# sangyun884/HR-VITON

Measured on AMD Instinct MI355X. Metric: 1024x768 try-on images/sec (train_generator.py step: tocg+glue, G fwd/bwd, D fwd/bwd x2, VGG, Adam), higher is better.
Workload: dtype bf16; 1 GPU; BASELINE configs[3] (SURVEY 8d config #4, headline): train_generator.py 1024x768, 4 img/GPU, --fp16 (bf16 MFMA operands, fp32 accumulate), SPADE ng...; global_batch=4, height=1024, width=768, parallelism=dp1-allreduce, persistent_grid_cus=256, dist_backend=none (single process), world_size=1, rccl_ranks=0

## Files before the change

hr-viton_amd/_lib.py:

```python
from __future__ import annotations

import ctypes as C
import os

HERE = os.path.dirname(os.path.abspath(__file__))
LIB_PATH = os.path.join(HERE, "libhrviton_hip.so")

HRV_MAX_SRC = 4
ACT_NONE, ACT_RELU, ACT_LRELU, ACT_TANH = 0, 1, 2, 3


class hrv_src_t(C.Structure):
    _fields_ = [("ptr", C.c_void_p), ("C", C.c_int32), ("cstride", C.c_int32), ("coff", C.c_int32),
                ("up_shift", C.c_int32), ("pre_act", C.c_int32), ("C_real", C.c_int32)]


class hrv_spade_epi_t(C.Structure):
    _fields_ = [("x", C.c_void_p), ("x_cstride", C.c_int32), ("x_coff", C.c_int32), ("C", C.c_int32),
                ("_pad", C.c_int32), ("mean", C.c_void_p), ("rstd", C.c_void_p), ("noise_z", C.c_void_p),
                ("noise_scale", C.c_void_p), ("g1p_out", C.c_void_p)]


class hrv_norm_bwd_t(C.Structure):
    _fields_ = [("N", C.c_int32), ("H", C.c_int32), ("W", C.c_int32), ("C", C.c_int32),
                ("x", C.c_void_p), ("x_cstride", C.c_int32), ("x_coff", C.c_int32),
                ("noise_z", C.c_void_p), ("noise_scale", C.c_void_p), ("mean", C.c_void_p), ("rstd", C.c_void_p),
                ("out", C.c_void_p), ("out_cstride", C.c_int32), ("out_coff", C.c_int32),
                ("g1p", C.c_void_p), ("g1p_cstride", C.c_int32), ("g1p_coff", C.c_int32),
                ("dout", C.c_void_p), ("dout_cstride", C.c_int32), ("dout_coff", C.c_int32),
                ("dnh", C.c_void_p), ("dnh_cstride", C.c_int32), ("dnh_coff", C.c_int32),
                ("dgb", C.c_void_p), ("dgb_cstride", C.c_int32), ("dgb_coff", C.c_int32),
                ("dx", C.c_void_p), ("dx_cstride", C.c_int32), ("dx_coff", C.c_int32),
                ("dx_accumulate", C.c_int32), ("act", C.c_int32), ("act_slope", C.c_float),
                ("dns_accumulate", C.c_int32), ("dnoise_scale", C.c_void_p), ("workspace", C.c_void_p),
                ("dgb_bf16", C.c_int32), ("out_bf16", C.c_int32), ("dx_bf16", C.c_int32), ("g1p_bf16", C.c_int32),
                ("dnh_bf16", C.c_int32), ("dout_bf16", C.c_int32),
                ("x_up_channels", C.c_int32), ("x2", C.c_void_p), ("x2_cstride", C.c_int32), ("x2_coff", C.c_int32)]


class hrv_sn_job_t(C.Structure):
    _fields_ = [("w", C.c_void_p), ("u", C.c_void_p), ("v", C.c_void_p), ("sigma", C.c_void_p), ("u_keep", C.c_void_p),
                ("v_keep", C.c_void_p), ("R", C.c_int32), ("K", C.c_int32)]


class hrv_thin_conv_t(C.Structure):
    _fields_ = [("src", C.c_void_p), ("N", C.c_int32), ("H", C.c_int32), ("W", C.c_int32), ("src_channels", C.c_int32),
                ("src_cstride", C.c_int32), ("src_coff", C.c_int32),
                ("w_oihw", C.c_void_p), ("Cout", C.c_int32), ("Cin", C.c_int32), ("KH", C.c_int32), ("KW", C.c_int32),
                ("sigma", C.c_void_p), ("wscale", C.c_float), ("mode", C.c_int32), ("shift", C.c_void_p),
                ("residual", C.c_void_p), ("res_cstride", C.c_int32), ("res_coff", C.c_int32), ("res_bf16", C.c_int32),
                ("res_mode", C.c_int32), ("act", C.c_int32), ("act_slope", C.c_float),
                ("out", C.c_void_p), ("out_cstride", C.c_int32), ("out_coff", C.c_int32), ("out_bf16", C.c_int32)]


class hrv_conv_cout1_t(C.Structure):
    _fields_ = [("x", C.c_void_p), ("N", C.c_int32), ("H", C.c_int32), ("W", C.c_int32), ("C", C.c_int32),
                ("x_cstride", C.c_int32), ("x_coff", C.c_int32), ("w_oihw", C.c_void_p), ("sigma", C.c_void_p),
                ("wscale", C.c_float), ("bias", C.c_void_p), ("K", C.c_int32), ("pad", C.c_int32),
                ("y", C.c_void_p), ("y_cstride", C.c_int32), ("y_coff", C.c_int32),
                ("dx", C.c_void_p), ("dx_cstride", C.c_int32), ("dx_coff", C.c_int32),
                ("add", C.c_void_p), ("add_cstride", C.c_int32), ("add_coff", C.c_int32),
                ("workspace", C.c_void_p), ("round_bf16", C.c_int32)]


class hrv_spade_gb_t(C.Structure):
    _fields_ = [("mode", C.c_int32), ("N", C.c_int32), ("H", C.c_int32), ("W", C.c_int32),
                ("src", C.c_void_p), ("src_cstride", C.c_int32), ("src_coff", C.c_int32), ("w_packed", C.c_void_p),
                ("C", C.c_int32), ("Cp", C.c_int32), ("hid", C.c_int32), ("x_f32", C.c_int32),
                ("x", C.c_void_p), ("x_cstride", C.c_int32), ("x_coff", C.c_int32),
                ("stat_stride", C.c_int32), ("g1p_bf16", C.c_int32),
                ("mean", C.c_void_p), ("rstd", C.c_void_p), ("noise_z", C.c_void_p), ("noise_scale", C.c_void_p),
                ("bias_gamma", C.c_void_p), ("bias_beta", C.c_void_p), ("g1p", C.c_void_p),
                ("act", C.c_int32), ("act_slope", C.c_float),
                ("out", C.c_void_p), ("out_cstride", C.c_int32), ("out_coff", C.c_int32), ("out_f32", C.c_int32),
                ("_pad", C.c_int32), ("mask", C.c_void_p), ("mask_cstride", C.c_int32), ("mask_coff", C.c_int32)]


class hrv_spade_fused_t(C.Structure):
    _fields_ = [("N", C.c_int32), ("H", C.c_int32), ("W", C.c_int32), ("C", C.c_int32),
                ("seg", C.c_void_p), ("seg_H", C.c_int32), ("seg_W", C.c_int32), ("seg_shift", C.c_int32), ("x_f32", C.c_int32),
                ("w_packed", C.c_void_p),
                ("x", C.c_void_p), ("x_cstride", C.c_int32), ("x_coff", C.c_int32),
                ("mean", C.c_void_p), ("rstd", C.c_void_p), ("noise_z", C.c_void_p), ("noise_scale", C.c_void_p),
                ("bias_gamma", C.c_void_p), ("bias_beta", C.c_void_p), ("g1p", C.c_void_p),
                ("act", C.c_int32), ("act_slope", C.c_float),
                ("out", C.c_void_p), ("out_cstride", C.c_int32), ("out_coff", C.c_int32),
                ("actv", C.c_void_p), ("actv_cstride", C.c_int32), ("actv_coff", C.c_int32),
                ("x_up_channels", C.c_int32), ("x2", C.c_void_p), ("x2_cstride", C.c_int32), ("x2_coff", C.c_int32)]


class hrv_conv_p2_t(C.Structure):
    _fields_ = [("N", C.c_int32), ("H", C.c_int32), ("W", C.c_int32), ("Cin", C.c_int32),
                ("src", C.c_void_p), ("src_cstride", C.c_int32), ("src_coff", C.c_int32), ("Cout", C.c_int32),
                ("w_packed", C.c_void_p), ("bias", C.c_void_p),
                ("act", C.c_int32), ("act_slope", C.c_float),
                ("mask", C.c_void_p), ("mask_cstride", C.c_int32), ("mask_coff", C.c_int32), ("mask_slope", C.c_float), ("out_f32", C.c_int32),
                ("out", C.c_void_p), ("out_cstride", C.c_int32), ("out_coff", C.c_int32),
                ("res_f32", C.c_int32), ("residual", C.c_void_p), ("res_cstride", C.c_int32), ("res_coff", C.c_int32),
                ("res_after_mask", C.c_int32)]


class hrv_conv_s2_t(C.Structure):
    _fields_ = [("mode", C.c_int32),
                ("N", C.c_int32), ("Hs", C.c_int32), ("Ws", C.c_int32), ("K", C.c_int32),
                ("src", C.c_void_p), ("src_cstride", C.c_int32), ("src_coff", C.c_int32),
                ("Ho", C.c_int32), ("Wo", C.c_int32), ("cols", C.c_int32), ("Cph", C.c_int32),
                ("w_packed", C.c_void_p), ("bias", C.c_void_p),
                ("act", C.c_int32), ("act_slope", C.c_float),
                ("out", C.c_void_p), ("out_cstride", C.c_int32), ("out_coff", C.c_int32), ("out_f32", C.c_int32),
                ("residual", C.c_void_p), ("res_cstride", C.c_int32), ("res_coff", C.c_int32), ("res_f32", C.c_int32),
                ("mask", C.c_void_p), ("mask_cstride", C.c_int32), ("mask_coff", C.c_int32), ("mask_slope", C.c_float)]


class hrv_s2_pack_job_t(C.Structure):
    _fields_ = [("mode_flags", C.c_int32), ("K", C.c_int32), ("cols", C.c_int32), ("Cph", C.c_int32),
                ("w", C.c_void_p), ("sigma", C.c_void_p), ("wscale", C.c_float), ("_pad", C.c_int32), ("out", C.c_void_p)]


class hrv_conv2d_t(C.Structure):
    _fields_ = [("N", C.c_int32), ("H", C.c_int32), ("W", C.c_int32), ("Ho", C.c_int32), ("Wo", C.c_int32),
                ("KH", C.c_int32), ("KW", C.c_int32), ("stride", C.c_int32), ("pad", C.c_int32),
                ("nsrc", C.c_int32), ("src", hrv_src_t * HRV_MAX_SRC),
                ("w_packed", C.c_void_p), ("w_oihw", C.c_void_p), ("Cout", C.c_int32), ("tile_cfg", C.c_int32),
                ("scale", C.c_void_p), ("shift", C.c_void_p), ("residual", C.c_void_p),
                ("res_cstride", C.c_int32), ("res_coff", C.c_int32), ("act", C.c_int32), ("act_slope", C.c_float),
                ("out", C.c_void_p), ("out_cstride", C.c_int32), ("out_coff", C.c_int32),
                ("spade", C.POINTER(hrv_spade_epi_t)), ("out_up_shift", C.c_int32), ("_pad2", C.c_int32),
                ("workspace", C.c_void_p), ("workspace_bytes", C.c_int64),
                ("pad_w_plus1", C.c_int32), ("free_extent", C.c_int32), ("out_step", C.c_int32),
                ("out_off_h", C.c_int32), ("out_off_w", C.c_int32), ("out_H", C.c_int32), ("out_W", C.c_int32),
                ("res_mode", C.c_int32), ("mixed_flags", C.c_int32), ("_pad3", C.c_int32)]


class hrv_flow_warp_t(C.Structure):
    _fields_ = [("src", C.c_void_p), ("N", C.c_int32), ("H", C.c_int32), ("W", C.c_int32), ("C", C.c_int32),
                ("src_cstride", C.c_int32), ("src_coff", C.c_int32), ("flow", C.c_void_p),
                ("fh", C.c_int32), ("fw", C.c_int32), ("Ho", C.c_int32), ("Wo", C.c_int32),
                ("rh", C.c_float), ("rw", C.c_float), ("norm_x", C.c_float), ("norm_y", C.c_float),
                ("out", C.c_void_p), ("out_cstride", C.c_int32), ("out_coff", C.c_int32), ("flow_up", C.c_void_p)]


class hrv_flow_warp_bwd_t(C.Structure):
    _fields_ = [("src", C.c_void_p), ("N", C.c_int32), ("H", C.c_int32), ("W", C.c_int32), ("C", C.c_int32),
                ("src_cstride", C.c_int32), ("src_coff", C.c_int32), ("flow_up", C.c_void_p),
                ("Ho", C.c_int32), ("Wo", C.c_int32), ("norm_x", C.c_float), ("norm_y", C.c_float),
                ("dout", C.c_void_p), ("dout_cstride", C.c_int32), ("dout_coff", C.c_int32),
                ("dsrc", C.c_void_p), ("dsrc_cstride", C.c_int32), ("dsrc_coff", C.c_int32),
                ("dflow", C.c_void_p), ("dflow_accumulate", C.c_int32), ("_pad", C.c_int32)]


class hrv_lpips_tap_t(C.Structure):
    _fields_ = [("f0", C.c_void_p), ("f1", C.c_void_p), ("lin", C.c_void_p),
                ("HW", C.c_int32), ("C", C.c_int32), ("cstride", C.c_int32), ("_pad", C.c_int32)]


_i32, _i64, _f, _vp = C.c_int32, C.c_int64, C.c_float, C.c_void_p
_ip = C.POINTER(C.c_int32)
SYMBOLS = {
    "hrv_version": (C.c_char_p, []),
    "hrv_last_error": (C.c_char_p, []),
    "hrv_device_check": (C.c_int, []),
    "hrv_set_reserved_cus": (C.c_int, [_i32]),
    "hrv_persistent_cus": (C.c_int, []),
    "hrv_diag_set_tlog": (C.c_int, [_vp, _i64]),
    "hrv_diag_reload_env": (C.c_int, []),
    "hrv_conv2d_pick_tile": (C.c_int, [_i64, _i32]),
    "hrv_conv2d_tile_bn": (C.c_int, [_i32]),
    "hrv_conv2d_tile_bm": (C.c_int, [_i32]),
    "hrv_conv2d_tile_row_bytes": (C.c_int, [_i32]),
    "hrv_conv2d_packed_elems": (_i64, [_i32, _i32, _i32, _i32, _ip, _i32]),
    "hrv_conv2d_pack_weight_f32": (C.c_int, [_vp, _i32, _i32, _i32, _i32, _ip, _ip, _i32, _vp]),
    "hrv_conv2d_pack_weight_dev_f32": (C.c_int, [_vp, _i32, _i32, _i32, _i32, _ip, _ip, _i32, _i32, _i32, _i32, _i32,
                                                 _i32, _f, _vp, _vp, _ip, _vp]),
    "hrv_conv2d_pack_weight_dev_bf16": (C.c_int, [_vp, _i32, _i32, _i32, _i32, _ip, _ip, _i32, _i32, _i32, _i32, _i32,
                                                  _i32, _f, _vp, _vp, _ip, _vp]),
    "hrv_conv2d_pack_record_bytes": (_i32, []),
    "hrv_conv2d_pack_weight_record": (C.c_int, [_vp, _i32, _i32, _i32, _i32, _ip, _ip, _i32, _i32, _i32, _i32, _i32, _i32, _f,
                                                _vp, _i32, _vp, _i32, _i32, _vp, _ip, _vp, _ip]),
    "hrv_conv2d_pack_weight_multi": (C.c_int, [_vp, _vp, _i32, _i32, _vp]),
    "hrv_conv2d_wgrad_workspace_bytes": (_i64, [_i32, _i32, _i32, _i32, _i64]),
    "hrv_conv2d_wgrad_nhwc_f32": (C.c_int, [_vp, _i32, _i32, _i32, _vp, _i32, _i32, _i32, _i32, _i32, _i32, _i32,
                                            _i32, _i32, _i32, _i32, _i32, _i32, _i32, _i32, _i32, _vp, _i64, _vp, _i32,
                                            _vp, _i32, _vp]),
    "hrv_conv2d_wgrad_bf16mma_nhwc_f32": (C.c_int, [_vp, _i32, _i32, _i32, _vp, _i32, _i32, _i32, _i32, _i32, _i32,
                                                    _i32, _i32, _i32, _i32, _i32, _i32, _i32, _i32, _i32, _i32, _vp,
                                                    _i64, _vp, _i32, _vp, _i32, _vp]),
    "hrv_conv2d_wgrad_bf16mma_st_nhwc_f32": (C.c_int, [_vp, _i32, _i32, _i32, _vp, _i32, _i32, _i32, _i32, _i32, _i32,
                                                       _i32, _i32, _i32, _i32, _i32, _i32, _i32, _i32, _i32, _i32,
                                                       _vp, _i64, _vp, _i32, _vp, _i32, _i32, _vp]),
    "hrv_colsum_nhwc_f32": (C.c_int, [_vp, _i64, _i32, _i32, _i32, _vp, _i64, _vp, _i32, _vp]),
    "hrv_norm_bwd_workspace_elems": (_i64, [_i32, _i32, _i32, _i32]),
    "hrv_spade_norm_bwd2_nhwc_f32": (C.c_int, [C.POINTER(hrv_norm_bwd_t), C.POINTER(hrv_norm_bwd_t), _vp]),
    "hrv_spade_norm_bwd_nhwc_f32": (C.c_int, [C.POINTER(hrv_norm_bwd_t), _vp]),
    "hrv_thin_conv_supported": (C.c_int, [_i32, _i32, _i32, _i32]),
    "hrv_thin_conv_bf16": (C.c_int, [C.POINTER(hrv_thin_conv_t), _vp]),
    "hrv_loss_f32": (C.c_int, [_vp, _vp, _i64, _i32, _f, _f, _vp, _vp, _vp, _i32, _vp]),
    "hrv_loss_bf16in_f32": (C.c_int, [_vp, _vp, _i64, _i32, _f, _f, _vp, _vp, _vp, _i32, _vp]),
    "hrv_scale_f32": (C.c_int, [_vp, _i64, _f, _vp, _vp]),
    "hrv_act_bwd_nhwc_f32": (C.c_int, [_vp, _i32, _i32, _vp, _i32, _i32, _i32, _i64, _i32, _f, _vp]),
    "hrv_tanh_bwd_f32": (C.c_int, [_vp, _vp, _i64, _vp, _vp]),
    "hrv_add_slice_nhwc_f32": (C.c_int, [_vp, _i32, _i32, _vp, _i32, _i32, _i32, _i64, _i32, _vp]),
    "hrv_downsum2x2_nhwc_f32": (C.c_int, [_vp, _i32, _i32, _i32, _i32, _i32, _i32, _vp, _i32, _i32, _i32, _vp]),
    "hrv_avgpool3x3s2_bwd_nhwc_f32": (C.c_int, [_vp, _i32, _i32, _i32, _i32, _i32, _i32, _vp, _i32, _i32, _i32, _vp]),
    "hrv_maxpool2x2_nhwc_f32": (C.c_int, [_vp, _i32, _i32, _i32, _i32, _vp, _vp]),
    "hrv_maxpool2x2_nhwc_bf16": (C.c_int, [_vp, _i32, _i32, _i32, _i32, _vp, _vp]),
    "hrv_maxpool2x2_bwd_nhwc_f32": (C.c_int, [_vp, _vp, _i32, _i32, _i32, _i32, _vp, _vp]),
    "hrv_maxpool2x2_bwd_relu_nhwc_f32": (C.c_int, [_vp, _vp, _i32, _i32, _i32, _i32, _vp, _vp]),
    "hrv_maxpool2x2_bwd_relu_nhwc_xbf16": (C.c_int, [_vp, _vp, _i32, _i32, _i32, _i32, _vp, _vp]),
    "hrv_maxpool2x2_bwd_relu_nhwc_bf16": (C.c_int, [_vp, _vp, _i32, _i32, _i32, _i32, _vp, _vp]),
    "hrv_add_slice_nhwc_bf16": (C.c_int, [_vp, _i32, _i32, _vp, _i32, _i32, _i32, _i64, _i32, _vp]),
    "hrv_adam_f32": (C.c_int, [_vp, _vp, _vp, _vp, _i64, _f, _f, _f, _f, _f, _i32, _f, _vp]),
    "hrv_adam_hyper_f32": (C.c_int, [_vp, _vp, _f, _f, _vp, _vp]),
    "hrv_adam_dev_f32": (C.c_int, [_vp, _vp, _vp, _vp, _i64, _vp, _f, _f, _f, _f, _f, _vp]),
    "hrv_spectral_norm_f32": (C.c_int, [_vp, _i32, _i32, _vp, _vp, _i32, _f, _vp, _vp, _vp]),
    "hrv_spectral_norm_bwd_f32": (C.c_int, [_vp, _vp, _vp, _vp, _vp, _i32, _i32, _vp, _vp, _i32, _vp]),
    "hrv_spectral_norm_batched_f32": (C.c_int, [_vp, _i32, _i32, _f, _vp, _vp]),
    "hrv_conv2d_pack_weight_pair_dev": (C.c_int, [_vp, _vp, _i32, _i32, _i32, _i32, _i32, _i32, _ip, _ip, _i32, _i32, _i32,
                                                  _i32, _vp, _ip, _vp]),
    "hrv_spade_vec_prep_f32": (C.c_int, [_vp, _vp, _vp, _i32, _vp, _vp, _vp]),
    "hrv_spade_vec_prep_multi_f32": (C.c_int, [_i32, _vp, _vp, _vp, _vp, _vp, _vp, _vp, _vp, _vp]),
    "hrv_shared_taps_prep_f32": (C.c_int, [_vp, _vp, _i32, _i32, _i32, _i32, _vp, _vp, _vp]),
    "hrv_shared_taps_grad_f32": (C.c_int, [_vp, _vp, _i32, _i32, _i32, _i32, _vp, _vp, _vp]),
    "hrv_conv2d_workspace_bytes": (_i64, [C.POINTER(hrv_conv2d_t)]),
    "hrv_conv2d_nhwc_f32": (C.c_int, [C.POINTER(hrv_conv2d_t), _vp]),
    "hrv_conv2d_packed_elems_bf16": (_i64, [_i32, _i32, _i32, _i32, _ip, _i32]),
    "hrv_conv2d_pack_weight_bf16": (C.c_int, [_vp, _i32, _i32, _i32, _i32, _ip, _ip, _i32, _vp]),
    "hrv_conv2d_nhwc_bf16": (C.c_int, [C.POINTER(hrv_conv2d_t), _vp]),
    "hrv_conv2d_naive_nhwc_f32": (C.c_int, [C.POINTER(hrv_conv2d_t), _vp]),
    "hrv_tapsum_nhwc_f32": (C.c_int, [_vp, _i32, _i32, _i32, _i32, _i32, _i32, _i32, _i32, _vp, _vp, _i32, _vp, _i32,
                                      _vp]),
    "hrv_instnorm_workspace_elems": (_i64, [_i32, _i32, _i32, _i32]),
    "hrv_instnorm_stats_nhwc_f32": (C.c_int, [_vp, _i32, _i32, _i32, _i32, _i32, _i32, _vp, _vp, _f, _vp, _vp, _vp,
                                              _vp]),
    "hrv_instnorm_stats2_nhwc_f32": (C.c_int, [_vp, _i32, _i32, _i32, _i32, _i32, _i32, _vp, _vp, _vp, _vp, _f, _vp, _vp, _vp, _vp, _vp, _vp]),
    "hrv_instnorm_stats2_up_nhwc_f32": (C.c_int, [_vp, _i32, _i32, _i32, _vp, _i32, _i32, _i32, _i32, _i32, _i32, _vp, _vp, _vp, _vp, _f, _vp,
                                                  _vp, _vp, _vp, _vp, _vp]),
    "hrv_instnorm_stats_nhwc_bf16": (C.c_int, [_vp, _i32, _i32, _i32, _i32, _i32, _i32, _vp, _vp, _f, _vp, _vp, _vp,
                                               _vp]),
    "hrv_instnorm_apply_nhwc_f32": (C.c_int, [_vp, _i32, _i32, _i32, _i32, _i32, _i32, _vp, _vp, _i32, _f, _vp, _i32,
                                              _i32, _vp]),
    "hrv_avgpool3x3s2_nhwc_f32": (C.c_int, [_vp, _i32, _i32, _i32, _i32, _i32, _i32, _vp, _i32, _i32, _vp]),
    "hrv_mul_channel_nhwc_f32": (C.c_int, [_vp, _i32, _i32, _vp, _i32, _i32, _i32, _i64, _vp]),
    "hrv_gauss_blur_nhwc_f32": (C.c_int, [_vp, _i32, _i32, _i32, _i32, _i32, _vp, _i32, _vp, _vp, _vp]),
    "hrv_parse_argmax_nhwc_f32": (C.c_int, [_vp, _i32, _i32, _i64, _vp, _vp, _i32, _vp]),
    "hrv_resize_nchw_f32": (C.c_int, [_vp, _i32, _i32, _i32, _i32, _i32, _i32, _vp, _vp]),
    "hrv_occlusion_nhwc_f32": (C.c_int, [_vp, _i32, _i32, _vp, _i32, _vp, _i32, _i32, _i64, _vp]),
    "hrv_nchw_to_nhwc_f32": (C.c_int, [_vp, _i32, _i32, _i32, _i32, _vp, _i32, _i32, _i32, _vp]),
    "hrv_nchw_f32_to_nhwc_bf16": (C.c_int, [_vp, _i32, _i32, _i32, _i32, _vp, _i32, _i32, _i32, _vp]),
    "hrv_nhwc_bf16_to_nchw_f32": (C.c_int, [_vp, _i32, _i32, _i32, _i32, _i32, _i32, _vp, _vp]),
    "hrv_nhwc_to_nchw_f32": (C.c_int, [_vp, _i32, _i32, _i32, _i32, _i32, _i32, _vp, _vp]),
    "hrv_space_to_depth2_nhwc_f32": (C.c_int, [_vp, _i32, _i32, _i32, _i32, _i32, _i32, _vp, _vp]),
    "hrv_depth_to_space2_nhwc_f32": (C.c_int, [_vp, _i32, _i32, _i32, _i32, _vp, _vp]),
    "hrv_conv_cout1_fwd_f32": (C.c_int, [C.POINTER(hrv_conv_cout1_t), _vp]),
    "hrv_conv_cout1_dgrad_f32": (C.c_int, [C.POINTER(hrv_conv_cout1_t), _vp]),
    "hrv_conv_cout1_wgrad_slabs": (_i32, [_i32, _i32, _i32]),
    "hrv_conv_cout1_wgrad_f32": (C.c_int, [C.POINTER(hrv_conv_cout1_t), _vp, _i32, _vp, _i32, _vp]),
    "hrv_concat_nhwc_nchw_f32": (C.c_int, [_vp, _i32, _i32, _i32, _vp, _i32, _i32, _i32, _i32, _vp, _i32, _vp]),
    "hrv_resize_bilinear_nhwc_f32": (C.c_int, [_vp, _i32, _i32, _i32, _i32, _i32, _i32, _i32, _i32, _f, _f,
                                               _vp, _i32, _i32, _vp, _i32, _i32, _vp]),
    "hrv_flow_warp_nhwc_f32": (C.c_int, [C.POINTER(hrv_flow_warp_t), _vp]),
    "hrv_bn_finalize_f32": (C.c_int, [_vp, _vp, _i32, _i32, _i32, _f, _i64, _vp, _vp, _f, _f, _vp, _vp, _vp, _vp, _vp,
                                      _vp, _vp]),
    "hrv_affine_act_nhwc_f32": (C.c_int, [_vp, _i32, _i32, _i32, _i64, _vp, _vp, _vp, _i32, _i32, _i32, _f, _vp, _i32,
                                          _i32, _vp]),
    "hrv_bn_bwd_workspace_elems": (_i64, [_i32]),
    "hrv_bn_bwd_nhwc_f32": (C.c_int, [_vp, _i32, _i32, _vp, _i32, _i32, _i32, _i64, _vp, _vp, _vp, _vp, _vp, _i32, _i32,
                                      _i32, _vp, _vp, _i32, _vp]),
    "hrv_resize_bilinear_bwd_nhwc_f32": (C.c_int, [_vp, _i32, _i32, _i32, _i32, _i32, _i32, _f, _f, _vp, _i32, _i32,
                                                   _i32, _i32, _i32, _vp]),
    "hrv_resize_nearest_nchw_f32": (C.c_int, [_vp, _i32, _i32, _i32, _i32, _i32, _vp, _vp]),
    "hrv_resize_nearest_nchw_bwd_f32": (C.c_int, [_vp, _i32, _i32, _i32, _i32, _i32, _vp, _vp]),
    "hrv_resize_nearest_nhwc_f32": (C.c_int, [_vp, _i32, _i32, _i32, _i32, _i32, _i32, _i32, _i32, _vp, _i32, _i32, _vp, _i32, _i32, _vp]),
    "hrv_resize_nearest_bwd_nhwc_f32": (C.c_int, [_vp, _i32, _i32, _i32, _i32, _i32, _i32, _vp, _i32, _i32, _i32, _i32, _i32, _vp]),
    "hrv_flow_warp_bwd_nhwc_f32": (C.c_int, [C.POINTER(hrv_flow_warp_bwd_t), _vp]),
    "hrv_grid_sample_nchw_f32": (C.c_int, [_vp, _i32, _i32, _i32, _i32, _vp, _i32, _i32, _vp, _vp]),
    "hrv_grid_sample_nchw_bwd_f32": (C.c_int, [_vp, _i32, _i32, _i32, _i32, _vp, _i32, _i32, _vp, _vp, _vp, _vp]),
    "hrv_softmax_nchw_f32": (C.c_int, [_vp, _i32, _i32, _i64, _vp, _vp]),
    "hrv_softmax_nchw_bwd_f32": (C.c_int, [_vp, _vp, _i32, _i32, _i64, _vp, _vp]),
    "hrv_cross_entropy_nchw_f32": (C.c_int, [_vp, _vp, _i32, _i32, _i64, _f, _vp, _vp, _vp, _vp]),
    "hrv_tapsum_bwd_nhwc_f32": (C.c_int, [_vp, _i32, _i32, _i32, _i32, _i32, _i32, _i32, _i32, _vp, _i32, _vp]),
    "hrv_tap_expand_nhwc": (C.c_int, [_vp, _i32, _i32, _i32, _i32, _i32, _i32, _i32, _i32, _i32, _i32, _vp, _vp]),
    "hrv_mul_f32": (C.c_int, [_vp, _vp, _i64, _vp, _vp]),
    "hrv_spade_gb_packed_bytes": (_i64, [_i32, _i32, _i32, _i32]),
    "hrv_spade_gb_supported": (C.c_int, [_i32, _i32, _i32, _i32, _i32, _i32, _i32]),
    "hrv_spade_gb_pack_dev": (C.c_int, [_i32, _vp, _vp, _i32, _i32, _i32, _vp, _vp]),
    "hrv_spade_gb_bf16": (C.c_int, [C.POINTER(hrv_spade_gb_t), _vp]),
    "hrv_conv_p2_packed_bytes": (C.c_int64, [_i32, _i32]),
    "hrv_conv_p2_supported": (C.c_int, [_i32, _i32, _i32, _i32, _i32]),
    "hrv_conv_p2_pack_dev": (C.c_int, [_i32, _vp, _vp, _i32, _i32, _vp, _f, _vp, _vp]),
    "hrv_conv_p2_bf16": (C.c_int, [C.POINTER(hrv_conv_p2_t), _vp]),
    "hrv_conv_s2_packed_bytes": (C.c_int64, [_i32, _i32, _i32]),
    "hrv_conv_s2_supported": (C.c_int, [_i32, _i32, _i32, _i32, _i32, _i32, _i32]),
    "hrv_conv_s2_pack_dev": (C.c_int, [_i32, _vp, _i32, _i32, _i32, _vp, _f, _vp, _vp]),
    "hrv_conv_s2_pack_multi_dev": (C.c_int, [_i32, C.POINTER(hrv_s2_pack_job_t), _vp]),
    "hrv_conv_s2_bf16": (C.c_int, [C.POINTER(hrv_conv_s2_t), _vp]),
    "hrv_space_to_depth2_cells_bf16": (C.c_int, [_vp, _i32, _i32, _i32, _i32, _i32, _i32, _i32, _i32, _i32, _vp, _vp]),
    "hrv_instnorm_apply_nhwc_bf16out": (C.c_int, [_vp, _i32, _i32, _i32, _i32, _i32, _i32, _vp, _vp, _i32, _f, _vp, _i32, _i32, _vp]),
    "hrv_scale_bf16": (C.c_int, [_vp, _i64, _f, _vp, _vp]),
    "hrv_split3_nhwc_bf16": (C.c_int, [_vp, _i64, _i32, _i32, _i32, _vp, _vp]),
    "hrv_conv2d_wgrad_s2_supported": (C.c_int, [_i32, _i32, _i32, _i32, _i32, _i32, _i32, _i32, _i32]),
    "hrv_conv2d_wgrad_tr_supported": (C.c_int, [_i32, _i32, _i32, _i32, _i32, _i32, _i32, _i32, _i32, _i32, _i32, _i32]),
    "hrv_pad_width_nhwc_bf16": (C.c_int, [_vp, _i64, _i32, _i32, _i32, _vp, _vp]),
    "hrv_spade_fused_packed_bytes": (C.c_int64, [_i32]),
    "hrv_spade_fused_supported": (C.c_int, [_i32, _i32, _i32, _i32, _i32, _i32]),
    "hrv_spade_fused_pack_dev": (C.c_int, [_vp, _vp, _i32, _vp, _vp, _i32, _vp, _vp]),
    "hrv_spade_fused_bf16": (C.c_int, [C.POINTER(hrv_spade_fused_t), _vp]),
    "hrv_tv_loss_f32": (C.c_int, [_vp, _i32, _i32, _i32, _vp, _vp, _vp, _vp]),
    "hrv_rgb_to_gray_u8": (C.c_int, [_vp, _i64, _vp, _vp]),
    "hrv_pair_stats_workspace_bytes": (_i64, [_i32, _i32, _i32]),
    "hrv_pair_stats_u8": (C.c_int, [_vp, _vp, _vp, _i32, _i32, _i32, _vp, _i64, _vp, _vp, _vp]),
    "hrv_lpips_prep_u8": (C.c_int, [_vp, _i32, _i32, _i32, C.POINTER(C.c_float), C.POINTER(C.c_float), _vp, _vp]),
    "hrv_lpips_prep_nchw_f32": (C.c_int, [_vp, _i32, _i32, _i32, _i32, C.POINTER(C.c_float), C.POINTER(C.c_float), _vp, _vp]),
    "hrv_maxpool3x3s2_nhwc_f32": (C.c_int, [_vp, _i32, _i32, _i32, _i32, _vp, _vp]),
    "hrv_lpips_head_f32": (C.c_int, [C.POINTER(hrv_lpips_tap_t), _i32, _i32, _vp, _vp]),
}

_lib = None


class HrvError(RuntimeError):
    pass


def load():
    global _lib
    if _lib is not None:
        return _lib
    if not os.path.exists(LIB_PATH):
        raise HrvError(
            f"{LIB_PATH} is missing: build it with `python -c 'import __graft_entry__ as g; g.build()'` "
            "(hipcc --offload-arch=gfx950). There is no CPU fallback for the HIP path.")
    lib = C.CDLL(LIB_PATH)
    for name, (res, args) in SYMBOLS.items():
        fn = getattr(lib, name)
        fn.restype = res
        fn.argtypes = args
    _lib = lib
    return lib


def reload_env():
    if _lib is not None:
        _lib.hrv_diag_reload_env()


# ... 5 lines not shown
```

hr-viton_amd/csrc/train.hip:

```cpp
#include <string.h>

#include "hrv_common.h"

namespace hrv {

typedef float f32x4 __attribute__((ext_vector_type(4)));

static inline int grid_for(size_t work, int block = 256) {
  size_t g = (work + block - 1) / block;
  const size_t cap = 256 * 16;
  return (int)(g < 1 ? 1 : (g > cap ? cap : g));
}

__device__ __forceinline__ float dact(float y, int act, float slope) {
  if (act == HRV_ACT_RELU) return y > 0.f ? 1.f : 0.f;
  if (act == HRV_ACT_LRELU) return y > 0.f ? 1.f : slope;
  return 1.f;
}

struct XSrc {
  const float* x; int x_cs, x_co;
  const float* x2; int x2_cs, x2_co, up_g;
  int H, W;
};
struct XThread {
  const float* base;
  int cs, lo, W, Wl;
};
__device__ __forceinline__ XThread xsrc_thread(const XSrc& s, int n, int g) {
  XThread t;
  t.W = s.W; t.Wl = s.W >> 1;
  t.lo = (s.up_g > 0 && g < s.up_g) ? 1 : 0;
  if (s.up_g > 0 && !t.lo) {
    t.cs = s.x2_cs;
    t.base = s.x2 + (size_t)n * s.H * s.W * s.x2_cs + s.x2_co + (g - s.up_g) * 4;
  } else {
    t.cs = s.x_cs;
    t.base = s.x + (size_t)n * (t.lo ? (s.H >> 1) * (s.W >> 1) : s.H * s.W) * s.x_cs + s.x_co + g * 4;
  }
  return t;
}
__device__ __forceinline__ const float* xsrc_ptr(const XThread& t, int px) {
  int q = px;
  if (t.lo) {
    const int h = px / t.W, w = px - h * t.W;
    q = (h >> 1) * t.Wl + (w >> 1);
  }
  return t.base + (size_t)q * t.cs;
}

struct NormBwdParams {
  XSrc xs;
  const float* z; const float* ns;
  const float* mean; const float* rstd;
  const float* out; int out_cs, out_co;
  const float* g1p; int g_cs, g_co;
  const float* dout; int do_cs, do_co;
  float* dnh; int dn_cs, dn_co;
  float* dgb; int dgb_cs, dgb_co;
  int N, H, W, C4, act; float slope;
  int NB; float* part;
  int dgb_bf16, out_bf16;
  int g1p_bf16;
  int dnh_bf16;
  int dout_bf16;
  int dbeta_in_place;
};

__device__ __forceinline__ f32x4 ld4(const float* p) { return *reinterpret_cast<const f32x4*>(p); }
__device__ __forceinline__ f32x4 ld4_bf16(const void* base, size_t elem) {
  const uint2 u = *reinterpret_cast<const uint2*>(reinterpret_cast<const unsigned short*>(base) + elem);
  f32x4 v;
  v[0] = __builtin_bit_cast(float, u.x << 16); v[1] = __builtin_bit_cast(float, u.x & 0xFFFF0000u);
  v[2] = __builtin_bit_cast(float, u.y << 16); v[3] = __builtin_bit_cast(float, u.y & 0xFFFF0000u);
  return v;
}
typedef __bf16 bf16x4t __attribute__((ext_vector_type(4)));
__device__ __forceinline__ void st4_bf16(void* base, size_t elem, f32x4 v) {
  *reinterpret_cast<bf16x4t*>(reinterpret_cast<unsigned short*>(base) + elem) = __builtin_convertvector(v, bf16x4t);
}

__global__ __launch_bounds__(256) void norm_bwd_stage1_kernel(const NormBwdParams p) {
  __shared__ f32x4 red[2][256];
  const int n = blockIdx.y, b = blockIdx.x, t = threadIdx.x;
  const int HW = p.H * p.W, C = p.C4 * 4;
  const int PB = (HW + p.NB - 1) / p.NB;
  const int p0 = b * PB, p1 = min(p0 + PB, HW);
  const int GB = p.C4 < NORM_GCAP ? p.C4 : NORM_GCAP;
  const int R = 256 / GB;
  const int r = t / GB, gl = t - r * GB;
  {
    const int g = blockIdx.z * GB + gl;
    f32x4 s1 = (f32x4)(0.f), s2 = (f32x4)(0.f);
    if (r < R && g < p.C4) {
      const f32x4 mu = ld4(p.mean + (size_t)n * C + g * 4), rs = ld4(p.rstd + (size_t)n * C + g * 4);
      const f32x4 ns4 = p.z ? ld4(p.ns + g * 4) : (f32x4)(0.f);
      const XThread xt = xsrc_thread(p.xs, n, g);
      struct In { f32x4 v, d, o, g1; float zz; };
      auto load = [&](int px) {
        In L;
        const size_t pix = (size_t)n * HW + px;
        L.v = ld4(xsrc_ptr(xt, px));
        L.zz = 0.f;
        if (p.z) {
          const int h = px / p.W, w = px - h * p.W;
          L.zz = p.z[((size_t)n * p.W + w) * p.H + h];
        }
        L.d = p.dout_bf16 ? ld4_bf16(p.dout, pix * p.do_cs + p.do_co + g * 4) : ld4(p.dout + pix * p.do_cs + p.do_co + g * 4);
        L.o = (f32x4)(0.f);
        if (p.act != HRV_ACT_NONE) {
          const size_t oe = pix * p.out_cs + p.out_co + g * 4;
          L.o = p.out_bf16 ? ld4_bf16(p.out, oe) : ld4(p.out + oe);
        }
        L.g1 = (f32x4)(1.f);
        if (p.g1p) {
          const size_t ge1 = pix * p.g_cs + p.g_co + g * 4;
          L.g1 = p.g1p_bf16 ? ld4_bf16(p.g1p, ge1) : ld4(p.g1p + ge1);
        }
        return L;
      };
      auto finish = [&](int px, const In& L) {
        const size_t pix = (size_t)n * HW + px;
        f32x4 v = L.v;
        if (p.z) v += L.zz * ns4;
        const f32x4 nh = (v - mu) * rs;
        f32x4 dpre = L.d;
        if (p.act != HRV_ACT_NONE) {
#pragma unroll
          for (int e = 0; e < 4; ++e) dpre[e] *= dact(L.o[e], p.act, p.slope);
        }
        f32x4 dnh = dpre;
        if (p.g1p) dnh *= L.g1;
        if (p.dnh_bf16) st4_bf16(p.dnh, pix * p.dn_cs + p.dn_co + g * 4, dnh);
        else *reinterpret_cast<f32x4*>(p.dnh + pix * p.dn_cs + p.dn_co + g * 4) = dnh;
        if (p.dgb) {
          const size_t ge = pix * p.dgb_cs + p.dgb_co + g * 4;
          if (p.dgb_bf16) {
            st4_bf16(p.dgb, ge, dpre * nh);
            if (!p.dbeta_in_place) st4_bf16(p.dgb, ge + C, dpre);
          } else {
            *reinterpret_cast<f32x4*>(p.dgb + ge) = dpre * nh;
            if (!p.dbeta_in_place) *reinterpret_cast<f32x4*>(p.dgb + ge + C) = dpre;
          }
        }
        s1 += dnh;
        s2 += dnh * nh;
      };
      int px = p0 + r;
      for (; px + R < p1; px += 2 * R) {
        const In A = load(px), B = load(px + R);
        finish(px, A);
        finish(px + R, B);
      }
      if (px < p1) finish(px, load(px));
    }
    red[0][t] = s1;
    red[1][t] = s2;
    __syncthreads();
    if (r == 0 && g < p.C4) {
      for (int rr = 1; rr < R; ++rr) { s1 += red[0][rr * GB + gl]; s2 += red[1][rr * GB + gl]; }
      float* dst = p.part + (((size_t)n * p.NB + b) * C + g * 4) * 2;
#pragma unroll
      for (int e = 0; e < 4; ++e) { dst[2 * e] = s1[e]; dst[2 * e + 1] = s2[e]; }
    }
  }
}

__global__ void norm_bwd_finalize_kernel(const float* __restrict__ part, int N, int NB, int C, int HW,
                                         float* __restrict__ m1, float* __restrict__ m2) {
  const int t = blockIdx.x * blockDim.x + threadIdx.x;
  const int i = t >> 4, l = t & 15;
  const bool live = i < N * C;
  const int ii = live ? i : 0;
  const int n = ii / C, c = ii - n * C;
  double s1 = 0.0, s2 = 0.0;
  for (int b = l; b < NB; b += 16) {
    const float* src = part + (((size_t)n * NB + b) * C + c) * 2;
    s1 += (double)src[0];
    s2 += (double)src[1];
  }
#pragma unroll
  for (int o = 8; o > 0; o >>= 1) {
    s1 += __shfl_xor(s1, o, 16);
    s2 += __shfl_xor(s2, o, 16);
  }
  if (live && l == 0) {
    m1[i] = (float)(s1 / HW);
    m2[i] = (float)(s2 / HW);
  }
}

struct NormBwd2Params {
  XSrc xs;
  const float* z; const float* ns;
  const float* mean; const float* rstd; const float* m1; const float* m2;
  const float* dnh; int dn_cs, dn_co; int dnh_bf16;
  float* dx; int dx_cs, dx_co; int accumulate;
  int dx_bf16;
  int N, H, W, C4;
  int NB; float* part;
};

__global__ __launch_bounds__(256) void norm_bwd_stage2_kernel(const NormBwd2Params p) {
  __shared__ f32x4 red[256];
  const int n = blockIdx.y, b = blockIdx.x, t = threadIdx.x;
  const int HW = p.H * p.W, C = p.C4 * 4;
  const int PB = (HW + p.NB - 1) / p.NB;
  const int p0 = b * PB, p1 = min(p0 + PB, HW);
  const int GB = p.C4 < NORM_GCAP ? p.C4 : NORM_GCAP;
  const int R = 256 / GB;
  const int r = t / GB, gl = t - r * GB;
  {
    const int g = blockIdx.z * GB + gl;
    f32x4 sz = (f32x4)(0.f);
    if (r < R && g < p.C4) {
      const size_t sc = (size_t)n * C + g * 4;
      const f32x4 mu = ld4(p.mean + sc), rs = ld4(p.rstd + sc), a1 = ld4(p.m1 + sc), a2 = ld4(p.m2 + sc);
      const f32x4 ns4 = p.z ? ld4(p.ns + g * 4) : (f32x4)(0.f);
      const XThread xt = xsrc_thread(p.xs, n, g);
      struct In { f32x4 v, dn, acc; float zz; };
      auto load = [&](int px) {
        In L;
        const size_t pix = (size_t)n * HW + px;
        L.v = ld4(xsrc_ptr(xt, px));
        L.zz = 0.f;
        if (p.z) {
          const int h = px / p.W, w = px - h * p.W;
          L.zz = p.z[((size_t)n * p.W + w) * p.H + h];
        }
        const size_t de = pix * p.dn_cs + p.dn_co + g * 4;
        L.dn = p.dnh_bf16 ? ld4_bf16(p.dnh, de) : ld4(p.dnh + de);
        L.acc = (f32x4)(0.f);
        if (!p.dx_bf16 && p.accumulate) L.acc = ld4(p.dx + pix * p.dx_cs + p.dx_co + g * 4);
        return L;
      };
      auto finish = [&](int px, const In& L) {
#pragma clang fp contract(off)
        const size_t pix = (size_t)n * HW + px;
        f32x4 v = L.v;
        if (p.z) v += L.zz * ns4;
        const f32x4 nh = (v - mu) * rs;
        f32x4 d = rs * (L.dn - a1 - nh * a2);
        sz += d * L.zz;
        if (p.dx_bf16) {
          st4_bf16(p.dx, pix * p.dx_cs + p.dx_co + g * 4, d);
        } else {
          float* o = p.dx + pix * p.dx_cs + p.dx_co + g * 4;
          if (p.accumulate) d += L.acc;
          *reinterpret_cast<f32x4*>(o) = d;
        }
      };
      int px = p0 + r;
      for (; px + R < p1; px += 2 * R) {
        const In A = load(px), B = load(px + R);
        finish(px, A);
        finish(px + R, B);
      }
      if (px < p1) finish(px, load(px));
    }
    if (p.z) {
      red[t] = sz;
      __syncthreads();
      if (r == 0 && g < p.C4) {
        for (int rr = 1; rr < R; ++rr) sz += red[rr * GB + gl];
        *reinterpret_cast<f32x4*>(p.part + ((size_t)n * p.NB + b) * C + g * 4) = sz;
      }
    }
  }
}

__global__ __launch_bounds__(256) void norm_bwd2_stage1_kernel(const NormBwdParams pa, const NormBwdParams pb) {
  __shared__ f32x4 red[4][256];
  const NormBwdParams& p = pa;
  const int n = blockIdx.y, b = blockIdx.x, t = threadIdx.x;
  const int HW = p.H * p.W, C = p.C4 * 4;
  const int PB = (HW + p.NB - 1) / p.NB;
  const int p0 = b * PB, p1 = min(p0 + PB, HW);
  const int GB = p.C4 < NORM_GCAP ? p.C4 : NORM_GCAP;
  const int R = 256 / GB;
  const int r = t / GB, gl = t - r * GB;
  const int g = blockIdx.z * GB + gl;
  f32x4 s1a = (f32x4)(0.f), s2a = (f32x4)(0.f), s1b = (f32x4)(0.f), s2b = (f32x4)(0.f);
  if (r < R && g < p.C4) {
    const f32x4 mua = ld4(pa.mean + (size_t)n * C + g * 4), rsa = ld4(pa.rstd + (size_t)n * C + g * 4);
    const f32x4 mub = ld4(pb.mean + (size_t)n * C + g * 4), rsb = ld4(pb.rstd + (size_t)n * C + g * 4);
    const f32x4 nsa = pa.z ? ld4(pa.ns + g * 4) : (f32x4)(0.f), nsb = pb.z ? ld4(pb.ns + g * 4) : (f32x4)(0.f);
    const XThread xt = xsrc_thread(p.xs, n, g);
    struct In1 { f32x4 d, o, g1; float zz; };
    struct In { f32x4 v; In1 a, b; };
    auto load1 = [&](const NormBwdParams& q, size_t pix, int h, int w) {
      In1 L;
      L.zz = q.z ? q.z[((size_t)n * p.W + w) * p.H + h] : 0.f;
      L.d = q.dout_bf16 ? ld4_bf16(q.dout, pix * q.do_cs + q.do_co + g * 4) : ld4(q.dout + pix * q.do_cs + q.do_co + g * 4);
      L.o = (f32x4)(0.f);
      if (q.act != HRV_ACT_NONE) {
        const size_t oe = pix * q.out_cs + q.out_co + g * 4;
        L.o = q.out_bf16 ? ld4_bf16(q.out, oe) : ld4(q.out + oe);
      }
      L.g1 = (f32x4)(1.f);
      if (q.g1p) {
        const size_t ge1 = pix * q.g_cs + q.g_co + g * 4;
        L.g1 = q.g1p_bf16 ? ld4_bf16(q.g1p, ge1) : ld4(q.g1p + ge1);
      }
      return L;
    };
    auto load = [&](int px) {
      In L;
      const size_t pix = (size_t)n * HW + px;
      L.v = ld4(xsrc_ptr(xt, px));
      const int h = px / p.W, w = px - h * p.W;
      L.a = load1(pa, pix, h, w);
      L.b = load1(pb, pix, h, w);
      return L;
    };
    auto finish1 = [&](const NormBwdParams& q, size_t pix, f32x4 v, const In1& L, f32x4 mu, f32x4 rs, f32x4 ns4, f32x4& s1, f32x4& s2) {
      if (q.z) v += L.zz * ns4;
      const f32x4 nh = (v - mu) * rs;
      f32x4 dpre = L.d;
      if (q.act != HRV_ACT_NONE) {
#pragma unroll
        for (int e = 0; e < 4; ++e) dpre[e] *= dact(L.o[e], q.act, q.slope);
      }
      f32x4 dnh = dpre;
      if (q.g1p) dnh *= L.g1;
      if (q.dnh_bf16) st4_bf16(q.dnh, pix * q.dn_cs + q.dn_co + g * 4, dnh);
      else *reinterpret_cast<f32x4*>(q.dnh + pix * q.dn_cs + q.dn_co + g * 4) = dnh;
      if (q.dgb) {
        const size_t ge = pix * q.dgb_cs + q.dgb_co + g * 4;
        if (q.dgb_bf16) {
          st4_bf16(q.dgb, ge, dpre * nh);
          if (!q.dbeta_in_place) st4_bf16(q.dgb, ge + C, dpre);
        } else {
          *reinterpret_cast<f32x4*>(q.dgb + ge) = dpre * nh;
          if (!q.dbeta_in_place) *reinterpret_cast<f32x4*>(q.dgb + ge + C) = dpre;
        }
      }
      s1 += dnh;
      s2 += dnh * nh;
    };
    auto finish = [&](int px, const In& L) {
      const size_t pix = (size_t)n * HW + px;
      finish1(pa, pix, L.v, L.a, mua, rsa, nsa, s1a, s2a);
      finish1(pb, pix, L.v, L.b, mub, rsb, nsb, s1b, s2b);
    };
    for (int px = p0 + r; px < p1; px += R) finish(px, load(px));
  }
  red[0][t] = s1a; red[1][t] = s2a; red[2][t] = s1b; red[3][t] = s2b;
  __syncthreads();
  if (r == 0 && g < p.C4) {
    for (int rr = 1; rr < R; ++rr) {
      s1a += red[0][rr * GB + gl]; s2a += red[1][rr * GB + gl];
      s1b += red[2][rr * GB + gl]; s2b += red[3][rr * GB + gl];
    }
    const size_t o = (((size_t)n * p.NB + b) * C + g * 4) * 2;
#pragma unroll
    for (int e = 0; e < 4; ++e) {
      pa.part[o + 2 * e] = s1a[e]; pa.part[o + 2 * e + 1] = s2a[e];
      pb.part[o + 2 * e] = s1b[e]; pb.part[o + 2 * e + 1] = s2b[e];
    }
  }
}

__global__ __launch_bounds__(256) void norm_bwd2_stage2_kernel(const NormBwd2Params pa, const NormBwd2Params pb) {
  __shared__ f32x4 red[2][256];
  const NormBwd2Params& p = pa;
  const int n = blockIdx.y, b = blockIdx.x, t = threadIdx.x;
  const int HW = p.H * p.W, C = p.C4 * 4;
  const int PB = (HW + p.NB - 1) / p.NB;
  const int p0 = b * PB, p1 = min(p0 + PB, HW);
  const int GB = p.C4 < NORM_GCAP ? p.C4 : NORM_GCAP;
  const int R = 256 / GB;
  const int r = t / GB, gl = t - r * GB;
  const int g = blockIdx.z * GB + gl;
  f32x4 sza = (f32x4)(0.f), szb = (f32x4)(0.f);
  if (r < R && g < p.C4) {
    const size_t sc = (size_t)n * C + g * 4;
    const f32x4 mua = ld4(pa.mean + sc), rsa = ld4(pa.rstd + sc), a1a = ld4(pa.m1 + sc), a2a = ld4(pa.m2 + sc);
    const f32x4 mub = ld4(pb.mean + sc), rsb = ld4(pb.rstd + sc), a1b = ld4(pb.m1 + sc), a2b = ld4(pb.m2 + sc);
    const f32x4 nsa = pa.z ? ld4(pa.ns + g * 4) : (f32x4)(0.f), nsb = pb.z ? ld4(pb.ns + g * 4) : (f32x4)(0.f);
    const XThread xt = xsrc_thread(p.xs, n, g);
    struct In { f32x4 v, dna, dnb; float za, zb; };
    auto load = [&](int px) {
      In L;
      const size_t pix = (size_t)n * HW + px;
      L.v = ld4(xsrc_ptr(xt, px));
      const int h = px / p.W, w = px - h * p.W;
      const size_t zi = ((size_t)n * p.W + w) * p.H + h;
      L.za = pa.z ? pa.z[zi] : 0.f;
      L.zb = pb.z ? pb.z[zi] : 0.f;
      const size_t dea = pix * pa.dn_cs + pa.dn_co + g * 4, deb = pix * pb.dn_cs + pb.dn_co + g * 4;
      L.dna = pa.dnh_bf16 ? ld4_bf16(pa.dnh, dea) : ld4(pa.dnh + dea);
      L.dnb = pb.dnh_bf16 ? ld4_bf16(pb.dnh, deb) : ld4(pb.dnh + deb);
      return L;
    };
    auto finish = [&](int px, const In& L) {
#pragma clang fp contract(off)
      const size_t pix = (size_t)n * HW + px;
      f32x4 va = L.v, vb = L.v;
      if (pa.z) va += L.za * nsa;
      if (pb.z) vb += L.zb * nsb;
      const f32x4 nha = (va - mua) * rsa, nhb = (vb - mub) * rsb;
      const f32x4 da = rsa * (L.dna - a1a - nha * a2a);
      const f32x4 db = rsb * (L.dnb - a1b - nhb * a2b);
      sza += da * L.za;
      szb += db * L.zb;
      *reinterpret_cast<f32x4*>(p.dx + pix * p.dx_cs + p.dx_co + g * 4) = db + da;
    };
    int px = p0 + r;
    for (; px + R < p1; px += 2 * R) {
      const In A = load(px), B = load(px + R);
      finish(px, A);
      finish(px + R, B);
    }
    if (px < p1) finish(px, load(px));
  }
  red[0][t] = sza; red[1][t] = szb;
  __syncthreads();
  if (r == 0 && g < p.C4) {
    for (int rr = 1; rr < R; ++rr) { sza += red[0][rr * GB + gl]; szb += red[1][rr * GB + gl]; }
    if (pa.z) *reinterpret_cast<f32x4*>(pa.part + ((size_t)n * p.NB + b) * C + g * 4) = sza;
    if (pb.z) *reinterpret_cast<f32x4*>(pb.part + ((size_t)n * p.NB + b) * C + g * 4) = szb;
  }
}

template <bool AB>
__global__ __launch_bounds__(256) void loss_kernel(const float* __restrict__ a, const float* __restrict__ b, size_t n,
                                                   int mode_flags, float gscale, float* __restrict__ grad,
                                                   float* __restrict__ part, int vec) {
  __shared__ float red[256];
  float s = 0.f;
  const int mode = mode_flags & 15;
  const bool relu_mask = (mode_flags & 16) != 0;
  const bool grad_bf16 = (mode_flags & 32) != 0;
  auto term = [&](float x, float y, float& g) -> float {
    float l;
    if (mode == 0) { const float d = x - y; l = fabsf(d); g = d > 0.f ? 1.f : (d < 0.f ? -1.f : 0.f); }
    else if (mode == 1) { l = fmaxf(1.f + x, 0.f); g = x > -1.f ? 1.f : 0.f; }
    else if (mode == 2) { l = fmaxf(1.f - x, 0.f); g = x < 1.f ? -1.f : 0.f; }
    else if (mode == 3) { l = -x; g = -1.f; }
    else { const float d = x - y; l = d * d; g = 2.f * d; }
    g = (relu_mask && !(x > 0.f)) ? 0.f : gscale * g;
    return l;
  };
  typedef unsigned short u16x4v __attribute__((ext_vector_type(4)));
  auto ld4v = [](const float* p, size_t k) -> f32x4 {
    if constexpr (AB) {
      const u16x4v h = *reinterpret_cast<const u16x4v*>(reinterpret_cast<const unsigned short*>(p) + k);
      f32x4 v;
#pragma unroll
      for (int e = 0; e < 4; ++e) v[e] = __builtin_bit_cast(float, (unsigned)h[e] << 16);
      return v;
    } else {
      return *reinterpret_cast<const f32x4*>(p + k);
    }
  };
  const size_t n4 = vec ? n / 4 : 0;
  for (size_t i = (size_t)blockIdx.x * blockDim.x + threadIdx.x; i < n4; i += (size_t)gridDim.x * blockDim.x) {
    const f32x4 x4 = ld4v(a, 4 * i);
    const f32x4 y4 = b ? ld4v(b, 4 * i) : (f32x4)(0.f);
    f32x4 g4;
#pragma unroll
    for (int e = 0; e < 4; ++e) {
      float g;
      s += term(x4[e], y4[e], g);
      g4[e] = g;
    }
    if (grad) {
      if (grad_bf16) st4_bf16(grad, 4 * i, g4);
      else *reinterpret_cast<f32x4*>(grad + 4 * i) = g4;
    }
  }
  for (size_t i = 4 * n4 + (size_t)blockIdx.x * blockDim.x + threadIdx.x; i < n; i += (size_t)gridDim.x * blockDim.x) {
    float x, y = 0.f, g;
    if constexpr (AB) {
      x = __builtin_bit_cast(float, (unsigned)reinterpret_cast<const unsigned short*>(a)[i] << 16);
      if (b) y = __builtin_bit_cast(float, (unsigned)reinterpret_cast<const unsigned short*>(b)[i] << 16);
    } else {
      x = a[i];
      if (b) y = b[i];
    }
    s += term(x, y, g);
    if (grad) {
      if (grad_bf16) reinterpret_cast<unsigned short*>(grad)[i] = (unsigned short)(__builtin_bit_cast(unsigned, __builtin_bit_cast(unsigned, g) + 0x7fffu + ((__builtin_bit_cast(unsigned, g) >> 16) & 1u)) >> 16);
      else grad[i] = g;
    }
  }
  red[threadIdx.x] = s;
  __syncthreads();
  for (int o = 128; o > 0; o >>= 1) {
    if (threadIdx.x < o) red[threadIdx.x] += red[threadIdx.x + o];
    __syncthreads();
  }
  if (threadIdx.x == 0) part[blockIdx.x] = red[0];
}

__global__ void loss_final_kernel(const float* __restrict__ part, int nb, float lscale, float* __restrict__ out,
                                  int accumulate) {
  if (blockIdx.x != 0 || threadIdx.x >= 64) return;
  double s = 0.0;
  for (int i = threadIdx.x; i < nb; i += 64) s += (double)part[i];
#pragma unroll
  for (int o = 32; o > 0; o >>= 1) s += __shfl_down(s, o, 64);
  if (threadIdx.x == 0) {
    const float v = (float)(s * (double)lscale);
    out[0] = accumulate ? out[0] + v : v;
  }
}

__global__ void scale_kernel(float* __restrict__ x, size_t n, float s_host, const float* __restrict__ s_dev) {
  const float s = s_dev ? s_host * s_dev[0] : s_host;
  for (size_t i = (size_t)blockIdx.x * blockDim.x + threadIdx.x; i < n; i += (size_t)gridDim.x * blockDim.x) x[i] *= s;
}

__global__ void tanh_bwd_kernel(const float* __restrict__ dy, const float* __restrict__ y, size_t n, float* __restrict__ out) {
  for (size_t i = (size_t)blockIdx.x * blockDim.x + threadIdx.x; i < n; i += (size_t)gridDim.x * blockDim.x) {
    const float t = y[i];
    out[i] = dy[i] * (1.f - t * t);
  }
}

__global__ void act_bwd_kernel(float* __restrict__ d, int dcs, int dco, const float* __restrict__ y, int ycs, int yco, int C4,
                               size_t npix, int act, float slope) {
  const size_t total = npix * C4;
  for (size_t i = (size_t)blockIdx.x * blockDim.x + threadIdx.x; i < total; i += (size_t)gridDim.x * blockDim.x) {
    const int g = (int)(i % C4);
    const size_t pix = i / C4;
    float* o = d + pix * dcs + dco + g * 4;
    f32x4 v = ld4(o);
    const f32x4 yy = ld4(y + pix * ycs + yco + g * 4);
#pragma unroll
    for (int e = 0; e < 4; ++e) v[e] *= dact(yy[e], act, slope);
    *reinterpret_cast<f32x4*>(o) = v;
  }
}

__global__ void add_slice_kernel(const float* __restrict__ a, int acs, int aco, float* __restrict__ out, int ocs, int oco,
                                 int C4, size_t npix, int accumulate) {
  const size_t total = npix * C4;
  for (size_t i = (size_t)blockIdx.x * blockDim.x + threadIdx.x; i < total; i += (size_t)gridDim.x * blockDim.x) {
    const int g = (int)(i % C4);
    const size_t pix = i / C4;
    f32x4 v = ld4(a + pix * acs + aco + g * 4);
    float* o = out + pix * ocs + oco + g * 4;
    if (accumulate) v += ld4(o);
    *reinterpret_cast<f32x4*>(o) = v;
  }
}

__global__ void downsum2x2_kernel(const float* __restrict__ dhi, int N, int Hl, int Wl, int C4, int hcs, int hco,
                                  float* __restrict__ dlo, int lcs, int lco, int accumulate) {
  const size_t total = (size_t)N * Hl * Wl * C4;
  for (size_t i = (size_t)blockIdx.x * blockDim.x + threadIdx.x; i < total; i += (size_t)gridDim.x * blockDim.x) {
    const int g = (int)(i % C4);
    const size_t pix = i / C4;
    const int w = (int)(pix % Wl);
    const size_t t = pix / Wl;
    const int h = (int)(t % Hl);
    const int n = (int)(t / Hl);
    const float* s = dhi + (((size_t)n * 2 * Hl + 2 * h) * 2 * Wl + 2 * w) * hcs + hco + g * 4;
    f32x4 v = ld4(s) + ld4(s + hcs) + ld4(s + (size_t)2 * Wl * hcs) + ld4(s + (size_t)2 * Wl * hcs + hcs);
    if (accumulate == 2) {
      st4_bf16(dlo, pix * lcs + lco + g * 4, v);
      continue;
    }
    float* o = dlo + pix * lcs + lco + g * 4;
    if (accumulate) v += ld4(o);
    *reinterpret_cast<f32x4*>(o) = v;
  }
}

__global__ void avgpool3s2_bwd_kernel(const float* __restrict__ dy, int N, int H, int W, int C4, int Ho, int Wo,
                                      int ycs, int yco, float* __restrict__ dx, int xcs, int xco, int accumulate) {
  const size_t total = (size_t)N * H * W * C4;
  for (size_t i = (size_t)blockIdx.x * blockDim.x + threadIdx.x; i < total; i += (size_t)gridDim.x * blockDim.x) {
    const int g = (int)(i % C4);
    const size_t pix = i / C4;
// ... 372 lines not shown
  float* const nso = ns_all + j.off_ns[q];
  for (int i = blockIdx.x * 256 + threadIdx.x; i < ncols; i += gridDim.x * 256) {
    const int l = i & 63, c = (i >> 6) * 32 + (l & 31);
    bc[i] = c < C ? (l < 32 ? j.gb[q][c] : j.bb[q][c]) : 0.f;
    if (i < Cp) nso[i] = i < C ? j.ns[q][i] : 0.f;
  }
}

struct SharedTaps {
  const float* w[4];
  const float* b[4];
  float* gw[4];
  float* gb[4];
  int n, hid, c, cp;
};
__global__ __launch_bounds__(256) void shared_taps_prep_kernel(const SharedTaps p, float* __restrict__ wt, float* __restrict__ bt) {
  const int K = 9 * p.cp, total = p.n * p.hid * K;
  for (int i = blockIdx.x * 256 + threadIdx.x; i < total; i += gridDim.x * 256) {
    const int k = i % K, row = i / K;
    const int tap = k / p.cp, ch = k - tap * p.cp;
    const int j = row / p.hid, o = row - j * p.hid;
    wt[i] = ch < p.c ? p.w[j][((size_t)o * p.c + ch) * 9 + tap] : 0.f;
  }
  for (int i = blockIdx.x * 256 + threadIdx.x; i < p.n * p.hid; i += gridDim.x * 256) bt[i] = p.b[i / p.hid][i % p.hid];
}
__global__ __launch_bounds__(256) void shared_taps_grad_kernel(const SharedTaps p, const float* __restrict__ dw,
                                                               const float* __restrict__ db) {
  const int per = p.hid * p.c * 9, total = p.n * per, K = 9 * p.cp;
  for (int i = blockIdx.x * 256 + threadIdx.x; i < total; i += gridDim.x * 256) {
    const int j = i / per, r = i - j * per;
    const int tap = r % 9, ch = (r / 9) % p.c, o = r / (9 * p.c);
    p.gw[j][r] = dw[(size_t)(j * p.hid + o) * K + tap * p.cp + ch];
  }
  for (int i = blockIdx.x * 256 + threadIdx.x; i < p.n * p.hid; i += gridDim.x * 256) p.gb[i / p.hid][i % p.hid] = db[i];
}

}

using namespace hrv;

extern "C" int hrv_spade_vec_prep_f32(const float* gamma_bias, const float* beta_bias, const float* noise_scale, int32_t C,
                                      float* bias_interleaved, float* noise_scale_padded, hrv_stream_t stream) {
  HRV_REQUIRE(gamma_bias && beta_bias && noise_scale && bias_interleaved && noise_scale_padded && C > 0, "spade_vec_prep: bad args");
  const int ncols = (C + 31) / 32 * 64, Cp = (C + 3) / 4 * 4;
  hipLaunchKernelGGL(spade_vec_prep_kernel, dim3((ncols + 255) / 256), dim3(256), 0, (hipStream_t)stream, gamma_bias, beta_bias,
                     noise_scale, C, ncols, Cp, bias_interleaved, noise_scale_padded);
  return check_launch("spade_vec_prep_kernel");
}

extern "C" int hrv_spade_vec_prep_multi_f32(int32_t n, const float* const* gamma_bias, const float* const* beta_bias,
                                            const float* const* noise_scale, const int32_t* C, const int32_t* off_bias, const int32_t* off_noise,
                                            float* bias_interleaved_all, float* noise_scale_padded_all, hrv_stream_t stream) {
  HRV_REQUIRE(n > 0 && n <= VEC_MAXJOBS && gamma_bias && beta_bias && noise_scale && C && off_bias && off_noise && bias_interleaved_all &&
                  noise_scale_padded_all, "spade_vec_prep_multi: 1 .. %d norms", VEC_MAXJOBS);
  VecJobs j;
  memset(&j, 0, sizeof(j));
  int cmax = 0;
  for (int i = 0; i < n; ++i) {
    HRV_REQUIRE(gamma_bias[i] && beta_bias[i] && noise_scale[i] && C[i] > 0 && off_bias[i] >= 0 && off_noise[i] >= 0 && off_bias[i] % 4 == 0 &&
                    off_noise[i] % 4 == 0, "spade_vec_prep_multi: job %d", i);
    j.gb[i] = gamma_bias[i]; j.bb[i] = beta_bias[i]; j.ns[i] = noise_scale[i];
    j.C[i] = C[i]; j.off_bc[i] = off_bias[i]; j.off_ns[i] = off_noise[i];
    if (C[i] > cmax) cmax = C[i];
  }
  const int ncols = (cmax + 31) / 32 * 64;
  hipLaunchKernelGGL(spade_vec_prep_multi_kernel, dim3((ncols + 255) / 256, n), dim3(256), 0, (hipStream_t)stream, j, bias_interleaved_all,
                     noise_scale_padded_all);
  return check_launch("spade_vec_prep_multi_kernel");
}

static int shared_taps_fill(SharedTaps& p, const float* const* w, const float* const* b, float* const* gw, float* const* gb,
                            int32_t n, int32_t hid, int32_t c, int32_t cp) {
  HRV_REQUIRE(n >= 1 && n <= 4 && hid > 0 && c > 0 && cp >= c, "shared_taps: n in 1..4, cp >= c");
  memset(&p, 0, sizeof(p));
  for (int i = 0; i < n; ++i) {
    if (w) { HRV_REQUIRE(w[i] && b[i], "shared_taps: null weight"); p.w[i] = w[i]; p.b[i] = b[i]; }
    if (gw) { HRV_REQUIRE(gw[i] && gb[i], "shared_taps: null gradient"); p.gw[i] = gw[i]; p.gb[i] = gb[i]; }
  }
  p.n = n; p.hid = hid; p.c = c; p.cp = cp;
  return HRV_OK;
}

extern "C" int hrv_shared_taps_prep_f32(const float* const* w, const float* const* b, int32_t n, int32_t hid, int32_t c,
                                        int32_t cp, float* wt, float* bt, hrv_stream_t stream) {
  HRV_REQUIRE(w && b && wt && bt, "shared_taps_prep: null pointer");
  SharedTaps p;
  const int rc = shared_taps_fill(p, w, b, nullptr, nullptr, n, hid, c, cp);
  if (rc) return rc;
  hipLaunchKernelGGL(shared_taps_prep_kernel, dim3(grid_for((size_t)n * hid * 9 * cp)), dim3(256), 0, (hipStream_t)stream, p, wt, bt);
  return check_launch("shared_taps_prep_kernel");
}

extern "C" int hrv_shared_taps_grad_f32(const float* dw, const float* db, int32_t n, int32_t hid, int32_t c, int32_t cp,
                                        float* const* gw, float* const* gb, hrv_stream_t stream) {
  HRV_REQUIRE(dw && db && gw && gb, "shared_taps_grad: null pointer");
  SharedTaps p;
  const int rc = shared_taps_fill(p, nullptr, nullptr, gw, gb, n, hid, c, cp);
  if (rc) return rc;
  hipLaunchKernelGGL(shared_taps_grad_kernel, dim3(grid_for((size_t)n * hid * c * 9)), dim3(256), 0, (hipStream_t)stream, p, dw, db);
  return check_launch("shared_taps_grad_kernel");
}

extern "C" int64_t hrv_norm_bwd_workspace_elems(int32_t N, int32_t H, int32_t W, int32_t C) {
  if (N <= 0 || H <= 0 || W <= 0 || C <= 0) return -1;
  const int nb = norm_slabs(H * W);
  return (int64_t)N * nb * ((C + 3) / 4 * 4) * 2 + (int64_t)N * ((C + 3) / 4 * 4) * 2;
}

static int norm_bwd_check(const hrv_norm_bwd_t* d) {
  HRV_REQUIRE(d && d->x && d->mean && d->rstd && d->dout && d->dnh && d->dx && d->workspace, "norm_bwd: null pointer");
  HRV_REQUIRE(d->N > 0 && d->H > 0 && d->W > 0 && d->C > 0 && d->C % 4 == 0, "norm_bwd: extent (C %% 4 == 0)");
  HRV_REQUIRE((d->noise_z == nullptr) == (d->noise_scale == nullptr), "norm_bwd: noise_z/noise_scale go together");
  HRV_REQUIRE(d->act == HRV_ACT_NONE || d->out, "norm_bwd: activation output needed for its derivative");
  HRV_REQUIRE(((d->x_cstride | d->x_coff | d->out_cstride | d->out_coff | d->g1p_cstride | d->g1p_coff | d->dout_cstride |
                d->dout_coff | d->dnh_cstride | d->dnh_coff | d->dgb_cstride | d->dgb_coff | d->dx_cstride | d->dx_coff) & 3) == 0,
              "norm_bwd: strides/offsets must be multiples of 4");
  const int C = d->C;
  if (d->x_up_channels > 0) {
    HRV_REQUIRE(d->x2 && d->x_up_channels % 4 == 0 && d->x_up_channels < C && d->H % 2 == 0 && d->W % 2 == 0 &&
                    d->x_coff + d->x_up_channels <= d->x_cstride && d->x2_cstride % 4 == 0 && d->x2_coff % 4 == 0 &&
                    d->x2_coff + (C - d->x_up_channels) <= d->x2_cstride && ((uintptr_t)d->x2 & 15) == 0,
                "norm_bwd: upsampled source (%d of %d channels, %d x %d)", d->x_up_channels, C, d->H, d->W);
  }
  HRV_REQUIRE(!(d->dx_bf16 && d->dx_accumulate), "norm_bwd: a bf16 dx cannot be accumulated into");
  return HRV_OK;
}

static void norm_bwd_fill(const hrv_norm_bwd_t* d, NormBwdParams& p, NormBwd2Params& q, float*& m1, float*& m2) {
  const int C = d->C, nb = norm_slabs(d->H * d->W);
  float* part = d->workspace;
  m1 = part + (size_t)d->N * nb * C * 2;
  m2 = m1 + (size_t)d->N * C;
  XSrc xs;
  xs.x = d->x; xs.x_cs = d->x_cstride; xs.x_co = d->x_coff; xs.H = d->H; xs.W = d->W;
  xs.x2 = d->x2; xs.x2_cs = d->x2_cstride; xs.x2_co = d->x2_coff; xs.up_g = d->x_up_channels / 4;
  p.xs = xs; p.z = d->noise_z; p.ns = d->noise_scale;
  p.mean = d->mean; p.rstd = d->rstd; p.out = d->out; p.out_cs = d->out_cstride; p.out_co = d->out_coff;
  p.g1p = d->g1p; p.g_cs = d->g1p_cstride; p.g_co = d->g1p_coff; p.g1p_bf16 = d->g1p_bf16;
  p.dout = d->dout; p.do_cs = d->dout_cstride; p.do_co = d->dout_coff; p.dout_bf16 = d->dout_bf16;
  p.dnh = d->dnh; p.dn_cs = d->dnh_cstride; p.dn_co = d->dnh_coff; p.dnh_bf16 = d->dnh_bf16;
  p.dgb = d->dgb; p.dgb_cs = d->dgb_cstride; p.dgb_co = d->dgb_coff;
  p.N = d->N; p.H = d->H; p.W = d->W; p.C4 = C / 4; p.act = d->act; p.slope = d->act_slope; p.NB = nb; p.part = part;
  p.dgb_bf16 = d->dgb_bf16; p.out_bf16 = d->out_bf16;
  p.dbeta_in_place = (d->dgb != nullptr && (const void*)d->dout == (const void*)d->dgb && d->dout_cstride == d->dgb_cstride &&
                      d->dout_coff == d->dgb_coff + C && d->dout_bf16 == d->dgb_bf16 && d->act == HRV_ACT_NONE) ? 1 : 0;
  q.xs = xs; q.z = d->noise_z; q.ns = d->noise_scale;
  q.mean = d->mean; q.rstd = d->rstd; q.m1 = m1; q.m2 = m2;
  q.dnh = d->dnh; q.dn_cs = d->dnh_cstride; q.dn_co = d->dnh_coff; q.dnh_bf16 = d->dnh_bf16;
  q.dx = d->dx; q.dx_cs = d->dx_cstride; q.dx_co = d->dx_coff; q.accumulate = d->dx_accumulate;
  q.dx_bf16 = d->dx_bf16;
  q.N = d->N; q.H = d->H; q.W = d->W; q.C4 = C / 4; q.NB = nb; q.part = part;
}

extern "C" int hrv_spade_norm_bwd_nhwc_f32(const hrv_norm_bwd_t* d, hrv_stream_t stream) {
  int rc = norm_bwd_check(d);
  if (rc) return rc;
  const int HW = d->H * d->W, C = d->C;
  const int nb = norm_slabs(HW);
  hipStream_t st = (hipStream_t)stream;
  NormBwdParams p;
  NormBwd2Params q;
  float *m1, *m2;
  norm_bwd_fill(d, p, q, m1, m2);
  hipLaunchKernelGGL(norm_bwd_stage1_kernel, dim3(nb, d->N, norm_chunks(C / 4)), dim3(256), 0, st, p);
  rc = check_launch("norm_bwd_stage1_kernel");
  if (rc) return rc;
  hipLaunchKernelGGL(norm_bwd_finalize_kernel, dim3((d->N * C * 16 + 255) / 256), dim3(256), 0, st, p.part, d->N, nb, C, HW, m1, m2);
  rc = check_launch("norm_bwd_finalize_kernel");
  if (rc) return rc;
  hipLaunchKernelGGL(norm_bwd_stage2_kernel, dim3(nb, d->N, norm_chunks(C / 4)), dim3(256), 0, st, q);
  rc = check_launch("norm_bwd_stage2_kernel");
  if (rc) return rc;
  if (d->noise_z && d->dnoise_scale) {
    hipLaunchKernelGGL(sum_rows_kernel<>, dim3((C + 15) / 16), dim3(256), 0, st, p.part, d->N * nb, C, d->dnoise_scale,
                       d->dns_accumulate);
    rc = check_launch("sum_rows_kernel");
  }
  return rc;
}

extern "C" int hrv_spade_norm_bwd2_nhwc_f32(const hrv_norm_bwd_t* a, const hrv_norm_bwd_t* b, hrv_stream_t stream) {
  int rc = norm_bwd_check(a);
  if (rc) return rc;
  rc = norm_bwd_check(b);
  if (rc) return rc;
  HRV_REQUIRE(a->x == b->x && a->x2 == b->x2 && a->x_cstride == b->x_cstride && a->x_coff == b->x_coff && a->x_up_channels == b->x_up_channels &&
                  a->N == b->N && a->H == b->H && a->W == b->W && a->C == b->C,
              "norm_bwd2: both norms must normalise the same x");
  HRV_REQUIRE(!a->dx_bf16 && !a->dx_accumulate && a->workspace != b->workspace && a->dnh != b->dnh, "norm_bwd2: dx fp32 (written, = dx_a + dx_b); separate scratch");
  const int HW = a->H * a->W, C = a->C;
  const int nb = norm_slabs(HW);
  hipStream_t st = (hipStream_t)stream;
  NormBwdParams pa, pb;
  NormBwd2Params qa, qb;
  float *m1a, *m2a, *m1b, *m2b;
  norm_bwd_fill(a, pa, qa, m1a, m2a);
  norm_bwd_fill(b, pb, qb, m1b, m2b);
  hipLaunchKernelGGL(norm_bwd2_stage1_kernel, dim3(nb, a->N, norm_chunks(C / 4)), dim3(256), 0, st, pa, pb);
  rc = check_launch("norm_bwd2_stage1_kernel");
  if (rc) return rc;
  hipLaunchKernelGGL(norm_bwd_finalize_kernel, dim3((a->N * C * 16 + 255) / 256), dim3(256), 0, st, pa.part, a->N, nb, C, HW, m1a, m2a);
  hipLaunchKernelGGL(norm_bwd_finalize_kernel, dim3((a->N * C * 16 + 255) / 256), dim3(256), 0, st, pb.part, a->N, nb, C, HW, m1b, m2b);
  rc = check_launch("norm_bwd_finalize_kernel");
  if (rc) return rc;
  hipLaunchKernelGGL(norm_bwd2_stage2_kernel, dim3(nb, a->N, norm_chunks(C / 4)), dim3(256), 0, st, qa, qb);
  rc = check_launch("norm_bwd2_stage2_kernel");
  if (rc) return rc;
  const hrv_norm_bwd_t* ds[2] = {a, b};
  const NormBwdParams* ps[2] = {&pa, &pb};
  for (int k = 0; k < 2; ++k)
    if (ds[k]->noise_z && ds[k]->dnoise_scale) {
      hipLaunchKernelGGL(sum_rows_kernel<>, dim3((C + 15) / 16), dim3(256), 0, st, ps[k]->part, a->N * nb, C, ds[k]->dnoise_scale,
                         ds[k]->dns_accumulate);
      rc = check_launch("sum_rows_kernel");
    }
  return rc;
}

extern "C" int hrv_loss_f32(const float* a, const float* b, int64_t n, int32_t mode, float lscale, float gscale,
                            float* grad, float* workspace, float* loss_out, int32_t accumulate, hrv_stream_t stream) {
  HRV_REQUIRE(a && workspace && loss_out && n > 0 && mode >= 0 && (mode & 15) <= 4 && (mode & ~31) == 0, "loss: bad args");
  HRV_REQUIRE(((mode & 15) != 0 && (mode & 15) != 4) || b, "loss: mode needs a target tensor");
  const int nb = grid_for((size_t)n) > 1024 ? 1024 : grid_for((size_t)n);
  hipStream_t st = (hipStream_t)stream;
  const int vec = (((uintptr_t)a | (uintptr_t)b | (uintptr_t)grad) & 15) == 0;
  hipLaunchKernelGGL(loss_kernel<false>, dim3(nb), dim3(256), 0, st, a, b, (size_t)n, mode, gscale, grad, workspace, vec);
  int rc = check_launch("loss_kernel");
  if (rc) return rc;
  hipLaunchKernelGGL(loss_final_kernel, dim3(1), dim3(64), 0, st, workspace, nb, lscale, loss_out, accumulate);
  return check_launch("loss_final_kernel");
}

extern "C" int hrv_loss_bf16in_f32(const uint16_t* a, const uint16_t* b, int64_t n, int32_t mode, float lscale, float gscale,
                                   float* grad, float* workspace, float* loss_out, int32_t accumulate, hrv_stream_t stream) {
  HRV_REQUIRE(a && workspace && loss_out && n > 0 && mode >= 0 && (mode & 15) <= 4 && (mode & ~63) == 0, "loss_bf16in: bad args");
  HRV_REQUIRE(((mode & 15) != 0 && (mode & 15) != 4) || b, "loss_bf16in: mode needs a target tensor");
  const int nb = grid_for((size_t)n) > 1024 ? 1024 : grid_for((size_t)n);
  hipStream_t st = (hipStream_t)stream;
  const int vec = ((((uintptr_t)a | (uintptr_t)b) & 7) | ((uintptr_t)grad & 15)) == 0;
  hipLaunchKernelGGL(loss_kernel<true>, dim3(nb), dim3(256), 0, st, (const float*)a, (const float*)b, (size_t)n, mode, gscale, grad,
                     workspace, vec);
  int rc = check_launch("loss_kernel[bf16 in]");
  if (rc) return rc;
  hipLaunchKernelGGL(loss_final_kernel, dim3(1), dim3(64), 0, st, workspace, nb, lscale, loss_out, accumulate);
  return check_launch("loss_final_kernel");
}

extern "C" int hrv_downsum2x2_nhwc_f32(const float* dhi, int32_t N, int32_t Hl, int32_t Wl, int32_t C, int32_t hi_cstride,
                                       int32_t hi_coff, float* dlo, int32_t lo_cstride, int32_t lo_coff,
                                       int32_t accumulate, hrv_stream_t stream) {
  HRV_REQUIRE(dhi && dlo && N > 0 && Hl > 0 && Wl > 0 && C > 0 && C % 4 == 0 &&
                  ((hi_cstride | hi_coff | lo_cstride | lo_coff) & 3) == 0, "downsum2x2: bad args");
  const size_t total = (size_t)N * Hl * Wl * (C / 4);
  hipLaunchKernelGGL(downsum2x2_kernel, dim3(grid_for(total)), dim3(256), 0, (hipStream_t)stream, dhi, N, Hl, Wl, C / 4,
                     hi_cstride, hi_coff, dlo, lo_cstride, lo_coff, accumulate);
  return check_launch("downsum2x2_kernel");
}

extern "C" int hrv_avgpool3x3s2_bwd_nhwc_f32(const float* dy, int32_t N, int32_t H, int32_t W, int32_t C, int32_t dy_cstride,
                                             int32_t dy_coff, float* dx, int32_t dx_cstride, int32_t dx_coff,
                                             int32_t accumulate, hrv_stream_t stream) {
  HRV_REQUIRE(dy && dx && N > 0 && H > 0 && W > 0 && C > 0 && C % 4 == 0 &&
                  ((dy_cstride | dy_coff | dx_cstride | dx_coff) & 3) == 0, "avgpool_bwd: bad args");
  const int Ho = (H + 2 - 3) / 2 + 1, Wo = (W + 2 - 3) / 2 + 1;
  const size_t total = (size_t)N * H * W * (C / 4);
  hipLaunchKernelGGL(avgpool3s2_bwd_kernel, dim3(grid_for(total)), dim3(256), 0, (hipStream_t)stream, dy, N, H, W, C / 4,
                     Ho, Wo, dy_cstride, dy_coff, dx, dx_cstride, dx_coff, accumulate);
  return check_launch("avgpool3s2_bwd_kernel");
}

extern "C" int hrv_maxpool2x2_nhwc_f32(const float* x, int32_t N, int32_t H, int32_t W, int32_t C, float* y,
                                       hrv_stream_t stream) {
  HRV_REQUIRE(x && y && N > 0 && H > 0 && W > 0 && H % 2 == 0 && W % 2 == 0 && C > 0 && C % 4 == 0, "maxpool: bad args");
  const size_t total = (size_t)N * (H / 2) * (W / 2) * (C / 4);
  hipLaunchKernelGGL(maxpool2_kernel<false>, dim3(grid_for(total)), dim3(256), 0, (hipStream_t)stream, x, N, H / 2, W / 2, C / 4, C,
                     y, C);
  return check_launch("maxpool2_kernel");
}

extern "C" int hrv_maxpool2x2_nhwc_bf16(const uint16_t* x, int32_t N, int32_t H, int32_t W, int32_t C, uint16_t* y,
                                        hrv_stream_t stream) {
  HRV_REQUIRE(x && y && N > 0 && H > 0 && W > 0 && H % 2 == 0 && W % 2 == 0 && C > 0 && C % 8 == 0, "maxpool_bf16: bad args");
  const size_t total = (size_t)N * (H / 2) * (W / 2) * (C / 4);
  hipLaunchKernelGGL(maxpool2_kernel<true>, dim3(grid_for(total)), dim3(256), 0, (hipStream_t)stream, (const float*)x, N, H / 2,
                     W / 2, C / 4, C, (float*)y, C);
  return check_launch("maxpool2_kernel[bf16]");
}

extern "C" int hrv_maxpool2x2_bwd_nhwc_f32(const float* x, const float* dy, int32_t N, int32_t H, int32_t W, int32_t C,
                                           float* dx, hrv_stream_t stream) {
  HRV_REQUIRE(x && dy && dx && N > 0 && H > 0 && W > 0 && H % 2 == 0 && W % 2 == 0 && C > 0 && C % 4 == 0, "maxpool_bwd: bad args");
  const size_t total = (size_t)N * (H / 2) * (W / 2) * (C / 4);
  hipLaunchKernelGGL(maxpool2_bwd_kernel<false>, dim3(grid_for(total)), dim3(256), 0, (hipStream_t)stream, x, dy, N, H / 2, W / 2,
                     C / 4, C, C, dx, 0);
  return check_launch("maxpool2_bwd_kernel");
}

extern "C" int hrv_maxpool2x2_bwd_relu_nhwc_f32(const float* x, const float* dy, int32_t N, int32_t H, int32_t W, int32_t C,
                                                float* dx, hrv_stream_t stream) {
  HRV_REQUIRE(x && dy && dx && N > 0 && H > 0 && W > 0 && H % 2 == 0 && W % 2 == 0 && C > 0 && C % 4 == 0, "maxpool_bwd_relu: bad args");
  const size_t total = (size_t)N * (H / 2) * (W / 2) * (C / 4);
  hipLaunchKernelGGL(maxpool2_bwd_kernel<false>, dim3(grid_for(total)), dim3(256), 0, (hipStream_t)stream, x, dy, N, H / 2, W / 2,
                     C / 4, C, C, dx, 1);
  return check_launch("maxpool2_bwd_kernel[relu]");
}

extern "C" int hrv_maxpool2x2_bwd_relu_nhwc_xbf16(const uint16_t* x, const float* dy, int32_t N, int32_t H, int32_t W, int32_t C,
                                                  float* dx, hrv_stream_t stream) {
  HRV_REQUIRE(x && dy && dx && N > 0 && H > 0 && W > 0 && H % 2 == 0 && W % 2 == 0 && C > 0 && C % 8 == 0, "maxpool_bwd_xbf16: bad args");
  const size_t total = (size_t)N * (H / 2) * (W / 2) * (C / 4);
  hipLaunchKernelGGL(maxpool2_bwd_kernel<true>, dim3(grid_for(total)), dim3(256), 0, (hipStream_t)stream, (const float*)x, dy, N,
                     H / 2, W / 2, C / 4, C, C, dx, 1);
  return check_launch("maxpool2_bwd_kernel[relu, bf16 x]");
}

extern "C" int hrv_maxpool2x2_bwd_relu_nhwc_bf16(const uint16_t* x, const uint16_t* dy, int32_t N, int32_t H, int32_t W, int32_t C,
                                                 uint16_t* dx, hrv_stream_t stream) {
  HRV_REQUIRE(x && dy && dx && N > 0 && H > 0 && W > 0 && H % 2 == 0 && W % 2 == 0 && C > 0 && C % 8 == 0, "maxpool_bwd_bf16: bad args");
  const size_t total = (size_t)N * (H / 2) * (W / 2) * (C / 4);
  hipLaunchKernelGGL((maxpool2_bwd_kernel<true, true>), dim3(grid_for(total)), dim3(256), 0, (hipStream_t)stream, (const float*)x,
                     (const float*)dy, N, H / 2, W / 2, C / 4, C, C, (float*)dx, 1);
  return check_launch("maxpool2_bwd_kernel[relu, bf16]");
}

extern "C" int hrv_add_slice_nhwc_bf16(const uint16_t* a, int32_t a_cstride, int32_t a_coff, uint16_t* out, int32_t out_cstride,
                                       int32_t out_coff, int32_t C, int64_t npix, int32_t accumulate, hrv_stream_t stream) {
  HRV_REQUIRE(a && out && npix > 0 && C > 0 && C % 4 == 0 && ((a_cstride | a_coff | out_cstride | out_coff) & 3) == 0,
              "add_slice_bf16: bad args");
  hipLaunchKernelGGL(add_slice_bf16_kernel, dim3(grid_for((size_t)npix * (C / 4))), dim3(256), 0, (hipStream_t)stream, a, a_cstride,
                     a_coff, out, out_cstride, out_coff, C / 4, (size_t)npix, accumulate);
  return check_launch("add_slice_bf16_kernel");
}

extern "C" int hrv_adam_f32(float* w, const float* g, float* m, float* v, int64_t n, float lr, float beta1, float beta2,
                            float eps, float weight_decay, int32_t step, float grad_scale, hrv_stream_t stream) {
  HRV_REQUIRE(w && g && m && v && n > 0 && step >= 1, "adam: bad args");
  const float bc1 = 1.f - powf(beta1, (float)step);
  const float bc2s = sqrtf(1.f - powf(beta2, (float)step));
  hipLaunchKernelGGL(adam_kernel, dim3(grid_for((size_t)n)), dim3(256), 0, (hipStream_t)stream, w, g, m, v, (size_t)n, lr,
                     beta1, beta2, eps, weight_decay, bc1, bc2s, grad_scale);
  return check_launch("adam_kernel");
}

extern "C" int hrv_adam_hyper_f32(int32_t* step_dev, const float* lr_dev, float beta1, float beta2, float* hyper_dev,
                                  hrv_stream_t stream) {
  HRV_REQUIRE(step_dev && lr_dev && hyper_dev, "adam_hyper: null pointer");
  hipLaunchKernelGGL(adam_hyper_kernel, dim3(1), dim3(64), 0, (hipStream_t)stream, step_dev, lr_dev, beta1, beta2, hyper_dev);
  return check_launch("adam_hyper_kernel");
}

extern "C" int hrv_adam_dev_f32(float* w, const float* g, float* m, float* v, int64_t n, const float* hyper_dev, float beta1,
                                float beta2, float eps, float weight_decay, float grad_scale, hrv_stream_t stream) {
  HRV_REQUIRE(w && g && m && v && hyper_dev && n > 0, "adam_dev: bad args");
  hipLaunchKernelGGL(adam_dev_kernel, dim3(grid_for((size_t)n)), dim3(256), 0, (hipStream_t)stream, w, g, m, v, (size_t)n, hyper_dev,
                     beta1, beta2, eps, weight_decay, grad_scale);
  return check_launch("adam_dev_kernel");
}

// ... 94 lines not shown
```

hr-viton_amd/gen_train.py:

```python
from __future__ import annotations

import os
from typing import Dict, List, Optional, Sequence, Tuple

import torch
import torch.nn as nn

from . import ops
from . import train_ops as T
from .ops import ACT_LRELU, ACT_NONE, ACT_RELU, ACT_TANH, Act, _ceil4

Grads = Dict[nn.Parameter, torch.Tensor]


def attach_grad_sync(sync):
    for p in sync.params:
        p._hrv_grad_sync = sync


def detach_grad_sync(params):
    for p in params:
        if hasattr(p, "_hrv_grad_sync"):
            del p._hrv_grad_sync

# ... 135 lines not shown
                out is not None or out_up != 0 or self._w2 is None):
            self._cache = None
            return super().forward(srcs, act, residual, out, out_up, slope, out_bf16)
        a2 = T.space_to_depth2(a)
        self._cache = (a.t.data_ptr(), a.coff, a2)
        b = self.bparam
        return T.conv_forward_dev(self.w2, [(a2, 0)], 1, 1, sigma=self.sigma, shift=None if b is None else b.data, act=act,
                                  slope=slope, name=self.name, out_bf16=out_bf16, batch=getattr(self, "pack_batch", None))

    def backward(self, dy: Act, srcs, grads: Grads, need_dx: bool = True, act_mask=None, slope: float = 0.2,
                 need_w: bool = True, dx_bf16: bool = False, dy_wgrad=None, add=None):
        a, _ = srcs[0]
        c = self._cache
        if c is None or c[0] != a.t.data_ptr() or c[1] != a.coff or act_mask is not None or add is not None:
            return super().backward(dy, srcs, grads, need_dx, act_mask, slope, need_w, dx_bf16, dy_wgrad, add)
        a2 = Act(c[2].t[:a.N], c[2].C)
        w = self.wparam.data
        Cout, cin = w.shape[0], w.shape[1]
        if need_w:
            dw2 = torch.empty_like(self._w2)
            db = grad_buffer(self.bparam) if self.bparam is not None else None
            T.conv_wgrad(dy, a2, 0, 0, 4 * self.Cq, 2, 2, 1, 1, dw2.view(Cout, 4 * self.Cq, 2, 2), name=self.name + ".wgrad",
                         dbias=db)
            G = dw2[:, :, :, :cin].permute(0, 3, 4, 1, 5, 2).reshape(Cout, cin, 4, 4)
            if self.spectral:
                dwo = grad_buffer(self.wparam)
                T.spectral_grad(G, w, self.u, self.v, self.sigma, dwo)
                _acc(grads, self.wparam, dwo)
            else:
                _acc(grads, self.wparam, G)
            if db is not None:
                _acc(grads, self.bparam, db)
        if not need_dx:
            return None
        d2 = T.conv_dgrad(dy, self.w2, a2.H, a2.W, 1, 1, sigma=self.sigma, name=self.name + ".dgrad",
                          batch=getattr(self, "pack_batch", None))
        return T.depth_to_space2(d2, a.C)


class SpadeT:

    def __init__(self, norm: nn.Module, act: int, name: str):
        self.norm, self.act, self.name = norm, act, name
        self.shared = TConv(norm.conv_shared[0], 1, 1, name + ".conv_shared")
        self.C = norm.conv_gamma.out_channels
        self.Cp = _ceil4(self.C)
        self.hid = norm.conv_gamma.in_channels
        G = (self.C + 31) // 32
        self.G = G
        self.cfg = 0 if G % 2 == 0 else 6
        dev = norm.conv_gamma.weight.device
        rows_g = torch.tensor([g * 64 + l for g in range(G) for l in range(32) if g * 32 + l < self.C], device=dev)
        self.rows_g, self.rows_b = rows_g, rows_g + 32

    def vecs(self):
        v = getattr(self, "_vec_pre", None)
        if v is not None:
            return v
        n = self.norm
        return T.spade_vec_prep(n.conv_gamma.bias.data, n.conv_beta.bias.data, n.noise_scale.data)

    def shared_as_1x1(self) -> Tuple[torch.Tensor, torch.Tensor, int]:
        w = self.shared.wparam.data
        co, c, kh, kw = w.shape
        return w.permute(0, 2, 3, 1), self.shared.bparam.data, c

    def forward(self, x: Act, actv: Optional[Act], z: Optional[torch.Tensor], save: bool = True, fused=None, stats=None):
        n = self.norm
        dev = x.t.device
        if fused is not None:
            sg, shift = fused
            zz = z
            if stats is not None:
                ns, (mean, rstd) = stats
            else:
                ns = self.vecs()[1] if zz is not None else None
                mean, rstd = ops.instnorm_stats(x, zz, ns if zz is not None else None)
            out = ops.alloc(x.N, x.H, x.W, self.C, dev, bf16=True)
            g1p = torch.empty((x.N, x.H, x.W, self.Cp), dtype=torch.bfloat16, device=dev) if save else None
            pk = T.spade_fused_pack(self.shared.wparam.data, self.shared.bparam.data, n.conv_gamma.weight.data, n.conv_beta.weight.data)
            T.spade_fused_forward(sg, shift, x, mean, rstd, zz, n.noise_scale.data, pk, n.conv_gamma.bias.data, n.conv_beta.bias.data,
                                  self.act, 0.2, out, g1p, actv if save else None, self.name + ".conv_shared+gamma|beta")
            ctx = dict(x=x, z=zz, ns=ns, mean=mean, rstd=rstd, actv=actv, g1p=Act(g1p, self.C) if save else None, out=out)
            return out, ctx
        bc, ns = self.vecs()
        zz = z
        if stats is not None:
            mean, rstd = stats[1]
        else:
            mean, rstd = ops.instnorm_stats(x, zz, ns if zz is not None else None)
        mb = T.MMA_BF16[0]
        cfg = ((8 if self.G % 2 == 0 else 9) if mb else self.cfg)
        if mb:
            cfg = ops.patch_tile(actv.bf16, 3, 3, 1, 1, 1, 0, self.hid, self.G * 64, x.N, x.H, x.W, wide=True) or cfg
        out_bf16 = mb and actv.bf16 and self.C % 8 == 0
        if (mb and actv.bf16 and out_bf16 and x.cstride % 4 == 0 and
                T.spade_gb_ok(0, self.C, self.Cp, self.hid, x.N, x.H, x.W)):
            out = ops.alloc(x.N, x.H, x.W, self.C, dev, bf16=True)
            g1p = torch.empty((x.N, x.H, x.W, self.Cp), dtype=torch.bfloat16, device=dev) if save else None
            pk = T.spade_gb_pack(0, n.conv_gamma.weight.data, n.conv_beta.weight.data)
            fl = 2.0 * x.N * x.H * x.W * 2 * self.C * self.hid * 9
            nbytes = (ops.act_bytes(actv) + (1.5 if save else 1) * ops.act_bytes(x) + ops.act_bytes(out) +
                      2.0 * self.C * self.hid * 9 * 2)
            T.spade_gb_forward(actv, x, mean, rstd, zz, n.noise_scale.data, pk, n.conv_gamma.bias.data, n.conv_beta.bias.data,
                               self.act, 0.2, out, g1p, self.name + ".conv_gamma|beta", fl, nbytes)
            ctx = dict(x=x, z=zz, ns=ns, mean=mean, rstd=rstd, actv=actv, g1p=Act(g1p, self.C) if save else None, out=out)
            return out, ctx
        packed, _, _ = T.pack_weight_pair_dev(n.conv_gamma.weight.data, n.conv_beta.weight.data, 1, [self.hid], [self.hid],
                                              cfg, 0, 1, mb, batch=getattr(self.shared, "pack_batch", None))
        out = ops.alloc(x.N, x.H, x.W, self.C, dev, bf16=mb and actv.bf16 and self.C % 8 == 0)
        g1p = torch.empty((x.N, x.H, x.W, self.Cp), dtype=torch.float32, device=dev) if save else None
        e = ops._lib.hrv_spade_epi_t()
        e.x, e.x_cstride, e.x_coff, e.C = x.t.data_ptr(), x.cstride, x.coff, self.Cp
        e.mean, e.rstd = mean.data_ptr(), rstd.data_ptr()
        if zz is not None:
            e.noise_z, e.noise_scale = zz.data_ptr(), ns.data_ptr()
        if save:
            e.g1p_out = g1p.data_ptr()
        import ctypes as C
        lib = ops._lib.load()
        d = ops._lib.hrv_conv2d_t()
        d.N, d.H, d.W, d.Ho, d.Wo = x.N, x.H, x.W, x.H, x.W
        d.KH, d.KW, d.stride, d.pad = 3, 3, 1, 1
        d.nsrc = 1
        s = d.src[0]
        s.ptr, s.C, s.cstride, s.coff, s.up_shift, s.pre_act, s.C_real = (actv.t.data_ptr(), self.hid, actv.cstride,
                                                                          actv.coff, 0, 0, self.hid)
        d.w_packed, d.Cout, d.tile_cfg = packed.data_ptr(), self.G * 64, cfg
        d.mixed_flags = ((7 if actv.bf16 else 15) & ~(1 if out.bf16 else 0)) if mb else 0
        d.shift = bc.data_ptr()
        d.act, d.act_slope = self.act, 0.2
        d.out, d.out_cstride, d.out_coff = out.t.data_ptr(), out.cstride, out.coff
        d.spade = C.pointer(e)
        fl = 2.0 * x.N * x.H * x.W * 2 * self.C * self.hid * 9
        nbytes = (ops.act_bytes(actv) + (2 if save else 1) * ops.act_bytes(x) + ops.act_bytes(out) +
                  2.0 * self.C * self.hid * 9 * (2 if mb else 4))
        with ops._Timed("conv", self.name + ".conv_gamma|beta", fl, nbytes, f"conv_mfma_kernel[tile {cfg}]"):
            fn = lib.hrv_conv2d_nhwc_bf16 if mb else lib.hrv_conv2d_nhwc_f32
            ops._lib.check(fn(C.byref(d), ops._stream()), "hrv_conv2d_nhwc_%s[spade]" % ("bf16" if mb else "f32"))
        ctx = dict(x=x, z=zz, ns=ns, mean=mean, rstd=rstd, actv=actv, g1p=Act(g1p, self.C) if save else None, out=out)
        return out, ctx

    def norm_args(self, ctx, dout: Act):
        n = self.norm
        dns = None
        if ctx["z"] is not None:
            dns = grad_buffer(n.noise_scale) if self.Cp == self.C else torch.empty(self.Cp, device=dout.t.device)
        return dict(mean=ctx["mean"], rstd=ctx["rstd"], dout=dout, act=self.act, slope=0.2,
                    out=ctx["out"] if self.act != ACT_NONE else None, g1p=ctx["g1p"], z=ctx["z"],
                    noise_scale=ctx["ns"] if ctx["z"] is not None else None, want_dgb=True, dnoise_scale=dns,
                    dgb_bf16=ctx["actv"].bf16)

    def dout_slot(self, ctx, want_bf16: bool):
        if (os.environ.get("HRV_DBETA_INPLACE", "1") == "0" or os.environ.get("HRV_NORM_BWD2", "0") != "0" or
                not T.MMA_BF16[0] or not want_bf16 or self.Cp != self.C or
                self.C % 8 != 0 or not ctx["actv"].bf16 or not ctx["out"].bf16):
            return None
        dgb, dbeta = T.norm_bwd_dgb(ctx["x"], True)
        return dgb, dbeta, (ctx["out"] if self.act != ACT_NONE else None)

    def backward(self, ctx, dout: Act, grads: Grads, dx: Optional[Act], dx_accumulate: bool, dact: Act,
                 dx_bf16: bool = False, dgb: Optional[Act] = None) -> Act:
        a = self.norm_args(ctx, dout)
        if dgb is not None:
            a.update(act=ACT_NONE, out=None, dgb=dgb)
        dx, dgb = T.norm_bwd(ctx["x"], dx=dx, dx_accumulate=dx_accumulate, dx_bf16=dx_bf16 and ctx["actv"].bf16, **a)
        self.after_norm(ctx, dgb, a["dnoise_scale"], grads, dact)
        return dx

    def after_norm(self, ctx, dgb: Act, dns: Optional[torch.Tensor], grads: Grads, dact: Act):
        n = self.norm
        C_, Cp = self.C, self.Cp
        dev = dgb.t.device
        if dns is not None:
            _acc(grads, n.noise_scale, dns[:C_])
        else:
            _acc(grads, n.noise_scale, torch.zeros(C_, device=dev))
        actv = ctx["actv"]
        if Cp == C_:
            wcat = (n.conv_gamma.weight.data, n.conv_beta.weight.data)
        else:
            wcat = torch.zeros((2 * Cp, self.hid, 3, 3), device=dev)
            wcat[:C_] = n.conv_gamma.weight.data
            wcat[Cp:Cp + C_] = n.conv_beta.weight.data
        with T.wgrad_side(dgb.N * dgb.H * dgb.W, dgb, actv):
            dwcat, db = _pair_slot(n.conv_gamma.weight, n.conv_beta.weight), _pair_slot(n.conv_gamma.bias, n.conv_beta.bias)
            if Cp != C_ or dwcat is None or db is None:
                dwcat = torch.empty((2 * Cp, self.hid, 3, 3), device=dev)
                db = torch.empty(2 * Cp, device=dev)
            T.conv_wgrad(dgb, actv, 0, 0, self.hid, 3, 3, 1, 1, dwcat, name=self.name + ".gb.wgrad", dbias=db)
            direct = flat_grad_slot(n.conv_gamma.weight) is not None
            keep = (lambda t: t) if direct else (lambda t: t.clone())
            _acc(grads, n.conv_gamma.weight, keep(dwcat[:C_]))
            _acc(grads, n.conv_beta.weight, keep(dwcat[Cp:Cp + C_]))
            _acc(grads, n.conv_gamma.bias, keep(db[:C_]))
            _acc(grads, n.conv_beta.bias, keep(db[Cp:Cp + C_]))
        if (Cp == C_ and T.MMA_BF16[0] and dgb.bf16 and actv.bf16 and dact.cstride % 8 == 0 and (2 * C_) % 32 == 0 and
                T.conv_p2_ok(2 * C_, self.hid, actv.N, actv.H, actv.W)):
            pk = T.conv_p2_pack(2, n.conv_gamma.weight.data, n.conv_beta.weight.data, 2 * C_, self.hid)
            T.conv_p2(dgb, pk, self.hid, dact, mask=actv, mask_slope=0.0, name=self.name + ".gb.dgrad",
                      flops=2.0 * actv.N * actv.H * actv.W * 2 * C_ * self.hid * 9, tag=" [spade_gb]")
        elif (Cp == C_ and T.MMA_BF16[0] and dgb.bf16 and actv.bf16 and
                T.spade_gb_ok(1, C_, Cp, self.hid, actv.N, actv.H, actv.W)):
            T.spade_gb_dgrad(dgb, T.spade_gb_pack(1, n.conv_gamma.weight.data, n.conv_beta.weight.data), C_, actv, 0.0, dact,
                             self.name + ".gb.dgrad")
        else:
            T.conv_dgrad(dgb, wcat, actv.H, actv.W, 1, 1, act_mask=actv, slope=0.0, out=dact, name=self.name + ".gb.dgrad",
                         batch=getattr(self.shared, "pack_batch", None) if Cp == C_ else None)


class BlockT:
    def __init__(self, blk: nn.Module, name: str):
        self.blk, self.name = blk, name
        self.learned = blk.learned_shortcut
        self.n0 = SpadeT(blk.norm_0, ACT_LRELU, name + ".norm_0")
        self.n1 = SpadeT(blk.norm_1, ACT_LRELU, name + ".norm_1")
        self.c0 = TConv(blk.conv_0, 1, 1, name + ".conv_0")
        self.c1 = TConv(blk.conv_1, 1, 1, name + ".conv_1")
        if self.learned:
            self.ns_ = SpadeT(blk.norm_s, ACT_NONE, name + ".norm_s")
            self.cs = TConv(blk.conv_s, 1, 0, name + ".conv_s")

    def convs(self):
        return [self.c0, self.c1] + ([self.cs] if self.learned else [])

    def wants_bf16_dout(self, ctx) -> bool:
        return bool(self.learned and ctx["h1"].bf16 and ctx["hs"].bf16 and self.c1.conv.out_channels % 8 == 0)

    def norms(self):
        return ([self.ns_] if self.learned else []) + [self.n0, self.n1]

    def _fused_ok(self, N: int, H: int, W: int, x_cstride: int, seg: Act, seg_shift: int) -> bool:
        if not (T.MMA_BF16[0] and seg.coff == 0 and seg.cstride == 8 and (seg.W >> seg_shift) % 4 == 0 and x_cstride % 4 == 0):
            return False
        return all(n_.C % 8 == 0 and n_.Cp == n_.C and n_.norm.conv_shared[0].weight.shape[1] <= 8 and
                   T.spade_fused_ok(n_.C, n_.hid, n_.norm.conv_shared[0].weight.shape[1], N, H, W) for n_ in self.norms())

    def fused_label_map(self, x: Act, seg: Act, seg_shift: int) -> Optional[Act]:
        if not self._fused_ok(x.N, x.H, x.W, x.cstride, seg, seg_shift):
            return None
        sg = seg if seg.bf16 else getattr(seg, "_as_bf16", None)
        if sg is None:
            sg = seg._as_bf16 = Act(seg.t.to(torch.bfloat16), seg.C)
        return sg

    def reads_upsampled_input(self, N: int, H: int, W: int, C_in: int, seg: Act, seg_shift: int) -> bool:
        if os.environ.get("HRV_XUP", "1") == "0" or os.environ.get("HRV_STATS2", "1") == "0" or not self.learned:
            return False
        if H % 2 or W % 2 or (C_in - 16) % 32 != 0 or self.n0.C != C_in or self.ns_.C != C_in:
            return False
        return self._fused_ok(N, H, W, 4, seg, seg_shift)

    def shared_forward(self, seg: Act, seg_shift: int):
        norms = self.norms()
        mb = T.MMA_BF16[0] and (seg.W >> seg_shift) % 4 == 0
        sg = seg
        if mb and seg.coff == 0 and seg.cstride == 8:
            sg = getattr(seg, "_as_bf16", None)
            if sg is None:
                sg = seg._as_bf16 = Act(seg.t.to(torch.bfloat16), seg.C)
        mb = mb and sg.bf16
        segx = ops.tap_expand(sg, seg_shift, 3)
        cp = sg.Cp
        wt_all, b_all = T.shared_taps_prep([n_.shared.wparam.data for n_ in norms], [n_.shared.bparam.data for n_ in norms], cp)
        hid = norms[0].hid
        actv_all = T.conv_forward_dev(wt_all, [(segx, 0)], 1, 0, shift=b_all, act=ACT_RELU,
                                      out_bf16=mb, name=self.name + ".conv_shared[x%d as 1x1 over taps]" % len(norms))
        return segx, [actv_all.slice(hid * i, hid) for i in range(len(norms))]

    def shared_backward(self, segx: Act, dact_all: Act, grads: Grads):
        norms = self.norms()
        hid, cp = norms[0].hid, segx.C // 9
        with T.wgrad_side(dact_all.N * dact_all.H * dact_all.W, dact_all, segx):
            dw = torch.empty((hid * len(norms), segx.C, 1, 1), device=dact_all.t.device)
            db = torch.empty(hid * len(norms), device=dact_all.t.device)
            T.conv_wgrad(dact_all, segx, 0, 0, segx.C, 1, 1, 1, 0, dw, name=self.name + ".conv_shared.wgrad", dbias=db)
            gws = [grad_buffer(n_.shared.wparam) for n_ in norms]
            gbs = [grad_buffer(n_.shared.bparam) for n_ in norms]
            T.shared_taps_grad(dw, db, gws, gbs, cp)
            for n_, gw, gb in zip(norms, gws, gbs):
                _acc(grads, n_.shared.wparam, gw)
                _acc(grads, n_.shared.bparam, gb)

    def forward(self, x: Act, seg: Act, seg_shift: int, zs, out: Optional[Act], out_up: int, out_act: int,
                save: bool = True):
        zi = iter(zs)
        ctx = {"x": x}
        sgf = self.fused_label_map(x, seg, seg_shift)
        fused = None
        if sgf is not None:
            fused = (sgf, seg_shift)
            norms = self.norms()
            hid = norms[0].hid
            segx, actvs = None, [None] * len(norms)
            if save:
                segx = ops.tap_expand(sgf, seg_shift, 3)
                actv_all = Act(torch.empty((x.N, x.H, x.W, hid * len(norms)), dtype=torch.bfloat16, device=x.t.device), hid * len(norms))
                actvs = [actv_all.slice(hid * i, hid) for i in range(len(norms))]
        else:
            segx, actvs = self.shared_forward(seg, seg_shift)
        ai = iter(actvs)
        ctx["segx"] = segx
        st_s = st_0 = None
        if self.learned:
            z_s, z_0 = next(zi), next(zi)
            if z_s is not None and z_0 is not None and not x.bf16 and os.environ.get("HRV_STATS2", "1") != "0":
                ns_s = self.ns_.vecs()[1]
                ns_0 = self.n0.vecs()[1]
                ms, m0 = ops.instnorm_stats2(x, z_s, ns_s, z_0, ns_0)
                st_s, st_0 = (ns_s, ms), (ns_0, m0)
            hs, ctx["ns"] = self.ns_.forward(x, next(ai), z_s, save, fused, st_s)
            x_s = self.cs.forward([(hs, 0)])
            ctx["hs"] = hs
        else:
            x_s = x
            z_0 = next(zi)
        h0, ctx["n0"] = self.n0.forward(x, next(ai), z_0, save, fused, st_0)
        dx = self.c0.forward([(h0, 0)])
        h1, ctx["n1"] = self.n1.forward(dx, next(ai), next(zi), save, fused)
        o = self.c1.forward([(h1, 0)], residual=x_s, act=out_act, out=out, out_up=out_up,
                            out_bf16=out is None and h1.bf16 and self.c1.conv.out_channels % 8 == 0)
        ctx.update(h0=h0, h1=h1)
        return o, ctx

    def backward(self, ctx, d_out: Act, grads: Grads) -> Act:
        x = ctx["x"]
        norms = self.norms()
        hid = norms[0].hid
        dact_all = ops.alloc(x.N, x.H, x.W, hid * len(norms), x.t.device,
                             bf16=bool(T.MMA_BF16[0] and ctx["segx"].bf16 and x.W % 4 == 0))
        k0 = 1 if self.learned else 0
        dh16 = bool(T.MMA_BF16[0] and os.environ.get("HRV_DH_BF16", "1") != "0")
        def down(conv, d_y, h, norm, nctx):
            slot = norm.dout_slot(nctx, dh16 and h.bf16)
            if slot is None:
                return conv.backward(d_y, [(h, 0)], grads, dx_bf16=dh16 and h.bf16), None
            dgb, dbeta, mask = slot
            conv.backward(d_y, [(h, 0)], grads, act_mask=mask, slope=0.2, dx_out=dbeta)
            return dbeta, dgb
        d_h1, dgb1 = down(self.c1, d_out, ctx["h1"], self.n1, ctx["n1"])
        d_dx = self.n1.backward(ctx["n1"], d_h1, grads, None, False, dact_all.slice(hid * (k0 + 1), hid), dx_bf16=True, dgb=dgb1)
        d_h0, dgb0 = down(self.c0, d_dx, ctx["h0"], self.n0, ctx["n0"])
        if (self.learned and ctx["n0"]["z"] is not None and ctx["ns"]["z"] is not None and not x.bf16 and
                os.environ.get("HRV_NORM_BWD2", "0") != "0"):
            d_hs = self.cs.backward(d_out, [(ctx["hs"], 0)], grads, dx_bf16=dh16 and ctx["hs"].bf16)
            a0, as_ = self.n0.norm_args(ctx["n0"], d_h0), self.ns_.norm_args(ctx["ns"], d_hs)
            d_x, dgb0, dgbs = T.norm_bwd2(x, a0, as_)
            self.n0.after_norm(ctx["n0"], dgb0, a0["dnoise_scale"], grads, dact_all.slice(hid * k0, hid))
            self.ns_.after_norm(ctx["ns"], dgbs, as_["dnoise_scale"], grads, dact_all.slice(0, hid))
            self.shared_backward(ctx["segx"], dact_all, grads)
            return d_x
        d_x = self.n0.backward(ctx["n0"], d_h0, grads, None, False, dact_all.slice(hid * k0, hid), dgb=dgb0)
        if self.learned:
            d_hs, dgbs = down(self.cs, d_out, ctx["hs"], self.ns_, ctx["ns"])
            self.ns_.backward(ctx["ns"], d_hs, grads, d_x, True, dact_all.slice(0, hid), dgb=dgbs)
        else:
            T.add_slice(d_out, d_x, True)
        self.shared_backward(ctx["segx"], dact_all, grads)
        return d_x


def noise_elems(gen: nn.Module, N: int) -> int:
    return sum((3 if getattr(gen, name).learned_shortcut else 2) * ((N * (gen.sw << j) * (gen.sh << j) + 3) // 4 * 4)
               for j, name in enumerate(gen._blocks()))


def noise_planes(gen: nn.Module, N: int, zall: torch.Tensor):
    out, off = {}, 0
    for j, name in enumerate(gen._blocks()):
        h, w = gen.sh << j, gen.sw << j
        zn = N * w * h
        planes = []
        for _ in range(3 if getattr(gen, name).learned_shortcut else 2):
            planes.append(zall[off:off + zn].view(N, w, h, 1))
            off += (zn + 3) // 4 * 4
        out[name] = planes
    return out


class GeneratorTrainPlan:
    def __init__(self, gen: nn.Module):
        self.gen = gen
        names = gen._blocks()
        self.names = names
        self.blocks = [BlockT(getattr(gen, n), n) for n in names]
        self.stems = [TConv(getattr(gen, f"conv_{i}"), 1, 1, f"conv_{i}") for i in range(len(names))]
        self.img = TConv(gen.conv_img, 1, 1, "conv_img")

    def forward(self, x: torch.Tensor, seg, noise, power_iteration: bool, save: bool = True):
        gen = self.gen
        N, _, H, W = x.shape
        nb = len(self.names)
        top = nb - 1
        dev = x.device
        T.prepare_convs(self, [c for b in self.blocks for c in b.convs()] + list(self.stems) + [self.img] +
                        [n_.shared for b in self.blocks for n_ in b.norms()], power_iteration, backward=save,
                        extra_weights=[w_ for b in self.blocks for n_ in b.norms()
                                       for w_ in (n_.norm.conv_gamma.weight.data, n_.norm.conv_beta.weight.data)])
        norms_all = [n_ for b in self.blocks for n_ in b.norms()]
        if os.environ.get("HRV_VEC_PREP_MULTI", "1") != "0":
            pre = T.spade_vec_prep_multi([(n_.norm.conv_gamma.bias.data, n_.norm.conv_beta.bias.data, n_.norm.noise_scale.data) for n_ in norms_all])
            for n_, v in zip(norms_all, pre):
                n_._vec_pre = v
        try:
            return self._forward(x, seg, noise, save)
        finally:
            for n_ in norms_all:
                n_._vec_pre = None

    def _forward(self, x: torch.Tensor, seg, noise, save: bool):
        gen = self.gen
        N, _, H, W = x.shape
        nb = len(self.names)
        top = nb - 1
        dev = x.device
        xin = ops.to_nhwc(x)
        xin_top = ops.to_nhwc(x, bf16=True) if (T.MMA_BF16[0] and W % 4 == 0) else xin
        sg = seg if isinstance(seg, Act) else ops.to_nhwc(seg)
        ctxs = []
        stem_in = []
        cur = None
        if noise is None:
            noise = noise_planes(gen, N, torch.randn(noise_elems(gen, N), device=dev))
        for j, name in enumerate(self.names):
            blk = self.blocks[j]
            h, w = gen.sh << j, gen.sw << j
            shift = top - j
            cin = getattr(gen, name).input_nc
            xs, xsh = (xin_top, 0) if shift == 0 else (xin, -shift)
            if (0 < shift <= 2 and xin_top.bf16 and N * h * w >= 65536 and w % 4 == 0 and os.environ.get("HRV_STEM_DOWN", "1") != "0"):
                f = 1 << shift
                xs, xsh = Act(xin_top.t[:, ::f, ::f, :].contiguous(), xin_top.C), 0
            stem_in.append((xs, xsh))
            if j == 0:
                cur = self.stems[0].forward([(xs, xsh)])
            elif isinstance(cur, ops.ActUp):
                self.stems[j].forward([(xs, xsh)], out=cur.hi)
            else:
                self.stems[j].forward([(xs, xsh)], out=cur.slice(cin - 16, 16))
            k = 3 if blk.learned else 2
            zs = [z.to(dev).contiguous() for z in noise[name]]
            assert len(zs) == k, (name, len(zs), k)
            if j == nb - 1:
                o, c = blk.forward(cur, sg, shift, zs, None, 0, ACT_LRELU, save)
            else:
                nxt_c = getattr(gen, self.names[j + 1]).input_nc
                if self.blocks[j + 1].reads_upsampled_input(N, h * 2, w * 2, nxt_c, sg, shift - 1):
                    lo = ops.alloc(N, h, w, nxt_c - 16, dev)
                    _, c = blk.forward(cur, sg, shift, zs, lo, 0, ACT_NONE, save)
                    o = ops.ActUp(lo, ops.alloc(N, h * 2, w * 2, 16, dev))
                else:
                    nxt = ops.alloc(N, h * 2, w * 2, nxt_c, dev)
                    o, c = blk.forward(cur, sg, shift, zs, nxt.slice(0, nxt_c - 16), 1, ACT_NONE, save)
                    o = nxt
            c["shift"] = shift
            ctxs.append(c)
            cur = o
        img = self.img.forward([(cur, 0)], act=ACT_TANH)
        return ops.to_nchw(img), dict(blocks=ctxs, last=cur, img=img, stem_in=stem_in)

    def backward(self, ctx, d_img: torch.Tensor) -> Grads:
        grads: Grads = {}
        gen = self.gen
        img: Act = ctx["img"]
        dimg = ops.to_nhwc(d_img.contiguous())
        dpre = Act(T.tanh_bwd(dimg.t, img.t), 3)
        dpre8 = None
        if ctx["last"].bf16:
            t8 = torch.zeros(dpre.t.shape[:3] + (8,), dtype=torch.bfloat16, device=dpre.t.device)
            t8[..., :4].copy_(dpre.t)
            dpre8 = Act(t8, 3)
        d_cur = self.img.backward(dpre if dpre8 is None else dpre8, [(ctx["last"], 0)], grads, act_mask=ctx["last"],
                                  slope=0.2, dx_bf16=self.blocks[-1].wants_bf16_dout(ctx["blocks"][-1]))
        for j in range(len(self.names) - 1, -1, -1):
            blk, c = self.blocks[j], ctx["blocks"][j]
            d_x = blk.backward(c, d_cur, grads)
            cin = getattr(gen, self.names[j]).input_nc
            xin, xsh = ctx["stem_in"][j]
            if j == 0:
                self.stems[0].backward(d_x, [(xin, xsh)], grads, need_dx=False)
            else:
                d_stem = d_x.slice(cin - 16, 16)
                d_stem_w = None
                if xin.bf16 and xsh == 0 and not d_stem.bf16:
                    d_stem_w = Act(d_stem.t[..., d_stem.coff:d_stem.coff + 16].to(torch.bfloat16), 16)
                self.stems[j].backward(d_stem, [(xin, xsh)], grads, need_dx=False, dy_wgrad=d_stem_w)
                d_cur = T.downsum2x2(d_x.slice(0, cin - 16), out_bf16=self.blocks[j - 1].wants_bf16_dout(ctx["blocks"][j - 1]))
        return grads


class _GenFn(torch.autograd.Function):
    @staticmethod
    def forward(ctx, gen, plan, x, seg, noise, *params):
        out, saved = plan.forward(x, seg, noise, power_iteration=True)
        ctx.plan, ctx.saved, ctx.params = plan, saved, params
        return out

    @staticmethod
    def backward(ctx, d_out):
        grads = ctx.plan.backward(ctx.saved, d_out)
        ctx.saved = None
        T.wgrad_join()
        return (None, None, None, None, None) + tuple(grads.get(p) for p in ctx.params)


def generator_train_forward(gen: nn.Module, x: torch.Tensor, seg, noise=None) -> torch.Tensor:
    ops.require_cuda(x, "SPADEGenerator.forward(x)")
# ... 560 lines not shown
```

hr-viton_amd/train_ops.py:

```python
from __future__ import annotations

import ctypes as C
import itertools
import os
from typing import Optional, Sequence, Tuple

import torch

from . import _lib, ops
from .ops import ACT_LRELU, ACT_NONE, ACT_RELU, Act, _ceil4, _stream, _Timed, _workspace


MMA_BF16 = [False]


def _bf16_tile(cout: int) -> int:
    p64, p128 = (cout + 63) // 64 * 64, (cout + 127) // 128 * 128
    return 8 if p128 <= p64 else 9


_FROZEN_PACKS: dict = {}


def evict_serving_packs(tokens):
# ... 567 lines not shown
            _thin_ok(dy, KH, KW, 1, pad, cin, N, H, W)):
        return _thin_conv(dy, w, 1, sigma, wscale, None, act_mask, res_mode, ACT_NONE, slope, out, name, fl)
    if p2:
        pk = (conv_p2_pack(2, pair[0], pair[1], Cout, cin) if pair is not None else
              conv_p2_pack(1, w, None, Cout, cin, sigma, wscale, frozen))
        return conv_p2(dy, pk, cin, out, mask=act_mask if res_mode == 1 else None, mask_slope=slope, name=name, flops=fl,
                       residual=add_after, res_after_mask=add_after is not None, variant="mode 2" if pair is not None else "mode 1")
    if stride == 1:
        if mb and (Ho, Wo) == (H, W):
            cfg = ops.patch_tile(dy.bf16, KH, KW, 1, KH - 1 - pad, 1, 0, dy.Cp, cin, N, H, W) or cfg
        if pair is not None:
            packed, g, _ = pack_weight_pair_dev(pair[0], pair[1], 2, [_ceil4(cin)], [cin], cfg, 1, pad, mb, batch=batch)
        else:
            packed, g = pack_weight_dev(w, [_ceil4(cin)], [cin], cfg, 1, 1, pad, wscale=wscale, sigma=sigma, bf16=mb,
                                        frozen=frozen, batch=batch)
        _run_engine([(dy, 0, Cout)], packed, cin, cfg, N, Ho, Wo, H, W, g[0], g[1], 1, g[2], g[3], out,
                    residual=act_mask, res_mode=res_mode, slope=slope, name=name, flops=fl, mma_bf16=mb)
        return out
    assert stride == 2, "data gradient implemented for stride 1 and 2"
    for a in range(2):
        for b in range(2):
            Hp, Wp = (H - a + 1) // 2, (W - b + 1) // 2
            if Hp <= 0 or Wp <= 0:
                continue
            cfg_p = _bf16_tile(cin) if mb else _f32_tile(N * Hp * Wp, cin)
            packed, g = pack_weight_dev(w, [_ceil4(cin)], [cin], cfg_p, 2, 2, pad, (a, b), wscale, sigma, bf16=mb, batch=batch)
            _run_engine([(dy, 0, Cout)], packed, cin, cfg_p, N, Ho, Wo, Hp, Wp, g[0], g[1], 1, g[2], g[3], out,
                        residual=act_mask, res_mode=res_mode, slope=slope, free_extent=1, out_step=2, out_off=(a, b),
                        out_hw=(H, W), name=f"{name}[phase {a}{b}]", flops=fl / 4, mma_bf16=mb)
    return out


def conv_wgrad(dy: Act, x: Act, x_up: int, ci_base: int, cin_tot: int, KH: int, KW: int, stride: int, pad: int,
               dw: torch.Tensor, accumulate: bool = False, name: str = "wgrad", dbias: Optional[torch.Tensor] = None,
               dbias_accumulate: bool = False):
    lib = _lib.load()
    N, Ho, Wo, Cout = dy.N, dy.H, dy.W, dy.C
    H, W = (x.H << x_up, x.W << x_up) if x_up >= 0 else (x.H >> -x_up, x.W >> -x_up)
    assert dw.is_contiguous() and tuple(dw.shape) == (Cout, cin_tot, KH, KW), (dw.shape, Cout, cin_tot, KH, KW)
    if (Cout == 1 and x_up == 0 and ci_base == 0 and cin_tot == x.C and not dy.bf16 and
            (Ho, Wo) == (H + 2 * pad - KH + 1, W + 2 * pad - KW + 1) and _cout1_ok(dw, x, stride, pad, "wgrad")):
        S = lib.hrv_conv_cout1_wgrad_slabs(N, Ho, Wo)
        ws = _workspace(dy.t.device, 4 * S * (x.C * KH * KW + 1))
        d = _cout1_desc(dw, x, pad, 1.0, None, dy)
        d.workspace = ws.data_ptr()
        with _Timed("wgrad", name, 2.0 * N * Ho * Wo * x.C * KH * KW, ops.act_bytes(x) + 4.0 * N * Ho * Wo, "cout1_kernel"):
            _lib.check(lib.hrv_conv_cout1_wgrad_f32(C.byref(d), dw.data_ptr(), 1 if accumulate else 0,
                                                    None if dbias is None else dbias.data_ptr(), 1 if dbias_accumulate else 0,
                                                    _stream()), f"hrv_conv_cout1_wgrad_f32[{name}]")
        return
    wo_real = Wo
    served = ""
    if MMA_BF16[0] and dy.bf16 and x.bf16 and x_up == 0:
        if stride == 1 and (Ho, Wo) == (H, W):
            c = lib.hrv_conv2d_wgrad_tr_supported(Cout, x.Cp, x.cstride, x.coff, dy.cstride, dy.coff, N, H, W, KH, KW, pad)
            if c > 0:
                served = f"conv_wgrad_tr_kernel[class {c - 1}]"
        elif (KH, KW, stride, pad) == (4, 4, 2, 2) and (Ho, Wo) == (H // 2 + 1, W // 2 + 1):
            c = lib.hrv_conv2d_wgrad_s2_supported(Cout, x.Cp, x.cstride, x.coff, dy.cstride, dy.coff, N, H, W)
            if c > 0:
                served = "conv_wgrad_s2_kernel"
    if MMA_BF16[0] and Wo % 4 != 0 and dy.bf16 and x.bf16 and dy.coff == 0 and dy.cstride == dy.C and dy.C % 8 == 0 and not served:
        dy = pad_width_bf16(dy)
        Wo = dy.W
    if (MMA_BF16[0] and Wo % 4 != 0 and Wo >= 32 and not (x.bf16 or dy.bf16) and dy.coff == 0 and dy.cstride == dy.Cp):
        with _Timed("layout", "pad_width", 0.0, 2.0 * ops.act_bytes(dy)):
            dy = Act(torch.nn.functional.pad(dy.t, (0, 0, 0, (-Wo) % 4)), dy.C)
        Wo = dy.W
    need = lib.hrv_conv2d_wgrad_workspace_bytes(Cout, cin_tot, KH, KW, N * Ho * Wo)
    ws = _workspace(dy.t.device, need)
    fl = 2.0 * N * Ho * wo_real * Cout * x.C * KH * KW
    fn = lib.hrv_conv2d_wgrad_bf16mma_nhwc_f32 if (MMA_BF16[0] and Wo % 4 == 0) else lib.hrv_conv2d_wgrad_nhwc_f32
    args = (dy.t.data_ptr(), dy.cstride, dy.coff, Cout, x.t.data_ptr(), x.Cp, x.cstride, x.coff, x_up, x.C, ci_base,
            cin_tot, N, H, W, Ho, Wo, KH, KW, stride, pad, ws.data_ptr(), ws.numel() * 4, dw.data_ptr(),
            1 if accumulate else 0, None if dbias is None else dbias.data_ptr(), 1 if dbias_accumulate else 0)
    nbytes = ops.act_bytes(dy) + ops.act_bytes(x) + 4.0 * Cout * x.C * KH * KW
    if served:
        kern, _, var = served.partition("[")
        var = var.rstrip("]")
    elif x.bf16 or dy.bf16:
        kern, var = "conv_wgrad_kernel", "bf16 stored" if dy.bf16 else "bf16 x-stored"
    else:
        kern, var = "conv_wgrad_kernel", "bf16" if fn is lib.hrv_conv2d_wgrad_bf16mma_nhwc_f32 else "fp32"
    with _Timed("wgrad", name, fl, nbytes, kern, var):
        if x.bf16 or dy.bf16:
            assert MMA_BF16[0] and (Wo % 4 == 0 or served), f"{name}: bf16-stored operands need the bf16 matrix-core weight gradient"
            assert x.bf16, f"{name}: bf16 dY with an fp32 X is not built"
            _lib.check(lib.hrv_conv2d_wgrad_bf16mma_st_nhwc_f32(*args, (1 if dy.bf16 else 0) | 2, _stream()),
                       "hrv_conv2d_wgrad_bf16mma_st_nhwc_f32")
        else:
            _lib.check(fn(*args, _stream()), "hrv_conv2d_wgrad_bf16mma_nhwc_f32" if fn is lib.hrv_conv2d_wgrad_bf16mma_nhwc_f32
                       else "hrv_conv2d_wgrad_nhwc_f32")


def colsum(a: Act, out: Optional[torch.Tensor] = None, accumulate: bool = False) -> torch.Tensor:
    lib = _lib.load()
    if out is None:
        out = torch.empty(a.C, dtype=torch.float32, device=a.t.device)
        accumulate = False
    P = a.N * a.H * a.W
    ws = _workspace(a.t.device, 256 * a.Cp * 4)
    _lib.check(lib.hrv_colsum_nhwc_f32(a.t.data_ptr(), P, a.C, a.cstride, a.coff, ws.data_ptr(), ws.numel() * 4,
                                       out.data_ptr(), 1 if accumulate else 0, _stream()), "hrv_colsum_nhwc_f32")
    return out


def _norm_bwd_desc(x, mean, rstd, dout, act, slope, out, g1p, z, noise_scale, want_dgb, dx, dx_accumulate, dnoise_scale, dns_accumulate,
                   dgb_bf16, dx_bf16, dgb=None):
    lib = _lib.load()
    N, H, W, Cp = x.N, x.H, x.W, x.Cp
    dev = x.t.device
    if dx is None:
        dx = ops.alloc(N, H, W, x.C, dev, bf16=dx_bf16 and x.C % 8 == 0)
        dx_accumulate = False
    dnh = torch.empty((N, H, W, Cp), dtype=torch.bfloat16 if MMA_BF16[0] else torch.float32, device=dev)
    if dgb is None:
        dgb = Act(torch.empty((N, H, W, 2 * Cp), dtype=torch.bfloat16 if dgb_bf16 else torch.float32, device=dev),
                  2 * Cp) if want_dgb else None
    ws = torch.empty(lib.hrv_norm_bwd_workspace_elems(N, H, W, Cp), dtype=torch.float32, device=dev)
    d = _lib.hrv_norm_bwd_t()
    d.N, d.H, d.W, d.C = N, H, W, Cp
    if isinstance(x, ops.ActUp):
        d.x, d.x_cstride, d.x_coff = x.lo.t.data_ptr(), x.lo.cstride, x.lo.coff
        d.x_up_channels, d.x2, d.x2_cstride, d.x2_coff = x.lo.C, x.hi.t.data_ptr(), x.hi.cstride, x.hi.coff
    else:
        d.x, d.x_cstride, d.x_coff = x.t.data_ptr(), x.cstride, x.coff
    if z is not None:
        d.noise_z, d.noise_scale = z.data_ptr(), noise_scale.data_ptr()
    d.mean, d.rstd = mean.data_ptr(), rstd.data_ptr()
    if out is not None:
        d.out, d.out_cstride, d.out_coff = out.t.data_ptr(), out.cstride, out.coff
        d.out_bf16 = 1 if out.bf16 else 0
    if g1p is not None:
        d.g1p, d.g1p_cstride, d.g1p_coff = g1p.t.data_ptr(), g1p.cstride, g1p.coff
        d.g1p_bf16 = 1 if g1p.bf16 else 0
    d.dout, d.dout_cstride, d.dout_coff = dout.t.data_ptr(), dout.cstride, dout.coff
    d.dout_bf16 = 1 if dout.bf16 else 0
    d.dnh, d.dnh_cstride, d.dnh_coff = dnh.data_ptr(), Cp, 0
    d.dnh_bf16 = 1 if dnh.dtype == torch.bfloat16 else 0
    if dgb is not None:
        d.dgb, d.dgb_cstride, d.dgb_coff = dgb.t.data_ptr(), dgb.cstride, dgb.coff
        d.dgb_bf16 = 1 if dgb.bf16 else 0
    d.dx, d.dx_cstride, d.dx_coff = dx.t.data_ptr(), dx.cstride, dx.coff
    d.dx_accumulate = 1 if dx_accumulate else 0
    d.dx_bf16 = 1 if dx.bf16 else 0
    assert not (dx.bf16 and dx_accumulate)
    d.act, d.act_slope = act, slope
    d.dns_accumulate = 1 if dns_accumulate else 0
    d.dnoise_scale = None if dnoise_scale is None else dnoise_scale.data_ptr()
    d.workspace = ws.data_ptr()
    return d, dx, dgb, (dnh, ws)


def norm_bwd(x: Act, mean: torch.Tensor, rstd: torch.Tensor, dout: Act, act: int = ACT_NONE, slope: float = 0.2,
             out: Optional[Act] = None, g1p: Optional[Act] = None, z: Optional[torch.Tensor] = None,
             noise_scale: Optional[torch.Tensor] = None, want_dgb: bool = False, dx: Optional[Act] = None,
             dx_accumulate: bool = False, dnoise_scale: Optional[torch.Tensor] = None, dns_accumulate: bool = False,
             dgb_bf16: bool = False, dx_bf16: bool = False, dgb: Optional[Act] = None):
    lib = _lib.load()
    d, dx, dgb, _keep = _norm_bwd_desc(x, mean, rstd, dout, act, slope, out, g1p, z, noise_scale, want_dgb, dx, dx_accumulate, dnoise_scale,
                                       dns_accumulate, dgb_bf16, dx_bf16, dgb)
    with _Timed("norm_bwd", "spade_norm_bwd", 0.0, 4.0 * x.N * x.H * x.W * x.Cp * (7 + (2 if want_dgb else 0))):
        _lib.check(lib.hrv_spade_norm_bwd_nhwc_f32(C.byref(d), _stream()), "hrv_spade_norm_bwd_nhwc_f32")
    return dx, dgb


def norm_bwd_dgb(x: Act, bf16: bool) -> Tuple[Act, Act]:
    dgb = Act(torch.empty((x.N, x.H, x.W, 2 * x.Cp), dtype=torch.bfloat16 if bf16 else torch.float32, device=x.t.device), 2 * x.Cp)
    return dgb, dgb.slice(x.Cp, x.C)


def norm_bwd2(x: Act, a: dict, b: dict):
    lib = _lib.load()
    da, dx, dgb_a, _ka = _norm_bwd_desc(x, a["mean"], a["rstd"], a["dout"], a.get("act", ACT_NONE), a.get("slope", 0.2), a.get("out"), a.get("g1p"),
                                        a.get("z"), a.get("noise_scale"), a.get("want_dgb", False), None, False, a.get("dnoise_scale"),
                                        a.get("dns_accumulate", False), a.get("dgb_bf16", False), False)
    db, _, dgb_b, _kb = _norm_bwd_desc(x, b["mean"], b["rstd"], b["dout"], b.get("act", ACT_NONE), b.get("slope", 0.2), b.get("out"), b.get("g1p"),
                                       b.get("z"), b.get("noise_scale"), b.get("want_dgb", False), dx, False, b.get("dnoise_scale"),
                                       b.get("dns_accumulate", False), b.get("dgb_bf16", False), False)
    with _Timed("norm_bwd", "spade_norm_bwd x2", 0.0, 4.0 * x.N * x.H * x.W * x.Cp * (10 + 2 * (a.get("want_dgb", False) + b.get("want_dgb", False)))):
        _lib.check(lib.hrv_spade_norm_bwd2_nhwc_f32(C.byref(da), C.byref(db), _stream()), "hrv_spade_norm_bwd2_nhwc_f32")
    return dx, dgb_a, dgb_b


LOSS_L1, LOSS_HINGE_D_FAKE, LOSS_HINGE_D_REAL, LOSS_NEG_MEAN, LOSS_MSE = 0, 1, 2, 3, 4
LOSS_RELU_MASK = 16


def loss(a: torch.Tensor, b: Optional[torch.Tensor], mode: int, lscale: float, gscale: float, loss_out: torch.Tensor,
         accumulate: bool = True, want_grad: bool = True, grad_bf16: bool = False) -> Optional[torch.Tensor]:
    lib = _lib.load()
    cl = torch.channels_last
    bf = a.dtype == torch.bfloat16
    assert b is None or b.dtype == a.dtype, "loss: both operands share one storage type"
    ok = a.is_contiguous() and (b is None or (b.shape == a.shape and b.is_contiguous()))
    ok = ok or (a.dim() == 4 and a.is_contiguous(memory_format=cl) and
                (b is None or (b.shape == a.shape and b.is_contiguous(memory_format=cl))))
    assert ok, "loss: operands must share one dense layout (strides of size-1 dims do not matter)"
    grad_bf16 = bool(grad_bf16 and bf and a.numel() % 4 == 0)
    grad = torch.empty_like(a, dtype=torch.bfloat16 if grad_bf16 else torch.float32) if want_grad else None
    if grad_bf16:
        mode |= 32
    ws = _workspace(a.device, 4096)
    fn = lib.hrv_loss_bf16in_f32 if bf else lib.hrv_loss_f32
    with _Timed("loss", "loss_f32", 0.0, (2.0 if bf else 4.0) * a.numel() * (1 + (b is not None)) + 4.0 * a.numel() * (grad is not None)):
        _lib.check(fn(a.data_ptr(), None if b is None else b.data_ptr(), a.numel(), mode, lscale, gscale,
                      None if grad is None else grad.data_ptr(), ws.data_ptr(), loss_out.data_ptr(),
                      1 if accumulate else 0, _stream()), "hrv_loss_f32")
    return grad


def downsum2x2(dhi: Act, dlo: Optional[Act] = None, accumulate: bool = False, out_bf16: bool = False) -> Act:
    lib = _lib.load()
    Hl, Wl = dhi.H // 2, dhi.W // 2
    if dlo is None:
        dlo = ops.alloc(dhi.N, Hl, Wl, dhi.C, dhi.t.device, bf16=out_bf16 and dhi.C % 8 == 0)
        accumulate = False
    assert not (dlo.bf16 and accumulate)
    with _Timed("ew", "downsum2x2", 0.0, ops.act_bytes(dhi) * (1.25 + (0.25 if accumulate else 0))):
        _lib.check(lib.hrv_downsum2x2_nhwc_f32(dhi.t.data_ptr(), dhi.N, Hl, Wl, dhi.Cp, dhi.cstride, dhi.coff,
                                               dlo.t.data_ptr(), dlo.cstride, dlo.coff,
                                               2 if dlo.bf16 else (1 if accumulate else 0), _stream()),
                   "hrv_downsum2x2_nhwc_f32")
    return dlo


def avgpool3x3s2_bwd(dy: Act, H: int, W: int, dx: Optional[Act] = None, accumulate: bool = False) -> Act:
    lib = _lib.load()
    if dx is None:
        dx = ops.alloc(dy.N, H, W, dy.C, dy.t.device)
        accumulate = False
    with _Timed("pool", "avgpool3x3s2_bwd", 0.0, ops.act_bytes(dy) + ops.act_bytes(dx) * (2 if accumulate else 1)):
        _lib.check(lib.hrv_avgpool3x3s2_bwd_nhwc_f32(dy.t.data_ptr(), dy.N, H, W, dy.Cp, dy.cstride, dy.coff,
                                                     dx.t.data_ptr(), dx.cstride, dx.coff, 1 if accumulate else 0,
                                                     _stream()), "hrv_avgpool3x3s2_bwd_nhwc_f32")
    return dx


def maxpool2x2(x: Act) -> Act:
    lib = _lib.load()
    assert x.coff == 0 and x.cstride == x.Cp
    y = ops.alloc(x.N, x.H // 2, x.W // 2, x.C, x.t.device, bf16=x.bf16)
    fn = lib.hrv_maxpool2x2_nhwc_bf16 if x.bf16 else lib.hrv_maxpool2x2_nhwc_f32
    with _Timed("pool", "maxpool2x2", 0.0, ops.act_bytes(x) * 1.25):
        _lib.check(fn(x.t.data_ptr(), x.N, x.H, x.W, x.Cp, y.t.data_ptr(), _stream()), "hrv_maxpool2x2_nhwc")
    return y


def maxpool2x2_bwd(x: Act, dy: Act, relu: bool = False) -> Act:
    lib = _lib.load()
    dx = ops.alloc(x.N, x.H, x.W, x.C, x.t.device, bf16=dy.bf16)
    assert (relu or not x.bf16) and (not dy.bf16 or (x.bf16 and relu)), \
        "maxpool2x2_bwd: a bf16-stored x needs relu=True; bf16 gradients need a bf16 x"
    if dy.bf16:
        fn = lib.hrv_maxpool2x2_bwd_relu_nhwc_bf16
    else:
        fn = (lib.hrv_maxpool2x2_bwd_relu_nhwc_xbf16 if x.bf16 else lib.hrv_maxpool2x2_bwd_relu_nhwc_f32) if relu \
            else lib.hrv_maxpool2x2_bwd_nhwc_f32
    with _Timed("pool", "maxpool2x2_bwd", 0.0, ops.act_bytes(x) + 5.0 * x.N * x.H * x.W * x.C):
        _lib.check(fn(x.t.data_ptr(), dy.t.data_ptr(), x.N, x.H, x.W, x.Cp, dx.t.data_ptr(), _stream()),
                   "hrv_maxpool2x2_bwd_nhwc_f32")
    return dx


def adam_step(w: torch.Tensor, g: torch.Tensor, m: torch.Tensor, v: torch.Tensor, lr: float, beta1: float, beta2: float,
              eps: float, weight_decay: float, step: int, grad_scale: float = 1.0):
    lib = _lib.load()
    with _Timed("adam", "adam_f32", 0.0, 28.0 * w.numel()):
        _lib.check(lib.hrv_adam_f32(w.data_ptr(), g.data_ptr(), m.data_ptr(), v.data_ptr(), w.numel(), lr, beta1, beta2, eps,
                                    weight_decay, step, grad_scale, _stream()), "hrv_adam_f32")


def adam_step_dev(w: torch.Tensor, g: torch.Tensor, m: torch.Tensor, v: torch.Tensor, step_dev: torch.Tensor, lr_dev: torch.Tensor,
                  hyper: torch.Tensor, beta1: float, beta2: float, eps: float, weight_decay: float, grad_scale: float = 1.0):
    lib = _lib.load()
    _lib.check(lib.hrv_adam_hyper_f32(step_dev.data_ptr(), lr_dev.data_ptr(), beta1, beta2, hyper.data_ptr(), _stream()),
               "hrv_adam_hyper_f32")
    with _Timed("adam", "adam_f32", 0.0, 28.0 * w.numel()):
        _lib.check(lib.hrv_adam_dev_f32(w.data_ptr(), g.data_ptr(), m.data_ptr(), v.data_ptr(), w.numel(), hyper.data_ptr(), beta1,
                                        beta2, eps, weight_decay, grad_scale, _stream()), "hrv_adam_dev_f32")


def spectral_sigma(w_orig: torch.Tensor, u: torch.Tensor, v: torch.Tensor, power_iterations: int,
                   eps: float = 1e-12) -> torch.Tensor:
    lib = _lib.load()
    R = w_orig.shape[0]
    K = w_orig.numel() // R
    scratch = torch.empty(R, dtype=torch.float32, device=w_orig.device)
    sigma = torch.empty(1, dtype=torch.float32, device=w_orig.device)
    _lib.check(lib.hrv_spectral_norm_f32(w_orig.data_ptr(), R, K, u.data_ptr(), v.data_ptr(), power_iterations, eps,
                                         scratch.data_ptr(), sigma.data_ptr(), _stream()), "hrv_spectral_norm_f32")
    return sigma


class SpectralBatch:

    def __init__(self, items):
        self.items = list(items)
        self.Rs = [w.shape[0] for w, _, _ in self.items]
        self.Ks = [w.numel() // w.shape[0] for w, _, _ in self.items]
        self.jobs = (_lib.hrv_sn_job_t * len(self.items))()
        for j, (R, K) in enumerate(zip(self.Rs, self.Ks)):
            self.jobs[j].R, self.jobs[j].K = R, K

    def run(self, power_iterations: int, eps: float = 1e-12):
        lib = _lib.load()
        dev = self.items[0][0].device
        n, sR, sK = len(self.items), sum(self.Rs), sum(self.Ks)
        sig = getattr(self, "_sig", None)
        if sig is None or sig.device != dev or sig.numel() != n:
            sig = self._sig = torch.empty(n, dtype=torch.float32, device=dev)
        ub = torch.empty(sR, dtype=torch.float32, device=dev)
        vb = torch.empty(sK, dtype=torch.float32, device=dev)
        scratch = _workspace(dev, 4 * sR)
        sp, up, vp = sig.data_ptr(), ub.data_ptr(), vb.data_ptr()
        ro = ko = 0
        for j, (w, u, v) in enumerate(self.items):
            J = self.jobs[j]
            J.w, J.u, J.v = w.data_ptr(), u.data_ptr(), v.data_ptr()
            J.sigma, J.u_keep, J.v_keep = sp + 4 * j, up + 4 * ro, vp + 4 * ko
            ro, ko = ro + self.Rs[j], ko + self.Ks[j]
        _lib.check(lib.hrv_spectral_norm_batched_f32(self.jobs, n, power_iterations, eps, scratch.data_ptr(), _stream()),
                   "hrv_spectral_norm_batched_f32")
        return sig.split(1), ub.split(self.Rs), vb.split(self.Ks)


def prepare_convs(owner, convs, power_iteration: bool, backward: bool = True, extra_weights: Sequence[torch.Tensor] = ()):
    _prepare_sigmas(owner, convs, power_iteration)
    if not convs:
        return
    dev = convs[0].wparam.data.device
    pb = getattr(owner, "_pack_batch", None)
    if pb is None or pb.device != dev:
        pb = owner._pack_batch = PackBatch(dev)
    for c in convs:
# ... 518 lines not shown
```

include/hrviton_hip.h:

```cpp
#ifndef HRVITON_HIP_H
#define HRVITON_HIP_H

#include <stddef.h>
#include <stdint.h>

#ifdef __cplusplus
extern "C" {
#endif

typedef void* hrv_stream_t;

enum hrv_status {
  HRV_OK = 0,
  HRV_ERR_ARG = -1,
  HRV_ERR_LAUNCH = -2,
  HRV_ERR_NODEV = -3
};

enum hrv_act { HRV_ACT_NONE = 0, HRV_ACT_RELU = 1, HRV_ACT_LRELU = 2, HRV_ACT_TANH = 3 };

const char* hrv_version(void);
const char* hrv_last_error(void);
int hrv_device_check(void);
int hrv_set_reserved_cus(int32_t k);
int hrv_persistent_cus(void);
int hrv_diag_set_tlog(void* buf, int64_t tiles);
int hrv_diag_reload_env(void);

#define HRV_MAX_SRC 4

typedef struct hrv_src {
  const void* ptr;
  int32_t C;
  int32_t cstride;
  int32_t coff;
  int32_t up_shift;
  int32_t pre_act;
  int32_t C_real;
} hrv_src_t;

typedef struct hrv_spade_epi {
  const float* x;
  int32_t x_cstride, x_coff;
  int32_t C;
  int32_t _pad;
  const float* mean;
  const float* rstd;
  const float* noise_z;
  const float* noise_scale;
  float* g1p_out;
} hrv_spade_epi_t;

typedef struct hrv_conv2d {
  int32_t N, H, W;
  int32_t Ho, Wo;
  int32_t KH, KW, stride, pad;
  int32_t nsrc;
  hrv_src_t src[HRV_MAX_SRC];
  const void* w_packed;
  const float* w_oihw;
  int32_t Cout;
  int32_t tile_cfg;
  const float* scale;
  const float* shift;
  const void* residual;
  int32_t res_cstride, res_coff;
  int32_t act;
  float act_slope;
  void* out;
  int32_t out_cstride, out_coff;
  const hrv_spade_epi_t* spade;
  int32_t out_up_shift;
  int32_t _pad2;
  void* workspace;
  int64_t workspace_bytes;
  int32_t pad_w_plus1;
  int32_t free_extent;
  int32_t out_step;
  int32_t out_off_h, out_off_w, out_H, out_W;
  int32_t res_mode;
  int32_t mixed_flags;
  int32_t _pad3;
} hrv_conv2d_t;

int hrv_conv2d_pick_tile(int64_t M, int32_t Cout);
int hrv_conv2d_tile_bn(int32_t tile_cfg);
int hrv_conv2d_tile_bm(int32_t tile_cfg);
int hrv_conv2d_tile_row_bytes(int32_t tile_cfg);
int64_t hrv_conv2d_packed_elems(int32_t Cout, int32_t KH, int32_t KW, int32_t nsrc,
                                const int32_t* srcC, int32_t tile_cfg);
int hrv_conv2d_pack_weight_f32(const float* w_oihw, int32_t Cout, int32_t KH, int32_t KW, int32_t nsrc,
                               const int32_t* srcC, const int32_t* srcC_real, int32_t tile_cfg,
                               float* out);
int hrv_conv2d_pack_weight_dev_f32(const float* w_oihw_dev, int32_t Cout, int32_t KH, int32_t KW, int32_t nsrc,
                                   const int32_t* srcC, const int32_t* srcC_real, int32_t tile_cfg, int32_t mode,
                                   int32_t stride, int32_t pad, int32_t phase_a, int32_t phase_b, float wscale,
                                   const float* sigma_dev, float* out_dev, int32_t* out_geom, hrv_stream_t stream);
int hrv_conv2d_pack_weight_dev_bf16(const float* w_oihw_dev, int32_t Cout, int32_t KH, int32_t KW, int32_t nsrc,
                                    const int32_t* srcC, const int32_t* srcC_real, int32_t tile_cfg, int32_t mode,
                                    int32_t stride, int32_t pad, int32_t phase_a, int32_t phase_b, float wscale,
                                    const float* sigma_dev, uint16_t* out_dev, int32_t* out_geom, hrv_stream_t stream);
int hrv_conv2d_pack_weight_pair_dev(const float* w_a_dev, const float* w_b_dev, int32_t rows_each, int32_t pair_mode,
                                    int32_t Cout, int32_t KH, int32_t KW, int32_t nsrc, const int32_t* srcC,
                                    const int32_t* srcC_real, int32_t tile_cfg, int32_t mode, int32_t pad, int32_t as_bf16,
                                    void* out_dev, int32_t* out_geom, hrv_stream_t stream);
int32_t hrv_conv2d_pack_record_bytes(void);
int hrv_conv2d_pack_weight_record(const float* w_oihw_dev, int32_t Cout, int32_t KH, int32_t KW, int32_t nsrc,
                                  const int32_t* srcC, const int32_t* srcC_real, int32_t tile_cfg, int32_t mode,
                                  int32_t stride, int32_t pad, int32_t phase_a, int32_t phase_b, float wscale,
                                  const float* sigma_dev, int32_t as_bf16, const float* w2_dev, int32_t pair_mode,
                                  int32_t rows_each, void* out_dev, int32_t* out_geom, void* record_host, int32_t* blocks);
int hrv_conv2d_pack_weight_multi(const void* records_dev, const int32_t* first_block_dev, int32_t n, int32_t blocks,
                                 hrv_stream_t stream);
int64_t hrv_conv2d_wgrad_workspace_bytes(int32_t Cout, int32_t CinTot, int32_t KH, int32_t KW, int64_t P);
int hrv_conv2d_wgrad_nhwc_f32(const float* dy, int32_t dy_cstride, int32_t dy_coff, int32_t Cout, const float* x,
                              int32_t x_C, int32_t x_cstride, int32_t x_coff, int32_t x_up_shift, int32_t x_C_real,
                              int32_t ci_base, int32_t CinTot, int32_t N, int32_t H, int32_t W, int32_t Ho, int32_t Wo,
                              int32_t KH, int32_t KW, int32_t stride, int32_t pad, float* workspace,
                              int64_t workspace_bytes, float* dw_oihw, int32_t accumulate, float* dbias,
                              int32_t dbias_accumulate, hrv_stream_t stream);
int hrv_conv2d_wgrad_bf16mma_nhwc_f32(const float* dy, int32_t dy_cstride, int32_t dy_coff, int32_t Cout, const float* x,
                              int32_t x_C, int32_t x_cstride, int32_t x_coff, int32_t x_up_shift, int32_t x_C_real,
                              int32_t ci_base, int32_t CinTot, int32_t N, int32_t H, int32_t W, int32_t Ho, int32_t Wo,
                              int32_t KH, int32_t KW, int32_t stride, int32_t pad, float* workspace,
                              int64_t workspace_bytes, float* dw_oihw, int32_t accumulate, float* dbias,
                              int32_t dbias_accumulate, hrv_stream_t stream);
int hrv_conv2d_wgrad_bf16mma_st_nhwc_f32(const void* dy, int32_t dy_cstride, int32_t dy_coff, int32_t Cout,
                              const void* x, int32_t x_C, int32_t x_cstride, int32_t x_coff, int32_t x_up_shift,
                              int32_t x_C_real, int32_t ci_base, int32_t CinTot, int32_t N, int32_t H, int32_t W,
                              int32_t Ho, int32_t Wo, int32_t KH, int32_t KW, int32_t stride, int32_t pad,
                              float* workspace, int64_t workspace_bytes, float* dw_oihw, int32_t accumulate,
                              float* dbias, int32_t dbias_accumulate, int32_t storage_flags, hrv_stream_t stream);
int hrv_colsum_nhwc_f32(const float* x, int64_t P, int32_t C, int32_t cstride, int32_t coff, float* workspace,
                        int64_t workspace_bytes, float* out, int32_t accumulate, hrv_stream_t stream);

typedef struct hrv_norm_bwd {
  int32_t N, H, W, C;
  const float* x;     int32_t x_cstride, x_coff;
  const float* noise_z; const float* noise_scale;
  const float* mean;  const float* rstd;
  const float* out;   int32_t out_cstride, out_coff;
  const float* g1p;   int32_t g1p_cstride, g1p_coff;
  const float* dout;  int32_t dout_cstride, dout_coff;
  float* dnh;         int32_t dnh_cstride, dnh_coff;
  float* dgb;         int32_t dgb_cstride, dgb_coff;
  float* dx;          int32_t dx_cstride, dx_coff;
  int32_t dx_accumulate;
  int32_t act;        float act_slope;
  int32_t dns_accumulate;
  float* dnoise_scale;
  float* workspace;
  int32_t dgb_bf16;
  int32_t out_bf16;
  int32_t dx_bf16;
  int32_t g1p_bf16;
  int32_t dnh_bf16;
  int32_t dout_bf16;
  int32_t x_up_channels;
  const float* x2;    int32_t x2_cstride, x2_coff;
} hrv_norm_bwd_t;
int64_t hrv_norm_bwd_workspace_elems(int32_t N, int32_t H, int32_t W, int32_t C);

typedef struct {
  const void* src; int32_t N, H, W, src_channels, src_cstride, src_coff;
  const float* w_oihw; int32_t Cout, Cin, KH, KW; const float* sigma; float wscale;
  int32_t mode;
  const float* shift;
  const void* residual; int32_t res_cstride, res_coff, res_bf16, res_mode;
  int32_t act; float act_slope;
  void* out; int32_t out_cstride, out_coff, out_bf16;
} hrv_thin_conv_t;
int hrv_thin_conv_supported(int32_t KH, int32_t KW, int32_t src_channels, int32_t out_columns);
int hrv_thin_conv_bf16(const hrv_thin_conv_t* d, hrv_stream_t stream);
int hrv_spade_norm_bwd_nhwc_f32(const hrv_norm_bwd_t* d, hrv_stream_t stream);
int hrv_spade_norm_bwd2_nhwc_f32(const hrv_norm_bwd_t* a, const hrv_norm_bwd_t* b, hrv_stream_t stream);
int hrv_loss_f32(const float* a, const float* b, int64_t n, int32_t mode, float lscale, float gscale, float* grad,
                 float* workspace, float* loss_out, int32_t accumulate, hrv_stream_t stream);
int hrv_loss_bf16in_f32(const uint16_t* a, const uint16_t* b, int64_t n, int32_t mode, float lscale, float gscale, float* grad,
                        float* workspace, float* loss_out, int32_t accumulate, hrv_stream_t stream);
int hrv_scale_f32(float* x, int64_t n, float s_host, const float* s_dev, hrv_stream_t stream);
int hrv_act_bwd_nhwc_f32(float* d, int32_t d_cstride, int32_t d_coff, const float* y, int32_t y_cstride, int32_t y_coff,
                         int32_t C, int64_t npix, int32_t act, float act_slope, hrv_stream_t stream);
int hrv_tanh_bwd_f32(const float* dy, const float* y, int64_t n, float* out, hrv_stream_t stream);
int hrv_add_slice_nhwc_f32(const float* a, int32_t a_cstride, int32_t a_coff, float* out, int32_t out_cstride,
                           int32_t out_coff, int32_t C, int64_t npix, int32_t accumulate, hrv_stream_t stream);
int hrv_downsum2x2_nhwc_f32(const float* dhi, int32_t N, int32_t Hl, int32_t Wl, int32_t C, int32_t hi_cstride,
                            int32_t hi_coff, float* dlo, int32_t lo_cstride, int32_t lo_coff, int32_t accumulate,
                            hrv_stream_t stream);
int hrv_avgpool3x3s2_bwd_nhwc_f32(const float* dy, int32_t N, int32_t H, int32_t W, int32_t C, int32_t dy_cstride,
                                  int32_t dy_coff, float* dx, int32_t dx_cstride, int32_t dx_coff, int32_t accumulate,
                                  hrv_stream_t stream);
int hrv_maxpool2x2_nhwc_f32(const float* x, int32_t N, int32_t H, int32_t W, int32_t C, float* y, hrv_stream_t stream);
int hrv_maxpool2x2_bwd_nhwc_f32(const float* x, const float* dy, int32_t N, int32_t H, int32_t W, int32_t C, float* dx,
                                hrv_stream_t stream);
int hrv_maxpool2x2_bwd_relu_nhwc_f32(const float* x, const float* dy, int32_t N, int32_t H, int32_t W, int32_t C, float* dx,
                                     hrv_stream_t stream);
int hrv_maxpool2x2_nhwc_bf16(const uint16_t* x, int32_t N, int32_t H, int32_t W, int32_t C, uint16_t* y, hrv_stream_t stream);
int hrv_maxpool2x2_bwd_relu_nhwc_bf16(const uint16_t* x, const uint16_t* dy, int32_t N, int32_t H, int32_t W, int32_t C,
                                      uint16_t* dx, hrv_stream_t stream);
int hrv_add_slice_nhwc_bf16(const uint16_t* a, int32_t a_cstride, int32_t a_coff, uint16_t* out, int32_t out_cstride,
                            int32_t out_coff, int32_t C, int64_t npix, int32_t accumulate, hrv_stream_t stream);
int hrv_maxpool2x2_bwd_relu_nhwc_xbf16(const uint16_t* x, const float* dy, int32_t N, int32_t H, int32_t W, int32_t C,
                                       float* dx, hrv_stream_t stream);
int hrv_adam_f32(float* w, const float* g, float* m, float* v, int64_t n, float lr, float beta1, float beta2, float eps,
                 float weight_decay, int32_t step, float grad_scale, hrv_stream_t stream);
int hrv_adam_hyper_f32(int32_t* step_dev, const float* lr_dev, float beta1, float beta2, float* hyper_dev, hrv_stream_t stream);
int hrv_adam_dev_f32(float* w, const float* g, float* m, float* v, int64_t n, const float* hyper_dev, float beta1, float beta2,
                     float eps, float weight_decay, float grad_scale, hrv_stream_t stream);
int hrv_spectral_norm_f32(const float* w, int32_t R, int32_t K, float* u, float* v, int32_t power_iterations, float eps,
                          float* wv_scratch, float* sigma_out, hrv_stream_t stream);
int hrv_spectral_norm_bwd_f32(const float* G, const float* w_orig, const float* u, const float* v, const float* sigma,
                              int32_t R, int32_t K, float* workspace, float* dw_orig, int32_t accumulate,
                              hrv_stream_t stream);
int hrv_spade_vec_prep_f32(const float* gamma_bias, const float* beta_bias, const float* noise_scale, int32_t C,
                           float* bias_interleaved, float* noise_scale_padded, hrv_stream_t stream);
int hrv_spade_vec_prep_multi_f32(int32_t n, const float* const* gamma_bias, const float* const* beta_bias, const float* const* noise_scale,
                                 const int32_t* C, const int32_t* off_bias, const int32_t* off_noise, float* bias_interleaved_all,
                                 float* noise_scale_padded_all, hrv_stream_t stream);
int hrv_shared_taps_prep_f32(const float* const* w, const float* const* b, int32_t n, int32_t hid, int32_t c, int32_t cp,
                             float* wt, float* bt, hrv_stream_t stream);
int hrv_shared_taps_grad_f32(const float* dw, const float* db, int32_t n, int32_t hid, int32_t c, int32_t cp,
                             float* const* gw, float* const* gb, hrv_stream_t stream);
typedef struct {
  const float* w;
  float *u, *v;
  float* sigma;
  float *u_keep, *v_keep;
  int32_t R, K;
} hrv_sn_job_t;
int hrv_spectral_norm_batched_f32(const hrv_sn_job_t* jobs, int32_t n_jobs, int32_t power_iterations, float eps,
                                  float* wv_scratch, hrv_stream_t stream);

int64_t hrv_conv2d_workspace_bytes(const hrv_conv2d_t* d);
int hrv_conv2d_nhwc_f32(const hrv_conv2d_t* d, hrv_stream_t stream);
int64_t hrv_conv2d_packed_elems_bf16(int32_t Cout, int32_t KH, int32_t KW, int32_t nsrc, const int32_t* srcC,
                                     int32_t tile_cfg);
int hrv_conv2d_pack_weight_bf16(const float* w_oihw, int32_t Cout, int32_t KH, int32_t KW, int32_t nsrc,
                                const int32_t* srcC, const int32_t* srcC_real, int32_t tile_cfg, uint16_t* out);
int hrv_conv2d_nhwc_bf16(const hrv_conv2d_t* d, hrv_stream_t stream);
int hrv_conv2d_naive_nhwc_f32(const hrv_conv2d_t* d, hrv_stream_t stream);

int hrv_tapsum_nhwc_f32(const float* y, int32_t N, int32_t H, int32_t W, int32_t KH, int32_t KW, int32_t pad,
                        int32_t Cout, int32_t y_cstride, const float* bias, const float* residual,
                        int32_t res_cstride, float* out, int32_t out_cstride, hrv_stream_t stream);

int64_t hrv_instnorm_workspace_elems(int32_t N, int32_t H, int32_t W, int32_t C);
int hrv_instnorm_stats_nhwc_f32(const float* x, int32_t N, int32_t H, int32_t W, int32_t C, int32_t cstride,
                                int32_t coff, const float* noise_z, const float* noise_scale, float eps,
                                float* workspace, float* mean, float* rstd, hrv_stream_t stream);
int hrv_instnorm_stats2_nhwc_f32(const float* x, int32_t N, int32_t H, int32_t W, int32_t C, int32_t cstride, int32_t coff,
                                 const float* z_a, const float* ns_a, const float* z_b, const float* ns_b, float eps, float* workspace,
                                 float* mean_a, float* rstd_a, float* mean_b, float* rstd_b, hrv_stream_t stream);
int hrv_instnorm_stats2_up_nhwc_f32(const float* lo, int32_t lo_cstride, int32_t lo_coff, int32_t up_channels, const float* hi,
                                    int32_t hi_cstride, int32_t hi_coff, int32_t N, int32_t H, int32_t W, int32_t C, const float* z_a,
                                    const float* ns_a, const float* z_b, const float* ns_b, float eps, float* workspace, float* mean_a,
                                    float* rstd_a, float* mean_b, float* rstd_b, hrv_stream_t stream);
int hrv_instnorm_stats_nhwc_bf16(const uint16_t* x, int32_t N, int32_t H, int32_t W, int32_t C, int32_t cstride,
                                 int32_t coff, const float* noise_z, const float* noise_scale, float eps,
                                 float* workspace, float* mean, float* rstd, hrv_stream_t stream);
int hrv_instnorm_apply_nhwc_f32(const float* x, int32_t N, int32_t H, int32_t W, int32_t C, int32_t cstride,
                                int32_t coff, const float* mean, const float* rstd, int32_t act, float act_slope,
                                float* out, int32_t out_cstride, int32_t out_coff, hrv_stream_t stream);
int hrv_avgpool3x3s2_nhwc_f32(const float* x, int32_t N, int32_t H, int32_t W, int32_t C, int32_t cstride,
                              int32_t coff, float* out, int32_t out_cstride, int32_t out_coff,
                              hrv_stream_t stream);

int hrv_mul_channel_nhwc_f32(float* x, int32_t x_cstride, int32_t ch, const float* m, int32_t m_cstride,
                             int32_t m_ch, int32_t binarize, int64_t npix, hrv_stream_t stream);
int hrv_gauss_blur_nhwc_f32(const float* in, int32_t N, int32_t H, int32_t W, int32_t C, int32_t cstride,
                            const float* taps_host, int32_t ksize, float* tmp, float* out, hrv_stream_t stream);
int hrv_parse_argmax_nhwc_f32(const float* g, int32_t cstride, int32_t nclass, int64_t npix, int64_t* labels,
                              float* parse7, int32_t parse_cstride, hrv_stream_t stream);
int hrv_resize_nchw_f32(const float* in, int32_t planes, int32_t H, int32_t W, int32_t Ho, int32_t Wo,
                        int32_t nearest, float* out, hrv_stream_t stream);
int hrv_occlusion_nhwc_f32(const float* g, int32_t g_cstride, int32_t nclass, float* cloth, int32_t cloth_cstride,
                           float* cm, int32_t cm_cstride, int32_t cm_ch, int64_t npix, hrv_stream_t stream);

int hrv_nchw_to_nhwc_f32(const float* in, int32_t N, int32_t C, int32_t H, int32_t W, float* out,
                         int32_t out_cstride, int32_t out_coff, int32_t zero_tail, hrv_stream_t stream);
int hrv_nhwc_to_nchw_f32(const float* in, int32_t in_cstride, int32_t in_coff, int32_t N, int32_t C,
                         int32_t H, int32_t W, float* out, hrv_stream_t stream);
int hrv_space_to_depth2_nhwc_f32(const float* in, int32_t N, int32_t H, int32_t W, int32_t C, int32_t in_cstride,
                                 int32_t in_coff, float* out, hrv_stream_t stream);
typedef struct {
  const float* x; int32_t N, H, W, C, x_cstride, x_coff;
  const float* w_oihw;
  const float* sigma; float wscale;
  const float* bias;
  int32_t K, pad;
  float* y; int32_t y_cstride, y_coff;
  float* dx; int32_t dx_cstride, dx_coff;
  const float* add; int32_t add_cstride, add_coff;
  float* workspace;
  int32_t round_bf16;
} hrv_conv_cout1_t;
int hrv_conv_cout1_fwd_f32(const hrv_conv_cout1_t* d, hrv_stream_t stream);
int hrv_conv_cout1_dgrad_f32(const hrv_conv_cout1_t* d, hrv_stream_t stream);
int32_t hrv_conv_cout1_wgrad_slabs(int32_t N, int32_t Ho, int32_t Wo);
int hrv_conv_cout1_wgrad_f32(const hrv_conv_cout1_t* d, float* dw, int32_t accumulate, float* dbias, int32_t dbias_accumulate,
                             hrv_stream_t stream);
int hrv_concat_nhwc_nchw_f32(const float* a, int32_t Ca, int32_t a_cstride, int32_t a_coff, const float* b, int32_t Cb, int32_t N,
                             int32_t H, int32_t W, float* out, int32_t out_cstride, hrv_stream_t stream);
int hrv_depth_to_space2_nhwc_f32(const float* in, int32_t N, int32_t H, int32_t W, int32_t C, float* out, hrv_stream_t stream);
int hrv_nchw_f32_to_nhwc_bf16(const float* in, int32_t N, int32_t C, int32_t H, int32_t W, uint16_t* out,
                              int32_t out_cstride, int32_t out_coff, int32_t zero_tail, hrv_stream_t stream);
int hrv_nhwc_bf16_to_nchw_f32(const uint16_t* in, int32_t in_cstride, int32_t in_coff, int32_t N, int32_t C,
                              int32_t H, int32_t W, float* out, hrv_stream_t stream);

int hrv_resize_bilinear_nhwc_f32(const float* in, int32_t N, int32_t H, int32_t W, int32_t C,
                                 int32_t in_cstride, int32_t in_coff, int32_t Ho, int32_t Wo, float rh,
                                 float rw, const float* addend, int32_t add_cstride, int32_t add_coff,
                                 float* out, int32_t out_cstride, int32_t out_coff, hrv_stream_t stream);

typedef struct hrv_flow_warp {
  const float* src;
  int32_t N, H, W, C;
  int32_t src_cstride, src_coff;
  const float* flow;
  int32_t fh, fw;
  int32_t Ho, Wo;
  float rh, rw;
  float norm_x, norm_y;
  float* out;
  int32_t out_cstride, out_coff;
  float* flow_up;
} hrv_flow_warp_t;
int hrv_flow_warp_nhwc_f32(const hrv_flow_warp_t* d, hrv_stream_t stream);

// ... 179 lines not shown
```

Baseline: 60.00 images/s.

## Specialize SPADE norm backward kernels by flags and enable paired norm_bwd2 by default

Templates the SPADE norm backward stage1/stage2 kernels (single and paired) on a compile-time flag word so common configurations get specialized instances with no runtime branching on bf16, activation, noise, upsample or accumulate options. The paired norm_bwd2 path, previously opt-in through an environment variable, now runs by default whenever a supported-check says it is faster, and it now composes with the in-place dbeta/dgb slots. Byte accounting for timing is refined. The cost is more kernel instances (binary size, compile time) and small numeric differences from explicit FMA use.

```diff
diff --git a/hr-viton_amd/_lib.py b/hr-viton_amd/_lib.py
--- a/hr-viton_amd/_lib.py
+++ b/hr-viton_amd/_lib.py
@@ -164,6 +164,8 @@
     "hrv_persistent_cus": (C.c_int, []),
     "hrv_diag_set_tlog": (C.c_int, [_vp, _i64]),
     "hrv_diag_reload_env": (C.c_int, []),
+    "hrv_diag_norm_bwd_instances": (C.c_char_p, []),
+    "hrv_diag_norm_bwd_route": (C.c_int, [C.POINTER(hrv_norm_bwd_t), C.POINTER(hrv_norm_bwd_t)]),
     "hrv_conv2d_pick_tile": (C.c_int, [_i64, _i32]),
     "hrv_conv2d_tile_bn": (C.c_int, [_i32]),
     "hrv_conv2d_tile_bm": (C.c_int, [_i32]),
@@ -191,6 +193,7 @@
     "hrv_colsum_nhwc_f32": (C.c_int, [_vp, _i64, _i32, _i32, _i32, _vp, _i64, _vp, _i32, _vp]),
     "hrv_norm_bwd_workspace_elems": (_i64, [_i32, _i32, _i32, _i32]),
     "hrv_spade_norm_bwd2_nhwc_f32": (C.c_int, [C.POINTER(hrv_norm_bwd_t), C.POINTER(hrv_norm_bwd_t), _vp]),
+    "hrv_spade_norm_bwd2_supported": (C.c_int, [C.POINTER(hrv_norm_bwd_t), C.POINTER(hrv_norm_bwd_t)]),
     "hrv_spade_norm_bwd_nhwc_f32": (C.c_int, [C.POINTER(hrv_norm_bwd_t), _vp]),
     "hrv_thin_conv_supported": (C.c_int, [_i32, _i32, _i32, _i32]),
     "hrv_thin_conv_bf16": (C.c_int, [C.POINTER(hrv_thin_conv_t), _vp]),
diff --git a/hr-viton_amd/csrc/train.hip b/hr-viton_amd/csrc/train.hip
--- a/hr-viton_amd/csrc/train.hip
+++ b/hr-viton_amd/csrc/train.hip
@@ -1,4 +1,6 @@
 #include <string.h>
+
+#include <string>
 
 #include "hrv_common.h"
 
@@ -27,11 +29,13 @@
   const float* base;
   int cs, lo, W, Wl;
 };
+template <int UP = -1>
 __device__ __forceinline__ XThread xsrc_thread(const XSrc& s, int n, int g) {
   XThread t;
+  const bool up = UP < 0 ? s.up_g > 0 : UP != 0;
   t.W = s.W; t.Wl = s.W >> 1;
-  t.lo = (s.up_g > 0 && g < s.up_g) ? 1 : 0;
-  if (s.up_g > 0 && !t.lo) {
+  t.lo = (up && g < s.up_g) ? 1 : 0;
+  if (up && !t.lo) {
     t.cs = s.x2_cs;
     t.base = s.x2 + (size_t)n * s.H * s.W * s.x2_cs + s.x2_co + (g - s.up_g) * 4;
   } else {
@@ -67,6 +71,7 @@
   int dbeta_in_place;
 };
 
+__device__ __forceinline__ f32x4 fma4(f32x4 a, f32x4 b, f32x4 c) { return __builtin_elementwise_fma(a, b, c); }
 __device__ __forceinline__ f32x4 ld4(const float* p) { return *reinterpret_cast<const f32x4*>(p); }
 __device__ __forceinline__ f32x4 ld4_bf16(const void* base, size_t elem) {
   const uint2 u = *reinterpret_cast<const uint2*>(reinterpret_cast<const unsigned short*>(base) + elem);
@@ -80,7 +85,23 @@
   *reinterpret_cast<bf16x4t*>(reinterpret_cast<unsigned short*>(base) + elem) = __builtin_convertvector(v, bf16x4t);
 }
 
-__global__ __launch_bounds__(256) void norm_bwd_stage1_kernel(const NormBwdParams p) {
+
+enum : int {
+  NF_DOUT_BF16 = 1 << 0, NF_ACT_SHIFT = 1, NF_ACT_MASK = 3 << NF_ACT_SHIFT , NF_OUT_BF16 = 1 << 3,
+  NF_G1P = 1 << 4, NF_G1P_BF16 = 1 << 5, NF_DNH_BF16 = 1 << 6, NF_DGB = 1 << 7, NF_DGB_BF16 = 1 << 8, NF_DBETA_IN_PLACE = 1 << 9,
+  NF_NOISE = 1 << 10, NF_UP = 1 << 11, NF_DX_BF16 = 1 << 12, NF_DX_ACC = 1 << 13,
+  NF_STAGE2 = NF_DNH_BF16 | NF_NOISE | NF_UP | NF_DX_BF16 | NF_DX_ACC,
+  NF_STAGE1 = (NF_DX_BF16 - 1)
+};
+template <int F> struct NormForm {
+  static __device__ __forceinline__ bool is(int bit, int run_time) { return F < 0 ? run_time != 0 : (F & bit) != 0; }
+  static __device__ __forceinline__ int act(int run_time) { return F < 0 ? run_time : (F & NF_ACT_MASK) >> NF_ACT_SHIFT; }
+  static constexpr int up = F < 0 ? -1 : ((F & NF_UP) ? 1 : 0);
+};
+
+template <int F>
+__device__ __forceinline__ void norm_bwd_stage1_body(const NormBwdParams& p) {
+  typedef NormForm<F> Fm;
   __shared__ f32x4 red[2][256];
   const int n = blockIdx.y, b = blockIdx.x, t = threadIdx.x;
   const int HW = p.H * p.W, C = p.C4 * 4;
@@ -94,57 +115,61 @@
     f32x4 s1 = (f32x4)(0.f), s2 = (f32x4)(0.f);
     if (r < R && g < p.C4) {
       const f32x4 mu = ld4(p.mean + (size_t)n * C + g * 4), rs = ld4(p.rstd + (size_t)n * C + g * 4);
-      const f32x4 ns4 = p.z ? ld4(p.ns + g * 4) : (f32x4)(0.f);
-      const XThread xt = xsrc_thread(p.xs, n, g);
+      const bool noise = Fm::is(NF_NOISE, p.z != nullptr), has_g1p = Fm::is(NF_G1P, p.g1p != nullptr), has_dgb = Fm::is(NF_DGB, p.dgb != nullptr);
+      const int act = Fm::act(p.act);
+      const f32x4 ns4 = noise ? ld4(p.ns + g * 4) : (f32x4)(0.f);
+      const XThread xt = xsrc_thread<Fm::up>(p.xs, n, g);
       struct In { f32x4 v, d, o, g1; float zz; };
       auto load = [&](int px) {
         In L;
         const size_t pix = (size_t)n * HW + px;
         L.v = ld4(xsrc_ptr(xt, px));
         L.zz = 0.f;
-        if (p.z) {
+        if (noise) {
           const int h = px / p.W, w = px - h * p.W;
           L.zz = p.z[((size_t)n * p.W + w) * p.H + h];
         }
-        L.d = p.dout_bf16 ? ld4_bf16(p.dout, pix * p.do_cs + p.do_co + g * 4) : ld4(p.dout + pix * p.do_cs + p.do_co + g * 4);
+        L.d = Fm::is(NF_DOUT_BF16, p.dout_bf16) ? ld4_bf16(p.dout, pix * p.do_cs + p.do_co + g * 4) : ld4(p.dout + pix * p.do_cs + p.do_co + g * 4);
         L.o = (f32x4)(0.f);
-        if (p.act != HRV_ACT_NONE) {
+        if (act != HRV_ACT_NONE) {
           const size_t oe = pix * p.out_cs + p.out_co + g * 4;
-          L.o = p.out_bf16 ? ld4_bf16(p.out, oe) : ld4(p.out + oe);
+          L.o = Fm::is(NF_OUT_BF16, p.out_bf16) ? ld4_bf16(p.out, oe) : ld4(p.out + oe);
         }
         L.g1 = (f32x4)(1.f);
-        if (p.g1p) {
+        if (has_g1p) {
           const size_t ge1 = pix * p.g_cs + p.g_co + g * 4;
-          L.g1 = p.g1p_bf16 ? ld4_bf16(p.g1p, ge1) : ld4(p.g1p + ge1);
+          L.g1 = Fm::is(NF_G1P_BF16, p.g1p_bf16) ? ld4_bf16(p.g1p, ge1) : ld4(p.g1p + ge1);
         }
         return L;
       };
       auto finish = [&](int px, const In& L) {
+#pragma clang fp contract(off)
         const size_t pix = (size_t)n * HW + px;
         f32x4 v = L.v;
-        if (p.z) v += L.zz * ns4;
+        if (noise) v = fma4((f32x4)(L.zz), ns4, v);
         const f32x4 nh = (v - mu) * rs;
         f32x4 dpre = L.d;
-        if (p.act != HRV_ACT_NONE) {
-#pragma unroll
-          for (int e = 0; e < 4; ++e) dpre[e] *= dact(L.o[e], p.act, p.slope);
+        if (act != HRV_ACT_NONE) {
+#pragma unroll
+          for (int e = 0; e < 4; ++e) dpre[e] *= dact(L.o[e], act, p.slope);
         }
         f32x4 dnh = dpre;
-        if (p.g1p) dnh *= L.g1;
-        if (p.dnh_bf16) st4_bf16(p.dnh, pix * p.dn_cs + p.dn_co + g * 4, dnh);
+        if (has_g1p) dnh *= L.g1;
+        if (Fm::is(NF_DNH_BF16, p.dnh_bf16)) st4_bf16(p.dnh, pix * p.dn_cs + p.dn_co + g * 4, dnh);
         else *reinterpret_cast<f32x4*>(p.dnh + pix * p.dn_cs + p.dn_co + g * 4) = dnh;
-        if (p.dgb) {
+        if (has_dgb) {
+          const bool keep_dbeta = Fm::is(NF_DBETA_IN_PLACE, p.dbeta_in_place);
           const size_t ge = pix * p.dgb_cs + p.dgb_co + g * 4;
-          if (p.dgb_bf16) {
+          if (Fm::is(NF_DGB_BF16, p.dgb_bf16)) {
             st4_bf16(p.dgb, ge, dpre * nh);
-            if (!p.dbeta_in_place) st4_bf16(p.dgb, ge + C, dpre);
+            if (!keep_dbeta) st4_bf16(p.dgb, ge + C, dpre);
           } else {
             *reinterpret_cast<f32x4*>(p.dgb + ge) = dpre * nh;
-            if (!p.dbeta_in_place) *reinterpret_cast<f32x4*>(p.dgb + ge + C) = dpre;
+            if (!keep_dbeta) *reinterpret_cast<f32x4*>(p.dgb + ge + C) = dpre;
           }
         }
         s1 += dnh;
-        s2 += dnh * nh;
+        s2 = fma4(dnh, nh, s2);
       };
       int px = p0 + r;
       for (; px + R < p1; px += 2 * R) {
@@ -165,6 +190,9 @@
     }
   }
 }
+__global__ __launch_bounds__(256) void norm_bwd_stage1_kernel(const NormBwdParams p) { norm_bwd_stage1_body<-1>(p); }
+template <int F>
+__global__ __launch_bounds__(256) void norm_bwd_stage1_inst(const NormBwdParams p) { norm_bwd_stage1_body<F>(p); }
 
 __global__ void norm_bwd_finalize_kernel(const float* __restrict__ part, int N, int NB, int C, int HW,
                                          float* __restrict__ m1, float* __restrict__ m2) {
@@ -201,7 +229,9 @@
   int NB; float* part;
 };
 
-__global__ __launch_bounds__(256) void norm_bwd_stage2_kernel(const NormBwd2Params p) {
+template <int F>
+__device__ __forceinline__ void norm_bwd_stage2_body(const NormBwd2Params& p) {
+  typedef NormForm<F> Fm;
   __shared__ f32x4 red[256];
   const int n = blockIdx.y, b = blockIdx.x, t = threadIdx.x;
   const int HW = p.H * p.W, C = p.C4 * 4;
@@ -216,37 +246,38 @@
     if (r < R && g < p.C4) {
       const size_t sc = (size_t)n * C + g * 4;
       const f32x4 mu = ld4(p.mean + sc), rs = ld4(p.rstd + sc), a1 = ld4(p.m1 + sc), a2 = ld4(p.m2 + sc);
-      const f32x4 ns4 = p.z ? ld4(p.ns + g * 4) : (f32x4)(0.f);
-      const XThread xt = xsrc_thread(p.xs, n, g);
+      const bool noise = Fm::is(NF_NOISE, p.z != nullptr), dx_bf16 = Fm::is(NF_DX_BF16, p.dx_bf16), acc = Fm::is(NF_DX_ACC, p.accumulate);
+      const f32x4 ns4 = noise ? ld4(p.ns + g * 4) : (f32x4)(0.f);
+      const XThread xt = xsrc_thread<Fm::up>(p.xs, n, g);
       struct In { f32x4 v, dn, acc; float zz; };
       auto load = [&](int px) {
         In L;
         const size_t pix = (size_t)n * HW + px;
         L.v = ld4(xsrc_ptr(xt, px));
         L.zz = 0.f;
-        if (p.z) {
+        if (noise) {
           const int h = px / p.W, w = px - h * p.W;
           L.zz = p.z[((size_t)n * p.W + w) * p.H + h];
         }
         const size_t de = pix * p.dn_cs + p.dn_co + g * 4;
-        L.dn = p.dnh_bf16 ? ld4_bf16(p.dnh, de) : ld4(p.dnh + de);
+        L.dn = Fm::is(NF_DNH_BF16, p.dnh_bf16) ? ld4_bf16(p.dnh, de) : ld4(p.dnh + de);
         L.acc = (f32x4)(0.f);
-        if (!p.dx_bf16 && p.accumulate) L.acc = ld4(p.dx + pix * p.dx_cs + p.dx_co + g * 4);
+        if (!dx_bf16 && acc) L.acc = ld4(p.dx + pix * p.dx_cs + p.dx_co + g * 4);
         return L;
       };
       auto finish = [&](int px, const In& L) {
 #pragma clang fp contract(off)
         const size_t pix = (size_t)n * HW + px;
         f32x4 v = L.v;
-        if (p.z) v += L.zz * ns4;
+        if (noise) v += L.zz * ns4;
         const f32x4 nh = (v - mu) * rs;
         f32x4 d = rs * (L.dn - a1 - nh * a2);
         sz += d * L.zz;
-        if (p.dx_bf16) {
+        if (dx_bf16) {
           st4_bf16(p.dx, pix * p.dx_cs + p.dx_co + g * 4, d);
         } else {
           float* o = p.dx + pix * p.dx_cs + p.dx_co + g * 4;
-          if (p.accumulate) d += L.acc;
+          if (acc) d += L.acc;
           *reinterpret_cast<f32x4*>(o) = d;
         }
       };
@@ -258,7 +289,7 @@
       }
       if (px < p1) finish(px, load(px));
     }
-    if (p.z) {
+    if (Fm::is(NF_NOISE, p.z != nullptr)) {
       red[t] = sz;
       __syncthreads();
       if (r == 0 && g < p.C4) {
@@ -268,8 +299,13 @@
     }
   }
 }
-
-__global__ __launch_bounds__(256) void norm_bwd2_stage1_kernel(const NormBwdParams pa, const NormBwdParams pb) {
+__global__ __launch_bounds__(256) void norm_bwd_stage2_kernel(const NormBwd2Params p) { norm_bwd_stage2_body<-1>(p); }
+template <int F>
+__global__ __launch_bounds__(256) void norm_bwd_stage2_inst(const NormBwd2Params p) { norm_bwd_stage2_body<F>(p); }
+
+template <int F>
+__device__ __forceinline__ void norm_bwd2_stage1_body(const NormBwdParams& pa, const NormBwdParams& pb) {
+  typedef NormForm<F> Fm;
   __shared__ f32x4 red[4][256];
   const NormBwdParams& p = pa;
   const int n = blockIdx.y, b = blockIdx.x, t = threadIdx.x;
@@ -284,23 +320,23 @@
   if (r < R && g < p.C4) {
     const f32x4 mua = ld4(pa.mean + (size_t)n * C + g * 4), rsa = ld4(pa.rstd + (size_t)n * C + g * 4);
     const f32x4 mub = ld4(pb.mean + (size_t)n * C + g * 4), rsb = ld4(pb.rstd + (size_t)n * C + g * 4);
-    const f32x4 nsa = pa.z ? ld4(pa.ns + g * 4) : (f32x4)(0.f), nsb = pb.z ? ld4(pb.ns + g * 4) : (f32x4)(0.f);
-    const XThread xt = xsrc_thread(p.xs, n, g);
+    const f32x4 nsa = Fm::is(NF_NOISE, pa.z != nullptr) ? ld4(pa.ns + g * 4) : (f32x4)(0.f), nsb = Fm::is(NF_NOISE, pb.z != nullptr) ? ld4(pb.ns + g * 4) : (f32x4)(0.f);
+    const XThread xt = xsrc_thread<Fm::up>(p.xs, n, g);
     struct In1 { f32x4 d, o, g1; float zz; };
     struct In { f32x4 v; In1 a, b; };
     auto load1 = [&](const NormBwdParams& q, size_t pix, int h, int w) {
       In1 L;
-      L.zz = q.z ? q.z[((size_t)n * p.W + w) * p.H + h] : 0.f;
-      L.d = q.dout_bf16 ? ld4_bf16(q.dout, pix * q.do_cs + q.do_co + g * 4) : ld4(q.dout + pix * q.do_cs + q.do_co + g * 4);
+      L.zz = Fm::is(NF_NOISE, q.z != nullptr) ? q.z[((size_t)n * p.W + w) * p.H + h] : 0.f;
+      L.d = Fm::is(NF_DOUT_BF16, q.dout_bf16) ? ld4_bf16(q.dout, pix * q.do_cs + q.do_co + g * 4) : ld4(q.dout + pix * q.do_cs + q.do_co + g * 4);
       L.o = (f32x4)(0.f);
-      if (q.act != HRV_ACT_NONE) {
+      if (Fm::act(q.act) != HRV_ACT_NONE) {
         const size_t oe = pix * q.out_cs + q.out_co + g * 4;
-        L.o = q.out_bf16 ? ld4_bf16(q.out, oe) : ld4(q.out + oe);
+        L.o = Fm::is(NF_OUT_BF16, q.out_bf16) ? ld4_bf16(q.out, oe) : ld4(q.out + oe);
       }
       L.g1 = (f32x4)(1.f);
-      if (q.g1p) {
+      if (Fm::is(NF_G1P, q.g1p != nullptr)) {
         const size_t ge1 = pix * q.g_cs + q.g_co + g * 4;
-        L.g1 = q.g1p_bf16 ? ld4_bf16(q.g1p, ge1) : ld4(q.g1p + ge1);
+        L.g1 = Fm::is(NF_G1P_BF16, q.g1p_bf16) ? ld4_bf16(q.g1p, ge1) : ld4(q.g1p + ge1);
       }
       return L;
     };
@@ -314,29 +350,31 @@
       return L;
     };
     auto finish1 = [&](const NormBwdParams& q, size_t pix, f32x4 v, const In1& L, f32x4 mu, f32x4 rs, f32x4 ns4, f32x4& s1, f32x4& s2) {
-      if (q.z) v += L.zz * ns4;
+#pragma clang fp contract(off)
+      if (Fm::is(NF_NOISE, q.z != nullptr)) v = fma4((f32x4)(L.zz), ns4, v);
       const f32x4 nh = (v - mu) * rs;
       f32x4 dpre = L.d;
-      if (q.act != HRV_ACT_NONE) {
-#pragma unroll
-        for (int e = 0; e < 4; ++e) dpre[e] *= dact(L.o[e], q.act, q.slope);
+      if (Fm::act(q.act) != HRV_ACT_NONE) {
+#pragma unroll
+        for (int e = 0; e < 4; ++e) dpre[e] *= dact(L.o[e], Fm::act(q.act), q.slope);
       }
       f32x4 dnh = dpre;
-      if (q.g1p) dnh *= L.g1;
-      if (q.dnh_bf16) st4_bf16(q.dnh, pix * q.dn_cs + q.dn_co + g * 4, dnh);
+      if (Fm::is(NF_G1P, q.g1p != nullptr)) dnh *= L.g1;
+      if (Fm::is(NF_DNH_BF16, q.dnh_bf16)) st4_bf16(q.dnh, pix * q.dn_cs + q.dn_co + g * 4, dnh);
       else *reinterpret_cast<f32x4*>(q.dnh + pix * q.dn_cs + q.dn_co + g * 4) = dnh;
-      if (q.dgb) {
+      if (Fm::is(NF_DGB, q.dgb != nullptr)) {
+        const bool keep_dbeta = Fm::is(NF_DBETA_IN_PLACE, q.dbeta_in_place);
         const size_t ge = pix * q.dgb_cs + q.dgb_co + g * 4;
-        if (q.dgb_bf16) {
+        if (Fm::is(NF_DGB_BF16, q.dgb_bf16)) {
           st4_bf16(q.dgb, ge, dpre * nh);
-          if (!q.dbeta_in_place) st4_bf16(q.dgb, ge + C, dpre);
+          if (!keep_dbeta) st4_bf16(q.dgb, ge + C, dpre);
         } else {
           *reinterpret_cast<f32x4*>(q.dgb + ge) = dpre * nh;
-          if (!q.dbeta_in_place) *reinterpret_cast<f32x4*>(q.dgb + ge + C) = dpre;
+          if (!keep_dbeta) *reinterpret_cast<f32x4*>(q.dgb + ge + C) = dpre;
         }
       }
       s1 += dnh;
-      s2 += dnh * nh;
+      s2 = fma4(dnh, nh, s2);
     };
     auto finish = [&](int px, const In& L) {
       const size_t pix = (size_t)n * HW + px;
@@ -360,8 +398,13 @@
     }
   }
 }
-
-__global__ __launch_bounds__(256) void norm_bwd2_stage2_kernel(const NormBwd2Params pa, const NormBwd2Params pb) {
+__global__ __launch_bounds__(256) void norm_bwd2_stage1_kernel(const NormBwdParams pa, const NormBwdParams pb) { norm_bwd2_stage1_body<-1>(pa, pb); }
+template <int F>
+__global__ __launch_bounds__(256) void norm_bwd2_stage1_inst(const NormBwdParams pa, const NormBwdParams pb) { norm_bwd2_stage1_body<F>(pa, pb); }
+
+template <int F>
+__device__ __forceinline__ void norm_bwd2_stage2_body(const NormBwd2Params& pa, const NormBwd2Params& pb) {
+  typedef NormForm<F> Fm;
   __shared__ f32x4 red[2][256];
   const NormBwd2Params& p = pa;
   const int n = blockIdx.y, b = blockIdx.x, t = threadIdx.x;
@@ -377,8 +420,9 @@
     const size_t sc = (size_t)n * C + g * 4;
     const f32x4 mua = ld4(pa.mean + sc), rsa = ld4(pa.rstd + sc), a1a = ld4(pa.m1 + sc), a2a = ld4(pa.m2 + sc);
     const f32x4 mub = ld4(pb.mean + sc), rsb = ld4(pb.rstd + sc), a1b = ld4(pb.m1 + sc), a2b = ld4(pb.m2 + sc);
-    const f32x4 nsa = pa.z ? ld4(pa.ns + g * 4) : (f32x4)(0.f), nsb = pb.z ? ld4(pb.ns + g * 4) : (f32x4)(0.f);
-    const XThread xt = xsrc_thread(p.xs, n, g);
+    const bool za = Fm::is(NF_NOISE, pa.z != nullptr), zb = Fm::is(NF_NOISE, pb.z != nullptr);
+    const f32x4 nsa = za ? ld4(pa.ns + g * 4) : (f32x4)(0.f), nsb = zb ? ld4(pb.ns + g * 4) : (f32x4)(0.f);
+    const XThread xt = xsrc_thread<Fm::up>(p.xs, n, g);
     struct In { f32x4 v, dna, dnb; float za, zb; };
     auto load = [&](int px) {
       In L;
@@ -386,19 +430,19 @@
       L.v = ld4(xsrc_ptr(xt, px));
       const int h = px / p.W, w = px - h * p.W;
       const size_t zi = ((size_t)n * p.W + w) * p.H + h;
-      L.za = pa.z ? pa.z[zi] : 0.f;
-      L.zb = pb.z ? pb.z[zi] : 0.f;
+      L.za = za ? pa.z[zi] : 0.f;
+      L.zb = zb ? pb.z[zi] : 0.f;
       const size_t dea = pix * pa.dn_cs + pa.dn_co + g * 4, deb = pix * pb.dn_cs + pb.dn_co + g * 4;
-      L.dna = pa.dnh_bf16 ? ld4_bf16(pa.dnh, dea) : ld4(pa.dnh + dea);
-      L.dnb = pb.dnh_bf16 ? ld4_bf16(pb.dnh, deb) : ld4(pb.dnh + deb);
+      L.dna = Fm::is(NF_DNH_BF16, pa.dnh_bf16) ? ld4_bf16(pa.dnh, dea) : ld4(pa.dnh + dea);
+      L.dnb = Fm::is(NF_DNH_BF16, pb.dnh_bf16) ? ld4_bf16(pb.dnh, deb) : ld4(pb.dnh + deb);
       return L;
     };
     auto finish = [&](int px, const In& L) {
 #pragma clang fp contract(off)
       const size_t pix = (size_t)n * HW + px;
       f32x4 va = L.v, vb = L.v;
-      if (pa.z) va += L.za * nsa;
-      if (pb.z) vb += L.zb * nsb;
+      if (za) va += L.za * nsa;
+      if (zb) vb += L.zb * nsb;
       const f32x4 nha = (va - mua) * rsa, nhb = (vb - mub) * rsb;
       const f32x4 da = rsa * (L.dna - a1a - nha * a2a);
       const f32x4 db = rsb * (L.dnb - a1b - nhb * a2b);
@@ -418,10 +462,13 @@
   __syncthreads();
   if (r == 0 && g < p.C4) {
     for (int rr = 1; rr < R; ++rr) { sza += red[0][rr * GB + gl]; szb += red[1][rr * GB + gl]; }
-    if (pa.z) *reinterpret_cast<f32x4*>(pa.part + ((size_t)n * p.NB + b) * C + g * 4) = sza;
-    if (pb.z) *reinterpret_cast<f32x4*>(pb.part + ((size_t)n * p.NB + b) * C + g * 4) = szb;
-  }
-}
+    if (Fm::is(NF_NOISE, pa.z != nullptr)) *reinterpret_cast<f32x4*>(pa.part + ((size_t)n * p.NB + b) * C + g * 4) = sza;
+    if (Fm::is(NF_NOISE, pb.z != nullptr)) *reinterpret_cast<f32x4*>(pb.part + ((size_t)n * p.NB + b) * C + g * 4) = szb;
+  }
+}
+__global__ __launch_bounds__(256) void norm_bwd2_stage2_kernel(const NormBwd2Params pa, const NormBwd2Params pb) { norm_bwd2_stage2_body<-1>(pa, pb); }
+template <int F>
+__global__ __launch_bounds__(256) void norm_bwd2_stage2_inst(const NormBwd2Params pa, const NormBwd2Params pb) { norm_bwd2_stage2_body<F>(pa, pb); }
 
 template <bool AB>
 __global__ __launch_bounds__(256) void loss_kernel(const float* __restrict__ a, const float* __restrict__ b, size_t n,
@@ -1100,6 +1147,121 @@
   q.N = d->N; q.H = d->H; q.W = d->W; q.C4 = C / 4; q.NB = nb; q.part = part;
 }
 
+static int norm_form_of(const hrv_norm_bwd_t* d, const NormBwdParams& p) {
+  int f = 0;
+  if (d->dout_bf16) f |= NF_DOUT_BF16;
+  f |= (d->act << NF_ACT_SHIFT) & NF_ACT_MASK;
+  if (d->act != HRV_ACT_NONE && d->out_bf16) f |= NF_OUT_BF16;
+  if (d->g1p) f |= NF_G1P | (d->g1p_bf16 ? NF_G1P_BF16 : 0);
+  if (d->dnh_bf16) f |= NF_DNH_BF16;
+  if (d->dgb) f |= NF_DGB | (d->dgb_bf16 ? NF_DGB_BF16 : 0) | (p.dbeta_in_place ? NF_DBETA_IN_PLACE : 0);
+  if (d->noise_z) f |= NF_NOISE;
+  if (d->x_up_channels > 0) f |= NF_UP;
+  if (d->dx_bf16) f |= NF_DX_BF16;
+  else if (d->dx_accumulate) f |= NF_DX_ACC;
+  return f;
+}
+
+constexpr int NF_SPADE = NF_DOUT_BF16 | NF_G1P | NF_DNH_BF16 | NF_DGB | NF_DGB_BF16 | NF_DBETA_IN_PLACE | NF_NOISE;
+constexpr int NF_IN_LRELU = (HRV_ACT_LRELU << NF_ACT_SHIFT) | NF_DNH_BF16;
+constexpr int NF_S2 = NF_DNH_BF16 | NF_NOISE;
+
+typedef void (*norm_s1_fn)(const NormBwdParams);
+typedef void (*norm_s2_fn)(const NormBwd2Params);
+typedef void (*norm_p1_fn)(const NormBwdParams, const NormBwdParams);
+typedef void (*norm_p2_fn)(const NormBwd2Params, const NormBwd2Params);
+template <class Fn> struct NormInst { int form; Fn fn; };
+#define S1(F) {F, norm_bwd_stage1_inst<F>}
+#define S2(F) {F, norm_bwd_stage2_inst<F>}
+#define P1(F) {F, norm_bwd2_stage1_inst<F>}
+#define P2(F) {F, norm_bwd2_stage2_inst<F>}
+static const NormInst<norm_s1_fn> norm_s1_insts[] = {S1(NF_SPADE | NF_G1P_BF16), S1(NF_SPADE | NF_G1P_BF16 | NF_UP), S1(NF_SPADE), S1(NF_IN_LRELU),
+                                                     S1(NF_IN_LRELU | NF_DOUT_BF16 | NF_OUT_BF16)};
+static const NormInst<norm_s2_fn> norm_s2_insts[] = {S2(NF_S2 | NF_DX_BF16), S2(NF_S2), S2(NF_S2 | NF_DX_ACC), S2(NF_S2 | NF_UP), S2(NF_S2 | NF_UP | NF_DX_ACC),
+                                                     S2(NF_DNH_BF16 | NF_DX_BF16)};
+static const NormInst<norm_p1_fn> norm_p1_insts[] = {P1(NF_SPADE | NF_G1P_BF16 | NF_UP), P1(NF_SPADE)};
+static const NormInst<norm_p2_fn> norm_p2_insts[] = {P2(NF_S2 | NF_UP), P2(NF_S2)};
+#undef S1
+#undef S2
+#undef P1
+#undef P2
+
+static bool norm_generic_forced() {
+  const char* e = hrv::env("HRV_NORM_BWD_GENERIC");
+  return e && atoi(e) != 0;
+}
+template <class Fn, size_t K>
+static Fn norm_inst_for(const NormInst<Fn> (&tab)[K], int form) {
+  if (!norm_generic_forced())
+    for (size_t i = 0; i < K; ++i)
+      if (tab[i].form == form) return tab[i].fn;
+  return nullptr;
+}
+
+static std::string norm_form_name(int f) {
+  static const struct { int bit; const char* name; } bits[] = {
+      {NF_DOUT_BF16, "dout_bf16"}, {NF_OUT_BF16, "out_bf16"}, {NF_G1P, "g1p"}, {NF_G1P_BF16, "g1p_bf16"}, {NF_DNH_BF16, "dnh_bf16"}, {NF_DGB, "dgb"},
+      {NF_DGB_BF16, "dgb_bf16"}, {NF_DBETA_IN_PLACE, "dbeta_in_place"}, {NF_NOISE, "noise"}, {NF_UP, "up"}, {NF_DX_BF16, "dx_bf16"}, {NF_DX_ACC, "dx_acc"}};
+  static const char* acts[] = {"", "relu", "lrelu", "tanh"};
+  std::string s = acts[(f & NF_ACT_MASK) >> NF_ACT_SHIFT];
+  for (const auto& b : bits)
+    if (f & b.bit) s += (s.empty() ? "" : "+") + std::string(b.name);
+  return s.empty() ? "plain" : s;
+}
+
+extern "C" const char* hrv_diag_norm_bwd_instances(void) {
+  static const std::string text = [] {
+    std::string t;
+    for (const auto& i : norm_s1_insts) t += "single.stage1 " + norm_form_name(i.form) + "\n";
+    for (const auto& i : norm_s2_insts) t += "single.stage2 " + norm_form_name(i.form) + "\n";
+    for (const auto& i : norm_p1_insts) t += "pair.stage1 " + norm_form_name(i.form) + "\n";
+    for (const auto& i : norm_p2_insts) t += "pair.stage2 " + norm_form_name(i.form) + "\n";
+    return t;
+  }();
+  return text.c_str();
+}
+
+static int norm_bwd2_check(const hrv_norm_bwd_t* a, const hrv_norm_bwd_t* b) {
+  int rc = norm_bwd_check(a);
+  if (rc) return rc;
+  rc = norm_bwd_check(b);
+  if (rc) return rc;
+  HRV_REQUIRE(a->x == b->x && a->x2 == b->x2 && a->x_cstride == b->x_cstride && a->x_coff == b->x_coff && a->x_up_channels == b->x_up_channels &&
+                  a->N == b->N && a->H == b->H && a->W == b->W && a->C == b->C,
+              "norm_bwd2: both norms must normalise the same x");
+  HRV_REQUIRE(!a->dx_bf16 && !a->dx_accumulate && a->workspace != b->workspace && a->dnh != b->dnh, "norm_bwd2: dx fp32 (written, = dx_a + dx_b); separate scratch");
+  return HRV_OK;
+}
+static void norm_bwd2_route(const hrv_norm_bwd_t* a, const hrv_norm_bwd_t* b, const NormBwdParams& pa, const NormBwdParams& pb, norm_p1_fn& k1,
+                            norm_p2_fn& k2) {
+  const int fa = norm_form_of(a, pa), fb = norm_form_of(b, pb) & ~NF_DX_ACC & ~NF_DX_BF16;
+  k1 = (fa & NF_STAGE1) == (fb & NF_STAGE1) ? norm_inst_for(norm_p1_insts, fa & NF_STAGE1) : nullptr;
+  k2 = (fa & NF_STAGE2) == (fb & NF_STAGE2) ? norm_inst_for(norm_p2_insts, fa & NF_STAGE2) : nullptr;
+}
+
+extern "C" int hrv_diag_norm_bwd_route(const hrv_norm_bwd_t* a, const hrv_norm_bwd_t* b) {
+  const int rc = b ? norm_bwd2_check(a, b) : norm_bwd_check(a);
+  if (rc) return rc;
+  NormBwdParams pa, pb;
+  NormBwd2Params qa, qb;
+  float *m1, *m2;
+  norm_bwd_fill(a, pa, qa, m1, m2);
+  if (!b) {
+    const int f = norm_form_of(a, pa);
+    return (norm_inst_for(norm_s1_insts, f & NF_STAGE1) ? 1 : 0) | (norm_inst_for(norm_s2_insts, f & NF_STAGE2) ? 2 : 0);
+  }
+  norm_bwd_fill(b, pb, qb, m1, m2);
+  norm_p1_fn k1;
+  norm_p2_fn k2;
+  norm_bwd2_route(a, b, pa, pb, k1, k2);
+  return (k1 ? 1 : 0) | (k2 ? 2 : 0);
+}
+
+extern "C" int hrv_spade_norm_bwd2_supported(const hrv_norm_bwd_t* a, const hrv_norm_bwd_t* b) {
+  if (norm_bwd2_check(a, b)) return 0;
+  return hrv_diag_norm_bwd_route(a, b) == 3 ? 1 : 0;
+}
+
 extern "C" int hrv_spade_norm_bwd_nhwc_f32(const hrv_norm_bwd_t* d, hrv_stream_t stream) {
   int rc = norm_bwd_check(d);
   if (rc) return rc;
@@ -1110,13 +1272,16 @@
   NormBwd2Params q;
   float *m1, *m2;
   norm_bwd_fill(d, p, q, m1, m2);
-  hipLaunchKernelGGL(norm_bwd_stage1_kernel, dim3(nb, d->N, norm_chunks(C / 4)), dim3(256), 0, st, p);
+  const int form = norm_form_of(d, p);
+  const norm_s1_fn k1 = norm_inst_for(norm_s1_insts, form & NF_STAGE1);
+  const norm_s2_fn k2 = norm_inst_for(norm_s2_insts, form & NF_STAGE2);
+  hipLaunchKernelGGL(k1 ? k1 : norm_bwd_stage1_kernel, dim3(nb, d->N, norm_chunks(C / 4)), dim3(256), 0, st, p);
   rc = check_launch("norm_bwd_stage1_kernel");
   if (rc) return rc;
   hipLaunchKernelGGL(norm_bwd_finalize_kernel, dim3((d->N * C * 16 + 255) / 256), dim3(256), 0, st, p.part, d->N, nb, C, HW, m1, m2);
   rc = check_launch("norm_bwd_finalize_kernel");
   if (rc) return rc;
-  hipLaunchKernelGGL(norm_bwd_stage2_kernel, dim3(nb, d->N, norm_chunks(C / 4)), dim3(256), 0, st, q);
+  hipLaunchKernelGGL(k2 ? k2 : norm_bwd_stage2_kernel, dim3(nb, d->N, norm_chunks(C / 4)), dim3(256), 0, st, q);
   rc = check_launch("norm_bwd_stage2_kernel");
   if (rc) return rc;
   if (d->noise_z && d->dnoise_scale) {
@@ -1128,14 +1293,8 @@
 }
 
 extern "C" int hrv_spade_norm_bwd2_nhwc_f32(const hrv_norm_bwd_t* a, const hrv_norm_bwd_t* b, hrv_stream_t stream) {
-  int rc = norm_bwd_check(a);
+  int rc = norm_bwd2_check(a, b);
   if (rc) return rc;
-  rc = norm_bwd_check(b);
-  if (rc) return rc;
-  HRV_REQUIRE(a->x == b->x && a->x2 == b->x2 && a->x_cstride == b->x_cstride && a->x_coff == b->x_coff && a->x_up_channels == b->x_up_channels &&
-                  a->N == b->N && a->H == b->H && a->W == b->W && a->C == b->C,
-              "norm_bwd2: both norms must normalise the same x");
-  HRV_REQUIRE(!a->dx_bf16 && !a->dx_accumulate && a->workspace != b->workspace && a->dnh != b->dnh, "norm_bwd2: dx fp32 (written, = dx_a + dx_b); separate scratch");
   const int HW = a->H * a->W, C = a->C;
   const int nb = norm_slabs(HW);
   hipStream_t st = (hipStream_t)stream;
@@ -1144,14 +1303,17 @@
   float *m1a, *m2a, *m1b, *m2b;
   norm_bwd_fill(a, pa, qa, m1a, m2a);
   norm_bwd_fill(b, pb, qb, m1b, m2b);
-  hipLaunchKernelGGL(norm_bwd2_stage1_kernel, dim3(nb, a->N, norm_chunks(C / 4)), dim3(256), 0, st, pa, pb);
+  norm_p1_fn k1;
+  norm_p2_fn k2;
+  norm_bwd2_route(a, b, pa, pb, k1, k2);
+  hipLaunchKernelGGL(k1 ? k1 : norm_bwd2_stage1_kernel, dim3(nb, a->N, norm_chunks(C / 4)), dim3(256), 0, st, pa, pb);
   rc = check_launch("norm_bwd2_stage1_kernel");
   if (rc) return rc;
   hipLaunchKernelGGL(norm_bwd_finalize_kernel, dim3((a->N * C * 16 + 255) / 256), dim3(256), 0, st, pa.part, a->N, nb, C, HW, m1a, m2a);
   hipLaunchKernelGGL(norm_bwd_finalize_kernel, dim3((a->N * C * 16 + 255) / 256), dim3(256), 0, st, pb.part, a->N, nb, C, HW, m1b, m2b);
   rc = check_launch("norm_bwd_finalize_kernel");
   if (rc) return rc;
-  hipLaunchKernelGGL(norm_bwd2_stage2_kernel, dim3(nb, a->N, norm_chunks(C / 4)), dim3(256), 0, st, qa, qb);
+  hipLaunchKernelGGL(k2 ? k2 : norm_bwd2_stage2_kernel, dim3(nb, a->N, norm_chunks(C / 4)), dim3(256), 0, st, qa, qb);
   rc = check_launch("norm_bwd2_stage2_kernel");
   if (rc) return rc;
   const hrv_norm_bwd_t* ds[2] = {a, b};
diff --git a/hr-viton_amd/gen_train.py b/hr-viton_amd/gen_train.py
--- a/hr-viton_amd/gen_train.py
+++ b/hr-viton_amd/gen_train.py
@@ -311,7 +311,7 @@
                     dgb_bf16=ctx["actv"].bf16)
 
     def dout_slot(self, ctx, want_bf16: bool):
-        if (os.environ.get("HRV_DBETA_INPLACE", "1") == "0" or os.environ.get("HRV_NORM_BWD2", "0") != "0" or
+        if (os.environ.get("HRV_DBETA_INPLACE", "1") == "0" or
                 not T.MMA_BF16[0] or not want_bf16 or self.Cp != self.C or
                 self.C % 8 != 0 or not ctx["actv"].bf16 or not ctx["out"].bf16):
             return None
@@ -500,18 +500,25 @@
         d_h1, dgb1 = down(self.c1, d_out, ctx["h1"], self.n1, ctx["n1"])
         d_dx = self.n1.backward(ctx["n1"], d_h1, grads, None, False, dact_all.slice(hid * (k0 + 1), hid), dx_bf16=True, dgb=dgb1)
         d_h0, dgb0 = down(self.c0, d_dx, ctx["h0"], self.n0, ctx["n0"])
-        if (self.learned and ctx["n0"]["z"] is not None and ctx["ns"]["z"] is not None and not x.bf16 and
-                os.environ.get("HRV_NORM_BWD2", "0") != "0"):
-            d_hs = self.cs.backward(d_out, [(ctx["hs"], 0)], grads, dx_bf16=dh16 and ctx["hs"].bf16)
+        mode = os.environ.get("HRV_NORM_BWD2", "")
+        d_hs = None
+        if self.learned and mode != "0" and ctx["n0"]["z"] is not None and ctx["ns"]["z"] is not None and not x.bf16:
+            d_hs, dgbs = down(self.cs, d_out, ctx["hs"], self.ns_, ctx["ns"])
             a0, as_ = self.n0.norm_args(ctx["n0"], d_h0), self.ns_.norm_args(ctx["ns"], d_hs)
-            d_x, dgb0, dgbs = T.norm_bwd2(x, a0, as_)
-            self.n0.after_norm(ctx["n0"], dgb0, a0["dnoise_scale"], grads, dact_all.slice(hid * k0, hid))
-            self.ns_.after_norm(ctx["ns"], dgbs, as_["dnoise_scale"], grads, dact_all.slice(0, hid))
-            self.shared_backward(ctx["segx"], dact_all, grads)
-            return d_x
+            for a, dgb in ((a0, dgb0), (as_, dgbs)):
+                if dgb is not None:
+                    a.update(act=ACT_NONE, out=None, dgb=dgb)
+            pair = T.norm_bwd2(x, a0, as_, only_where_faster=mode != "1")
+            if pair is not None:
+                d_x, dgb0, dgbs = pair
+                self.n0.after_norm(ctx["n0"], dgb0, a0["dnoise_scale"], grads, dact_all.slice(hid * k0, hid))
+                self.ns_.after_norm(ctx["ns"], dgbs, as_["dnoise_scale"], grads, dact_all.slice(0, hid))
+                self.shared_backward(ctx["segx"], dact_all, grads)
+                return d_x
         d_x = self.n0.backward(ctx["n0"], d_h0, grads, None, False, dact_all.slice(hid * k0, hid), dgb=dgb0)
         if self.learned:
-            d_hs, dgbs = down(self.cs, d_out, ctx["hs"], self.ns_, ctx["ns"])
+            if d_hs is None:
+                d_hs, dgbs = down(self.cs, d_out, ctx["hs"], self.ns_, ctx["ns"])
             self.ns_.backward(ctx["ns"], d_hs, grads, d_x, True, dact_all.slice(0, hid), dgb=dgbs)
         else:
             T.add_slice(d_out, d_x, True)
diff --git a/hr-viton_amd/train_ops.py b/hr-viton_amd/train_ops.py
--- a/hr-viton_amd/train_ops.py
+++ b/hr-viton_amd/train_ops.py
@@ -743,15 +743,27 @@
     return d, dx, dgb, (dnh, ws)
 
 
+def _norm_bwd_bytes(d, in_place: bool, second_of_pair: bool = False) -> float:
+    w = lambda bf16: 2 if bf16 else 4
+    s1 = 4 + w(d.dout_bf16) + (w(d.out_bf16) if d.act != ACT_NONE else 0) + (w(d.g1p_bf16) if d.g1p else 0) + w(d.dnh_bf16)
+    if d.dgb:
+        s1 += w(d.dgb_bf16) * (1 if in_place else 2)
+    s2 = 4 + w(d.dnh_bf16) + w(d.dx_bf16) + (4 if d.dx_accumulate else 0)
+    if second_of_pair:
+        s1, s2 = s1 - 4, s2 - 4 - w(d.dx_bf16)
+    return float(d.N) * d.H * d.W * d.C * (s1 + s2)
+
+
 def norm_bwd(x: Act, mean: torch.Tensor, rstd: torch.Tensor, dout: Act, act: int = ACT_NONE, slope: float = 0.2,
              out: Optional[Act] = None, g1p: Optional[Act] = None, z: Optional[torch.Tensor] = None,
              noise_scale: Optional[torch.Tensor] = None, want_dgb: bool = False, dx: Optional[Act] = None,
              dx_accumulate: bool = False, dnoise_scale: Optional[torch.Tensor] = None, dns_accumulate: bool = False,
              dgb_bf16: bool = False, dx_bf16: bool = False, dgb: Optional[Act] = None):
     lib = _lib.load()
+    in_place = dgb is not None
     d, dx, dgb, _keep = _norm_bwd_desc(x, mean, rstd, dout, act, slope, out, g1p, z, noise_scale, want_dgb, dx, dx_accumulate, dnoise_scale,
                                        dns_accumulate, dgb_bf16, dx_bf16, dgb)
-    with _Timed("norm_bwd", "spade_norm_bwd", 0.0, 4.0 * x.N * x.H * x.W * x.Cp * (7 + (2 if want_dgb else 0))):
+    with _Timed("norm_bwd", "spade_norm_bwd", 0.0, _norm_bwd_bytes(d, in_place)):
         _lib.check(lib.hrv_spade_norm_bwd_nhwc_f32(C.byref(d), _stream()), "hrv_spade_norm_bwd_nhwc_f32")
     return dx, dgb
 
@@ -761,17 +773,24 @@
     return dgb, dgb.slice(x.Cp, x.C)
 
 
-def norm_bwd2(x: Act, a: dict, b: dict):
+def norm_bwd2(x: Act, a: dict, b: dict, only_where_faster: bool = False):
     lib = _lib.load()
     da, dx, dgb_a, _ka = _norm_bwd_desc(x, a["mean"], a["rstd"], a["dout"], a.get("act", ACT_NONE), a.get("slope", 0.2), a.get("out"), a.get("g1p"),
                                         a.get("z"), a.get("noise_scale"), a.get("want_dgb", False), None, False, a.get("dnoise_scale"),
-                                        a.get("dns_accumulate", False), a.get("dgb_bf16", False), False)
+                                        a.get("dns_accumulate", False), a.get("dgb_bf16", False), False, a.get("dgb"))
     db, _, dgb_b, _kb = _norm_bwd_desc(x, b["mean"], b["rstd"], b["dout"], b.get("act", ACT_NONE), b.get("slope", 0.2), b.get("out"), b.get("g1p"),
                                        b.get("z"), b.get("noise_scale"), b.get("want_dgb", False), dx, False, b.get("dnoise_scale"),
-                                       b.get("dns_accumulate", False), b.get("dgb_bf16", False), False)
-    with _Timed("norm_bwd", "spade_norm_bwd x2", 0.0, 4.0 * x.N * x.H * x.W * x.Cp * (10 + 2 * (a.get("want_dgb", False) + b.get("want_dgb", False)))):
+                                       b.get("dns_accumulate", False), b.get("dgb_bf16", False), False, b.get("dgb"))
+    if only_where_faster and not lib.hrv_spade_norm_bwd2_supported(C.byref(da), C.byref(db)):
+        return None
+    nbytes = _norm_bwd_bytes(da, a.get("dgb") is not None) + _norm_bwd_bytes(db, b.get("dgb") is not None, second_of_pair=True)
+    with _Timed("norm_bwd", "spade_norm_bwd x2", 0.0, nbytes):
         _lib.check(lib.hrv_spade_norm_bwd2_nhwc_f32(C.byref(da), C.byref(db), _stream()), "hrv_spade_norm_bwd2_nhwc_f32")
     return dx, dgb_a, dgb_b
+
+
+def norm_bwd_instances():
+    return _lib.load().hrv_diag_norm_bwd_instances().decode().splitlines()
 
 
 LOSS_L1, LOSS_HINGE_D_FAKE, LOSS_HINGE_D_REAL, LOSS_NEG_MEAN, LOSS_MSE = 0, 1, 2, 3, 4
diff --git a/include/hrviton_hip.h b/include/hrviton_hip.h
--- a/include/hrviton_hip.h
+++ b/include/hrviton_hip.h
@@ -174,6 +174,9 @@
 int hrv_thin_conv_bf16(const hrv_thin_conv_t* d, hrv_stream_t stream);
 int hrv_spade_norm_bwd_nhwc_f32(const hrv_norm_bwd_t* d, hrv_stream_t stream);
 int hrv_spade_norm_bwd2_nhwc_f32(const hrv_norm_bwd_t* a, const hrv_norm_bwd_t* b, hrv_stream_t stream);
+const char* hrv_diag_norm_bwd_instances(void);
+int hrv_diag_norm_bwd_route(const hrv_norm_bwd_t* a, const hrv_norm_bwd_t* b);
+int hrv_spade_norm_bwd2_supported(const hrv_norm_bwd_t* a, const hrv_norm_bwd_t* b);
 int hrv_loss_f32(const float* a, const float* b, int64_t n, int32_t mode, float lscale, float gscale, float* grad,
                  float* workspace, float* loss_out, int32_t accumulate, hrv_stream_t stream);
 int hrv_loss_bf16in_f32(const uint16_t* a, const uint16_t* b, int64_t n, int32_t mode, float lscale, float gscale, float* grad,
```

Measured after the change: 61.51 images/s, median of 6. +2.5%, better.
